# sergiventosa/ts-PWS

Hardware: AMD Instinct MI355X
Metric: stacked samples/s (Morlet ts-PWS, 10k×131072) + % HBM roofline, 1/2/4/8 GPU (higher is better)
Workload: dtype f64; 1 GPU; 10000 traces/GPU x 131072 samples, Morlet w0=pi*sqrt(2/ln2) V=4 J=14, two-stage K=10 + unbiased phase coherence (BASELINE configs[2]); HBM-resident float32 traces; traces_total=10000, traces_per_gpu=10000, parallelism=one GPU: no collective, world_size=1

## Files before the change

include/tspws_hip.h:

```cpp
#ifndef TSPWS_HIP_H
#define TSPWS_HIP_H

#include <stddef.h>
#include <stdint.h>
#include "ts_pws1f_lib.h"

#ifdef __cplusplus
extern "C" {
#endif

enum {
	TSPWS_OK        = 0,
	TSPWS_E_ARG     = -1,
	TSPWS_E_NOMEM   = 4,
	TSPWS_E_NODEV   = 5,
	TSPWS_E_HIP     = 6,
	TSPWS_E_FRAME   = 7
};

typedef struct tspws_hip_plan tspws_hip_plan;

typedef struct {
	int      type;
	unsigned S, V, J, N;
	double   s0, b0, w0;
	double   Cpsi;
	size_t   ncoef;
	size_t   ntaps;
	int      device;
} tspws_hip_frame_info;

int         tspws_hip_device_count(void);
const char *tspws_hip_last_error(void);
int  tspws_hip_alloc(void **d_ptr, size_t bytes, int device);
int  tspws_hip_free(void *d_ptr);
int  tspws_hip_upload(void *d_dst, const void *h_src, size_t bytes, void *stream);
int  tspws_hip_download(void *h_dst, const void *d_src, size_t bytes, void *stream);
int  tspws_hip_zero(void *d_ptr, size_t bytes, void *stream);
int  tspws_hip_sync(void *stream);


void tspws_resolve_params(t_tsPWS *p, unsigned nsamp, float dt);

int  tspws_hip_plan_create(tspws_hip_plan **plan, int type, unsigned J, unsigned V, unsigned N,
                           double s0, double b0, double w0, int uni, int device);
void tspws_hip_plan_destroy(tspws_hip_plan *plan);
int  tspws_hip_plan_info(const tspws_hip_plan *plan, tspws_hip_frame_info *info);
int  tspws_hip_plan_tables(const tspws_hip_plan *plan, double *scale, unsigned *L, int *c, int *cd,
                           unsigned *D, unsigned *Ns);
int  tspws_hip_plan_taps(const tspws_hip_plan *plan, double *h_w, double *h_wd);

int  tspws_hip_fold(float *d_sigall, size_t mtr, size_t max, size_t ld, void *stream);
int  tspws_hip_remove_mean(float *d_sigall, size_t mtr, size_t max, size_t ld, void *stream);

int  tspws_hip_partial_stacks(tspws_hip_plan *plan, const float *d_sigall, size_t ld,
                              size_t mtr_local, size_t first, size_t mtr_global, unsigned Kmax,
                              double *d_P, size_t ldP, void *stream);

int  tspws_hip_partial_stacks_range(tspws_hip_plan *plan, const float *d_sigall, size_t ld,
                                    size_t mtr_local, size_t first, size_t mtr_global, unsigned Kmax,
                                    unsigned g_begin, unsigned g_end, double *d_P, size_t ldP, void *stream);

int  tspws_hip_forward_f64(tspws_hip_plan *plan, const double *d_x, size_t ntr, size_t ld, double *d_Y, void *stream);
int  tspws_hip_forward_f32(tspws_hip_plan *plan, const float  *d_x, size_t ntr, size_t ld, double *d_Y, void *stream);
unsigned tspws_hip_spectral_first_scale(const tspws_hip_plan *plan, unsigned nsmax);
unsigned tspws_hip_spectral_end_scale(const tspws_hip_plan *plan);
unsigned tspws_hip_spectral_transform_length(const tspws_hip_plan *plan);
unsigned tspws_hip_spectral_choice(const tspws_hip_plan *plan, size_t ntr);
int  tspws_hip_forward_spectral_f64(tspws_hip_plan *plan, const double *d_x, size_t ntr, size_t ld, double *d_Y, unsigned nsmax, void *stream);
int  tspws_hip_forward_spectral_f32(tspws_hip_plan *plan, const float  *d_x, size_t ntr, size_t ld, double *d_Y, unsigned nsmax, void *stream);
int  tspws_hip_inverse(tspws_hip_plan *plan, const double *d_Y, size_t nrec, double *d_x, void *stream);
typedef struct {
	unsigned items;
	unsigned per_scale;
	unsigned waves;
	unsigned waves_lds;
	unsigned waves_fast;
	unsigned generic;
} tspws_hip_inverse_info_t;
int  tspws_hip_inverse_info(const tspws_hip_plan *plan, tspws_hip_inverse_info_t *info);

typedef struct { unsigned s_begin, s_end; } tspws_band;
#define TSPWS_MAX_BANDS 1024u
int  tspws_hip_inverse_bands(tspws_hip_plan *plan, const double *d_Y, size_t nset, const tspws_band *h_bands, unsigned R,
                             double *d_re, double *d_im, void *stream);
int  tspws_bands_from_frequencies(const double *scale, unsigned S, double w0, double dt, const double *f_lo, const double *f_hi, unsigned R,
                                  tspws_band *bands, double *fc);

int  tspws_hip_accumulate(tspws_hip_plan *plan, const double *d_Y, size_t ntr, double *d_ST, double *d_PS,
                          int zero_first, void *stream);
int  tspws_hip_stacks_double(tspws_hip_plan *plan, const double *d_P, unsigned K, size_t ldP,
                             double *d_ST, double *d_PS, void *stream);
int  tspws_hip_stacks_float(tspws_hip_plan *plan, const float *d_sigall, size_t mtr, size_t ld,
                            double *d_ST, double *d_PS, void *stream);
int  tspws_hip_weight(tspws_hip_plan *plan, double *d_OUT, const double *d_ST, const double *d_PS,
                      unsigned K, unsigned M, double wu, int unbiased, void *stream);
int  tspws_hip_epilogue(float *d_ls, float *d_tsPWS, const double *d_x_st, const double *d_x_out,
                        size_t N, unsigned mtr, void *stream);

int  tspws_hip_stack_local(tspws_hip_plan *plan, const t_tsPWS *p, const float *d_sigall, size_t ld,
                           size_t mtr_local, size_t first, size_t mtr_global, void *stream);
int  tspws_hip_reduce_buffer(tspws_hip_plan *plan, const t_tsPWS *p, size_t mtr_global,
                             double **d_buf, size_t *ndoubles);
int  tspws_hip_stack_finish(tspws_hip_plan *plan, const t_tsPWS *p, size_t mtr_global,
                            float *d_ls, float *d_tsPWS, void *stream);

int  tspws_hip_stack_finish_range(tspws_hip_plan *plan, const t_tsPWS *p, size_t mtr_global,
                                  unsigned g_begin, unsigned g_end, void *stream);
int  tspws_hip_stack_finish_tail(tspws_hip_plan *plan, const t_tsPWS *p, size_t mtr_global,
                                 float *d_ls, float *d_tsPWS, void *stream);

int  tspws_hip_stack(tspws_hip_plan *plan, const t_tsPWS *p, const float *d_sigall, size_t ld, size_t mtr,
                     float *d_ls, float *d_tsPWS, void *stream);
int  tspws_hip_stack_batch(tspws_hip_plan *plan, const t_tsPWS *p, const float *d_sigall, size_t ld, const size_t *h_first, unsigned B,
                           float *d_ls, float *d_tsPWS, void *stream);
typedef struct {
	unsigned single_pass;
	unsigned two_stage_pass;
	unsigned looped;
	unsigned empty;
	unsigned rounds;
	unsigned pass_batches;
} tspws_hip_batch_stats;
int  tspws_hip_stack_batch_stats(const tspws_hip_plan *plan, tspws_hip_batch_stats *stats);
int  tspws_hip_stack_batch_bands(tspws_hip_plan *plan, const t_tsPWS *p, const float *d_sigall, size_t ld, const size_t *h_first, unsigned B,
                                 const tspws_band *h_bands, unsigned R, float *d_ls, float *d_tsPWS, float *d_ls_env, float *d_tsPWS_env,
                                 void *stream);
typedef struct {
	tspws_hip_batch_stats batch;
	unsigned finish_batches;
	unsigned scales;
	unsigned quadrature;
} tspws_hip_stack_bands_stats;
int  tspws_hip_stack_batch_bands_stats(const tspws_hip_plan *plan, tspws_hip_stack_bands_stats *stats);
int  tspws_hip_profile_begin(tspws_hip_plan *plan, size_t max_calls);
int  tspws_hip_profile_read(tspws_hip_plan *plan, double *stage_ms, double *call_ms, size_t cap, size_t *ncalls);
int  tspws_hip_profile_end(tspws_hip_plan *plan, double *mean_ms, size_t *ncalls);
int  tspws_hip_stream_launches(const tspws_hip_plan *plan);

int  tspws_hip_finish_shard(const tspws_hip_plan *plan, const t_tsPWS *p, size_t mtr_global, unsigned rank, unsigned world,
                            unsigned *s_begin, unsigned *s_end);
int  tspws_hip_stack_finish_scales(tspws_hip_plan *plan, const t_tsPWS *p, size_t mtr_global, unsigned s_begin, unsigned s_end,
                                   double *d_x2, void *stream);

int  tspws_jackknife_plan(char *sel, const time_t *time, size_t mtr, unsigned d, unsigned n, unsigned C);
int  tspws_hip_jackknife(tspws_hip_plan *plan, const t_tsPWS *p, const float *d_sigall, size_t ld,
                         size_t mtr, const char *h_sel, unsigned C,
                         float *d_ls_out, float *d_ts_out, unsigned *h_mtr_out, void *stream);

int  tspws_hip_stack_jackknife(tspws_hip_plan *plan, const t_tsPWS *p, const float *d_sigall, size_t ld, size_t mtr,
                               float *d_ls, float *d_tsPWS, const char *h_sel, unsigned C,
                               float *d_ls_out, float *d_ts_out, unsigned *h_mtr_out, void *stream);

int  tspws_hip_jackknife_buffer(tspws_hip_plan *plan, const t_tsPWS *p, unsigned C, double **d_buf, size_t *nd);
int  tspws_hip_jackknife_local(tspws_hip_plan *plan, const t_tsPWS *p, const float *d_sigall, size_t ld, size_t mtr_local,
                               size_t first, size_t mtr_global, const char *h_sel, unsigned C, void *stream);
int  tspws_hip_jackknife_finish(tspws_hip_plan *plan, const t_tsPWS *p, size_t mtr_global, const char *h_sel, unsigned C,
                                unsigned c_begin, unsigned c_end, float *d_ls_out, float *d_ts_out, unsigned *h_mtr_out,
                                void *stream);

int  tspws_selection_classes(const char *sel, unsigned C, size_t mtr, unsigned *class_of_trace, char *kept, unsigned *ncls);
int  tspws_hip_jackknife_single(tspws_hip_plan *plan, const t_tsPWS *p, const float *d_sigall, size_t ld, size_t mtr,
                                const char *h_sel, unsigned C, float *d_ls_out, float *d_ts_out, unsigned *h_mtr_out, void *stream);

int  tspws_hip_jackknife_batch(tspws_hip_plan *plan, const t_tsPWS *p, const float *d_sigall, size_t ld, const size_t *h_first, unsigned B,
                               const char *h_sel, unsigned C, float *d_ls, float *d_tsPWS, float *d_ls_out, float *d_ts_out,
                               unsigned *h_mtr_out, void *stream);
typedef struct {
	unsigned shared;
	unsigned looped;
	unsigned empty;
	unsigned rounds;
	unsigned pass_batches;
	unsigned classes;
} tspws_hip_jk_batch_stats;
int  tspws_hip_jackknife_batch_stats(const tspws_hip_plan *plan, tspws_hip_jk_batch_stats *stats);

int  tspws_hip_jackknife_batch_two_stage(tspws_hip_plan *plan, const t_tsPWS *p, const float *d_sigall, size_t ld, const size_t *h_first,
                                         unsigned B, const char *h_sel, unsigned C, float *d_ls, float *d_tsPWS, float *d_ls_out,
                                         float *d_ts_out, unsigned *h_mtr_out, void *stream);
typedef struct {
	unsigned shared;
	unsigned looped;
	unsigned empty;
	unsigned rounds;
	unsigned tiles;
	unsigned rows;
} tspws_hip_jk_batch2_stats;
int  tspws_hip_jackknife_batch_two_stage_stats(const tspws_hip_plan *plan, tspws_hip_jk_batch2_stats *stats);

int  tspws_subsampling_plan(char *sel, size_t J, size_t K);
int  tspws_hip_subsample(tspws_hip_plan *plan, const t_tsPWS *p, const float *d_sigall, size_t ld, size_t mtr, unsigned M,
                         float *d_ls_out, float *d_ts_out, void *stream);
int  tspws_hip_subsample_sel(tspws_hip_plan *plan, const t_tsPWS *p, const float *d_sigall, size_t ld, size_t mtr, unsigned M,
                             const char *h_sel, float *d_ls_out, float *d_ts_out, void *stream);

int  tspws_subsampling_plan_batch(char *sel, const size_t *first, unsigned B, unsigned M, double prob);
int  tspws_hip_subsample_batch_sel(tspws_hip_plan *plan, const t_tsPWS *p, const float *d_sigall, size_t ld, const size_t *h_first, unsigned B,
                                   unsigned M, const char *h_sel, float *d_ls_out, float *d_ts_out, unsigned *h_mtr_out, void *stream);
int  tspws_hip_subsample_batch(tspws_hip_plan *plan, const t_tsPWS *p, const float *d_sigall, size_t ld, const size_t *h_first, unsigned B,
                               unsigned M, float *d_ls_out, float *d_ts_out, unsigned *h_mtr_out, void *stream);
typedef struct {
	unsigned single_shared;
	unsigned two_stage_shared;
	unsigned looped;
	unsigned empty;
	unsigned rounds;
	unsigned rows;
} tspws_hip_sub_batch_stats;
int  tspws_hip_subsample_batch_stats(const tspws_hip_plan *plan, tspws_hip_sub_batch_stats *stats);

int  tspws_bootstrap_plan(unsigned char *cnt, size_t J);
int  tspws_bootstrap_plan_batch(unsigned char *cnt, const size_t *first, unsigned B, unsigned M);
int  tspws_hip_bootstrap_batch_cnt(tspws_hip_plan *plan, const t_tsPWS *p, const float *d_sigall, size_t ld, const size_t *h_first, unsigned B,
                                   unsigned M, const unsigned char *h_cnt, float *d_ls_out, float *d_ts_out, unsigned *h_mtr_out, float *d_stats,
                                   void *stream);
int  tspws_hip_bootstrap_batch(tspws_hip_plan *plan, const t_tsPWS *p, const float *d_sigall, size_t ld, const size_t *h_first, unsigned B,
                               unsigned M, float *d_ls_out, float *d_ts_out, unsigned *h_mtr_out, float *d_stats, void *stream);
typedef struct {
	unsigned shared;
	unsigned empty;
	unsigned rounds;
	unsigned rows;
	unsigned max_count;
} tspws_hip_boot_batch_stats;
int  tspws_hip_bootstrap_batch_stats(const tspws_hip_plan *plan, tspws_hip_boot_batch_stats *stats);

int  tspws_hip_weighted_stack_batch(tspws_hip_plan *plan, const t_tsPWS *p, const float *d_sigall, size_t ld, const size_t *h_first, unsigned B,
                                    unsigned M, const double *h_w, float *d_ls_out, float *d_ts_out, unsigned *h_mtr_out, double *h_keff,
                                    void *stream);
typedef struct {
	unsigned shared;
	unsigned empty;
	unsigned rounds;
	unsigned rows;
} tspws_hip_weighted_batch_stats;
int  tspws_hip_weighted_stack_batch_stats(const tspws_hip_plan *plan, tspws_hip_weighted_batch_stats *stats);
int  tspws_weights_from_scores(double *w, const double *score, const size_t *first, unsigned B, int rule, double a);

int  tspws_hip_replica_bands(tspws_hip_plan *plan, const float *d_rows, size_t ld, unsigned B, unsigned M, const unsigned *h_mtr,
                             const double *h_q, unsigned Q, float *d_bands, void *stream);
typedef struct {
	unsigned lds;
	unsigned global;
	unsigned empty;
	unsigned rounds;
	unsigned lds_max_rows;
} tspws_hip_bands_stats;
int  tspws_hip_replica_bands_stats(const tspws_hip_plan *plan, tspws_hip_bands_stats *stats);

int  tspws_hip_trace_scores(tspws_hip_plan *plan, const float *d_sigall, size_t ld, const size_t *h_first, unsigned B, const float *d_ref,
                            size_t ldr, unsigned R, size_t n0, size_t n1, double *d_scores, double *d_energy, void *stream);
typedef struct {
	unsigned vec;
	unsigned segments;
	unsigned rounds;
	unsigned empty;
} tspws_hip_trace_scores_stats_t;
int  tspws_hip_trace_scores_stats(const tspws_hip_plan *plan, tspws_hip_trace_scores_stats_t *stats);
int  tspws_selection_from_scores(char *sel, unsigned *kept, const double *score, const size_t *first, unsigned B, int rule, double a);
int  tspws_hip_selective_stack_batch(tspws_hip_plan *plan, const t_tsPWS *p, const float *d_sigall, size_t ld, const size_t *h_first, unsigned B,
                                     int against, int rule, double a, unsigned iters, size_t n0, size_t n1, float *d_ls, float *d_tsPWS,
                                     char *h_sel, unsigned *h_kept, unsigned *iters_done, void *stream);

int  tspws_hip_stretch_rows(tspws_hip_plan *plan, const float *d_rows, size_t ld, unsigned B, unsigned M, const unsigned *h_mtr,
                            const float *d_ref, size_t ldr, double z, const double *h_eps, unsigned E, const size_t *h_win, unsigned W,
                            double *d_cc, double *d_fit, void *stream);
typedef struct {
	unsigned rounds;
	unsigned segments;
	unsigned rows;
	unsigned left_out;
	unsigned chunks;
} tspws_hip_stretch_stats;
int  tspws_hip_stretch_rows_stats(const tspws_hip_plan *plan, tspws_hip_stretch_stats *stats);
int  tspws_stretch_grid(double *eps, double eps_max, unsigned E);

int  tspws_hip_wxs_coef(tspws_hip_plan *plan, const double *d_Yc, const double *d_Yr, const unsigned *h_ens, size_t nrow, unsigned B, double z,
                        const tspws_band *h_bands, unsigned R, const size_t *h_win, unsigned W, int skip_wrapped, double *d_sums, double *d_fit,
                        void *stream);
int  tspws_hip_wxs_rows(tspws_hip_plan *plan, const float *d_rows, size_t ld, unsigned B, unsigned M, const unsigned *h_mtr, const float *d_ref,
                        size_t ldr, double z, const tspws_band *h_bands, unsigned R, const size_t *h_win, unsigned W, int skip_wrapped,
                        double *d_sums, double *d_fit, void *stream);
typedef struct {
	unsigned rounds;
	unsigned rows;
	unsigned left_out;
	unsigned items;
	unsigned scales;
} tspws_hip_wxs_stats;
int  tspws_hip_wxs_rows_stats(const tspws_hip_plan *plan, tspws_hip_wxs_stats *stats);

typedef struct {
	unsigned L, hop, P, q0, q1, h;
	double taper, min_coh, max_err, max_delta, err_floor;
} tspws_mwcs_par;
int    tspws_mwcs_bins(unsigned P, double dt, double f_lo, double f_hi, unsigned *q0, unsigned *q1);
size_t tspws_mwcs_basis_size(const tspws_mwcs_par *par);
int    tspws_mwcs_basis(const tspws_mwcs_par *par, double *tab);
int  tspws_hip_mwcs_rows(tspws_hip_plan *plan, const float *d_rows, size_t ld, unsigned B, unsigned M, const unsigned *h_mtr, const float *d_ref,
                         size_t ldr, double z, const tspws_mwcs_par *par, const size_t *h_win, unsigned W, double *d_win, double *d_fit,
                         double *d_spec, double *d_spec_ref, void *stream);
typedef struct {
	unsigned rounds;
	unsigned rows;
	unsigned left_out;
	unsigned windows;
	unsigned bins;
} tspws_hip_mwcs_stats;
int  tspws_hip_mwcs_rows_stats(const tspws_hip_plan *plan, tspws_hip_mwcs_stats *stats);

typedef struct { unsigned Lmax, b; } tspws_dtw_par;
int  tspws_hip_dtw_rows(tspws_hip_plan *plan, const float *d_rows, size_t ld, unsigned B, unsigned M, const unsigned *h_mtr, const float *d_ref,
                        size_t ldr, double z, const tspws_dtw_par *par, const size_t *h_win, unsigned W, int *d_lag, double *d_fit, void *stream);
typedef struct {
	unsigned rounds;
	unsigned rows;
	unsigned left_out;
	unsigned lags;
	unsigned samples;
} tspws_hip_dtw_stats;
int  tspws_hip_dtw_rows_stats(const tspws_hip_plan *plan, tspws_hip_dtw_stats *stats);

int  tspws_hip_ftan_coef(tspws_hip_plan *plan, const double *d_Y, const unsigned *h_ens, size_t nrow, unsigned B, double z, unsigned s_begin,
                         unsigned s_end, const size_t *h_win, unsigned W, const size_t *h_noise, unsigned P, int skip_wrapped, double *d_peaks,
                         double *d_noise, void *stream);
int  tspws_hip_ftan_rows(tspws_hip_plan *plan, const float *d_rows, size_t ld, unsigned B, unsigned M, const unsigned *h_mtr, double z,
                         unsigned s_begin, unsigned s_end, const size_t *h_win, unsigned W, const size_t *h_noise, unsigned P, int skip_wrapped,
                         double *d_peaks, double *d_noise, void *stream);
typedef struct {
	unsigned rounds;
	unsigned rows;
	unsigned left_out;
	unsigned items;
	unsigned classes;
} tspws_hip_ftan_stats;
int  tspws_hip_ftan_rows_stats(const tspws_hip_plan *plan, tspws_hip_ftan_stats *stats);
int  tspws_ftan_windows(double dist, double vmin, double vmax, double dt, double z, size_t N, int sides, size_t *win);
int  tspws_ftan_periods(const double *scale, unsigned S, double w0, double dt, double *T);

int  tspws_hip_convergence(tspws_hip_plan *plan, const t_tsPWS *p, const float *d_sigall, size_t ld, size_t mtr,
                           const float *d_ref_ts, const float *d_ref_ls, double *h_ts_sim, double *h_ts_misfit,
                           double *h_ls_sim, double *h_ls_misfit, float *d_ts_steps, float *d_ls_steps, void *stream);

int  tspws_hip_convergence_batch(tspws_hip_plan *plan, const t_tsPWS *p, const float *d_sigall, size_t ld, const size_t *h_first, unsigned B,
                                 const float *d_ref_ts, const float *d_ref_ls, double *h_ts_sim, double *h_ts_misfit, double *h_ls_sim,
                                 double *h_ls_misfit, float *d_ts_steps, float *d_ls_steps, void *stream);
typedef struct {
	unsigned single_steps;
	unsigned two_stage_steps;
	unsigned rows;
	unsigned rounds;
	unsigned looped;
	unsigned empty;
} tspws_hip_conv_batch_stats;
int  tspws_hip_convergence_batch_stats(const tspws_hip_plan *plan, tspws_hip_conv_batch_stats *stats);

typedef struct tspws_hip_comm tspws_hip_comm;
int   tspws_hip_comm_create(tspws_hip_comm **comm, int ndev, const int *devices);
void  tspws_hip_comm_destroy(tspws_hip_comm *comm);
int   tspws_hip_comm_size(const tspws_hip_comm *comm);
int   tspws_hip_comm_device(const tspws_hip_comm *comm, int i);
void *tspws_hip_comm_stream(const tspws_hip_comm *comm, int i);
const char *tspws_hip_comm_backend(const tspws_hip_comm *comm);
int   tspws_hip_allreduce_f64(tspws_hip_comm *comm, double *const *d_bufs, size_t count, void *const *streams);
int   tspws_hip_reduce_f64(tspws_hip_comm *comm, double *const *d_bufs, size_t count, int root, void *const *streams);
void  tspws_shard_range(size_t mtr, unsigned r, unsigned n, size_t *first, size_t *count);

typedef struct tspws_hip_multi tspws_hip_multi;
int   tspws_hip_multi_create(tspws_hip_multi **m, int ndev, const int *devices, int type, unsigned J, unsigned V, unsigned N,
                             double s0, double b0, double w0, int uni);
void  tspws_hip_multi_destroy(tspws_hip_multi *m);
tspws_hip_comm *tspws_hip_multi_comm(tspws_hip_multi *m);
// ... 21 lines not shown
```

ts-pws_amd/__init__.py:

```python
import ctypes as C
import os
import subprocess

_HERE = os.path.dirname(os.path.abspath(__file__))
ROOT = os.path.dirname(_HERE)
LIB_PATH = os.environ.get("TSPWS_LIB_PATH") or os.path.join(_HERE, "lib", "libtspws_hip.so")

time_t = C.c_long


class t_tsPWS(C.Structure):
    _fields_ = [
        ("type", C.c_int), ("uni", C.c_uint), ("J", C.c_uint), ("V", C.c_uint),
        ("s0", C.c_double), ("b0", C.c_double), ("w0", C.c_double), ("wu", C.c_double),
        ("fmin", C.c_double), ("Q", C.c_double), ("cycle", C.c_double),
        ("w0set", C.c_int), ("lrm", C.c_int), ("bin", C.c_int), ("lkinst", C.c_int),
        ("lVfix", C.c_int), ("ls0fix", C.c_int), ("lb0fix", C.c_int), ("verbose", C.c_int),
        ("fold", C.c_int), ("unbiased", C.c_int), ("convergence", C.c_int),
        ("subsmpl_N", C.c_uint), ("subsmpl_p", C.c_double),
        ("jackknife_n", C.c_uint), ("jackknife_d", C.c_uint), ("obin", C.c_uint),
        ("AllSteps", C.c_int), ("Nmax", C.c_uint), ("Kmax", C.c_uint),
        ("kinst", C.c_char_p), ("filein", C.c_char_p), ("fileout", C.c_char_p), ("fileconv", C.c_char_p),
    ]


class FrameInfo(C.Structure):
    _fields_ = [
        ("type", C.c_int), ("S", C.c_uint), ("V", C.c_uint), ("J", C.c_uint), ("N", C.c_uint),
        ("s0", C.c_double), ("b0", C.c_double), ("w0", C.c_double), ("Cpsi", C.c_double),
        ("ncoef", C.c_size_t), ("ntaps", C.c_size_t), ("device", C.c_int),
    ]


class InverseInfo(C.Structure):
    _fields_ = [("items", C.c_uint), ("per_scale", C.c_uint), ("waves", C.c_uint), ("waves_lds", C.c_uint), ("waves_fast", C.c_uint),
                ("generic", C.c_uint)]


class TspwsError(RuntimeError):
    pass


def build(verbose=False):
    out = subprocess.run(["make", "-C", _HERE, "all"], capture_output=True, text=True)
    if verbose or out.returncode:
        print(out.stdout + out.stderr)
    if out.returncode:
        raise TspwsError("building libtspws_hip.so failed")
    return LIB_PATH


_lib = None

_vp, _u, _d, _sz, _i, _f = C.c_void_p, C.c_uint, C.c_double, C.c_size_t, C.c_int, C.c_float
SYMBOLS = {
    "tspws_main": (_i, [_vp, _vp, _vp]),
    "tspws_hip_device_count": (_i, []),
    "tspws_hip_last_error": (C.c_char_p, []),
    "tspws_hip_alloc": (_i, [C.POINTER(_vp), _sz, _i]),
    "tspws_hip_free": (_i, [_vp]),
    "tspws_hip_upload": (_i, [_vp, _vp, _sz, _vp]),
    "tspws_hip_download": (_i, [_vp, _vp, _sz, _vp]),
    "tspws_hip_zero": (_i, [_vp, _sz, _vp]),
    "tspws_hip_sync": (_i, [_vp]),
    "tspws_resolve_params": (None, [_vp, _u, _f]),
    "tspws_hip_plan_create": (_i, [C.POINTER(_vp), _i, _u, _u, _u, _d, _d, _d, _i, _i]),
    "tspws_hip_plan_destroy": (None, [_vp]),
    "tspws_hip_plan_info": (_i, [_vp, _vp]),
    "tspws_hip_plan_tables": (_i, [_vp] + [_vp] * 6),
    "tspws_hip_plan_taps": (_i, [_vp, _vp, _vp]),
    "tspws_hip_fold": (_i, [_vp, _sz, _sz, _sz, _vp]),
    "tspws_hip_remove_mean": (_i, [_vp, _sz, _sz, _sz, _vp]),
    "tspws_hip_partial_stacks": (_i, [_vp, _vp, _sz, _sz, _sz, _sz, _u, _vp, _sz, _vp]),
    "tspws_hip_partial_stacks_range": (_i, [_vp, _vp, _sz, _sz, _sz, _sz, _u, _u, _u, _vp, _sz, _vp]),
    "tspws_hip_forward_f64": (_i, [_vp, _vp, _sz, _sz, _vp, _vp]),
    "tspws_hip_forward_f32": (_i, [_vp, _vp, _sz, _sz, _vp, _vp]),
    "tspws_hip_spectral_first_scale": (_u, [_vp, _u]),
    "tspws_hip_spectral_end_scale": (_u, [_vp]),
    "tspws_hip_spectral_transform_length": (_u, [_vp]),
    "tspws_hip_spectral_choice": (_u, [_vp, _sz]),
    "tspws_hip_forward_spectral_f64": (_i, [_vp, _vp, _sz, _sz, _vp, _u, _vp]),
    "tspws_hip_forward_spectral_f32": (_i, [_vp, _vp, _sz, _sz, _vp, _u, _vp]),
    "tspws_hip_inverse": (_i, [_vp, _vp, _sz, _vp, _vp]),
    "tspws_hip_inverse_info": (_i, [_vp, _vp]),
    "tspws_hip_inverse_bands": (_i, [_vp, _vp, _sz, _vp, _u, _vp, _vp, _vp]),
    "tspws_bands_from_frequencies": (_i, [_vp, _u, _d, _d, _vp, _vp, _u, _vp, _vp]),
    "tspws_hip_accumulate": (_i, [_vp, _vp, _sz, _vp, _vp, _i, _vp]),
    "tspws_hip_stacks_double": (_i, [_vp, _vp, _u, _sz, _vp, _vp, _vp]),
    "tspws_hip_stacks_float": (_i, [_vp, _vp, _sz, _sz, _vp, _vp, _vp]),
    "tspws_hip_weight": (_i, [_vp, _vp, _vp, _vp, _u, _u, _d, _i, _vp]),
    "tspws_hip_epilogue": (_i, [_vp, _vp, _vp, _vp, _sz, _u, _vp]),
    "tspws_hip_stack_local": (_i, [_vp, _vp, _vp, _sz, _sz, _sz, _sz, _vp]),
    "tspws_hip_reduce_buffer": (_i, [_vp, _vp, _sz, C.POINTER(_vp), C.POINTER(_sz)]),
    "tspws_hip_stack_finish": (_i, [_vp, _vp, _sz, _vp, _vp, _vp]),
    "tspws_hip_stack_finish_range": (_i, [_vp, _vp, _sz, _u, _u, _vp]),
    "tspws_hip_stack_finish_tail": (_i, [_vp, _vp, _sz, _vp, _vp, _vp]),
    "tspws_hip_stack": (_i, [_vp, _vp, _vp, _sz, _sz, _vp, _vp, _vp]),
    "tspws_hip_stack_batch": (_i, [_vp, _vp, _vp, _sz, _vp, _u, _vp, _vp, _vp]),
    "tspws_hip_stack_batch_stats": (_i, [_vp, _vp]),
    "tspws_hip_stack_batch_bands": (_i, [_vp, _vp, _vp, _sz, _vp, _u, _vp, _u, _vp, _vp, _vp, _vp, _vp]),
    "tspws_hip_stack_batch_bands_stats": (_i, [_vp, _vp]),
    "tspws_hip_profile_begin": (_i, [_vp, _sz]),
    "tspws_hip_profile_read": (_i, [_vp, _vp, _vp, _sz, C.POINTER(_sz)]),
    "tspws_hip_profile_end": (_i, [_vp, C.POINTER(_d), C.POINTER(_sz)]),
    "tspws_hip_stream_launches": (_i, [_vp]),
    "tspws_jackknife_plan": (_i, [_vp, _vp, _sz, _u, _u, _u]),
    "tspws_hip_jackknife": (_i, [_vp, _vp, _vp, _sz, _sz, _vp, _u, _vp, _vp, _vp, _vp]),
    "tspws_hip_stack_jackknife": (_i, [_vp, _vp, _vp, _sz, _sz, _vp, _vp, _vp, _u, _vp, _vp, _vp, _vp]),
    "tspws_main_release": (None, []),
    "tspws_main_on": (_i, [_i, _vp, _vp, _vp]),
    "tspws_main_cached_devices": (C.c_ulonglong, []),
    "tspws_hip_finish_shard": (_i, [_vp, _vp, _sz, _u, _u, C.POINTER(_u), C.POINTER(_u)]),
    "tspws_hip_stack_finish_scales": (_i, [_vp, _vp, _sz, _u, _u, _vp, _vp]),
    "tspws_hip_jackknife_buffer": (_i, [_vp, _vp, _u, C.POINTER(_vp), C.POINTER(_sz)]),
    "tspws_hip_jackknife_local": (_i, [_vp, _vp, _vp, _sz, _sz, _sz, _sz, _vp, _u, _vp]),
    "tspws_hip_jackknife_finish": (_i, [_vp, _vp, _sz, _vp, _u, _u, _u, _vp, _vp, _vp, _vp]),
    "tspws_selection_classes": (_i, [_vp, _u, _sz, _vp, _vp, C.POINTER(_u)]),
    "tspws_hip_jackknife_single": (_i, [_vp, _vp, _vp, _sz, _sz, _vp, _u, _vp, _vp, _vp, _vp]),
    "tspws_hip_jackknife_batch": (_i, [_vp, _vp, _vp, _sz, _vp, _u, _vp, _u, _vp, _vp, _vp, _vp, _vp, _vp]),
    "tspws_hip_jackknife_batch_stats": (_i, [_vp, _vp]),
    "tspws_hip_jackknife_batch_two_stage": (_i, [_vp, _vp, _vp, _sz, _vp, _u, _vp, _u, _vp, _vp, _vp, _vp, _vp, _vp]),
    "tspws_hip_jackknife_batch_two_stage_stats": (_i, [_vp, _vp]),
    "tspws_subsampling_plan": (_i, [_vp, _sz, _sz]),
    "tspws_hip_subsample": (_i, [_vp, _vp, _vp, _sz, _sz, _u, _vp, _vp, _vp]),
    "tspws_hip_subsample_sel": (_i, [_vp, _vp, _vp, _sz, _sz, _u, _vp, _vp, _vp, _vp]),
    "tspws_subsampling_plan_batch": (_i, [_vp, _vp, _u, _u, _d]),
    "tspws_hip_subsample_batch_sel": (_i, [_vp, _vp, _vp, _sz, _vp, _u, _u, _vp, _vp, _vp, _vp, _vp]),
    "tspws_hip_subsample_batch": (_i, [_vp, _vp, _vp, _sz, _vp, _u, _u, _vp, _vp, _vp, _vp]),
    "tspws_hip_subsample_batch_stats": (_i, [_vp, _vp]),
    "tspws_bootstrap_plan": (_i, [_vp, _sz]),
    "tspws_bootstrap_plan_batch": (_i, [_vp, _vp, _u, _u]),
    "tspws_hip_bootstrap_batch_cnt": (_i, [_vp, _vp, _vp, _sz, _vp, _u, _u, _vp, _vp, _vp, _vp, _vp, _vp]),
    "tspws_hip_bootstrap_batch": (_i, [_vp, _vp, _vp, _sz, _vp, _u, _u, _vp, _vp, _vp, _vp, _vp]),
    "tspws_hip_bootstrap_batch_stats": (_i, [_vp, _vp]),
    "tspws_hip_weighted_stack_batch": (_i, [_vp, _vp, _vp, _sz, _vp, _u, _u, _vp, _vp, _vp, _vp, _vp, _vp]),
    "tspws_hip_weighted_stack_batch_stats": (_i, [_vp, _vp]),
    "tspws_weights_from_scores": (_i, [_vp, _vp, _vp, _u, _i, _d]),
    "tspws_hip_replica_bands": (_i, [_vp, _vp, _sz, _u, _u, _vp, _vp, _u, _vp, _vp]),
    "tspws_hip_replica_bands_stats": (_i, [_vp, _vp]),
    "tspws_hip_trace_scores": (_i, [_vp, _vp, _sz, _vp, _u, _vp, _sz, _u, _sz, _sz, _vp, _vp, _vp]),
    "tspws_hip_trace_scores_stats": (_i, [_vp, _vp]),
    "tspws_selection_from_scores": (_i, [_vp, _vp, _vp, _vp, _u, _i, _d]),
    "tspws_hip_stretch_rows": (_i, [_vp, _vp, _sz, _u, _u, _vp, _vp, _sz, _d, _vp, _u, _vp, _u, _vp, _vp, _vp]),
    "tspws_hip_stretch_rows_stats": (_i, [_vp, _vp]),
    "tspws_stretch_grid": (_i, [_vp, _d, _u]),
    "tspws_hip_wxs_coef": (_i, [_vp, _vp, _vp, _vp, _sz, _u, _d, _vp, _u, _vp, _u, _i, _vp, _vp, _vp]),
    "tspws_hip_wxs_rows": (_i, [_vp, _vp, _sz, _u, _u, _vp, _vp, _sz, _d, _vp, _u, _vp, _u, _i, _vp, _vp, _vp]),
    "tspws_hip_wxs_rows_stats": (_i, [_vp, _vp]),
    "tspws_hip_mwcs_rows": (_i, [_vp, _vp, _sz, _u, _u, _vp, _vp, _sz, _d, _vp, _vp, _u, _vp, _vp, _vp, _vp, _vp]),
    "tspws_hip_mwcs_rows_stats": (_i, [_vp, _vp]),
    "tspws_mwcs_bins": (_i, [_u, _d, _d, _d, _vp, _vp]),
    "tspws_hip_dtw_rows": (_i, [_vp, _vp, _sz, _u, _u, _vp, _vp, _sz, _d, _vp, _vp, _u, _vp, _vp, _vp]),
    "tspws_hip_dtw_rows_stats": (_i, [_vp, _vp]),
    "tspws_hip_ftan_coef": (_i, [_vp, _vp, _vp, _sz, _u, _d, _u, _u, _vp, _u, _vp, _u, _i, _vp, _vp, _vp]),
    "tspws_hip_ftan_rows": (_i, [_vp, _vp, _sz, _u, _u, _vp, _d, _u, _u, _vp, _u, _vp, _u, _i, _vp, _vp, _vp]),
    "tspws_hip_ftan_rows_stats": (_i, [_vp, _vp]),
    "tspws_ftan_windows": (_i, [_d, _d, _d, _d, _d, _sz, _i, _vp]),
    "tspws_ftan_periods": (_i, [_vp, _u, _d, _d, _vp]),
    "tspws_mwcs_basis_size": (_sz, [_vp]),
    "tspws_mwcs_basis": (_i, [_vp, _vp]),
    "tspws_hip_selective_stack_batch": (_i, [_vp, _vp, _vp, _sz, _vp, _u, _i, _i, _d, _u, _sz, _sz, _vp, _vp, _vp, _vp, _vp, _vp]),
    "tspws_hip_convergence": (_i, [_vp, _vp, _vp, _sz, _sz, _vp, _vp, _vp, _vp, _vp, _vp, _vp, _vp, _vp]),
    "tspws_hip_convergence_batch": (_i, [_vp, _vp, _vp, _sz, _vp, _u, _vp, _vp, _vp, _vp, _vp, _vp, _vp, _vp, _vp]),
    "tspws_hip_convergence_batch_stats": (_i, [_vp, _vp]),
    "tspws_hip_synth": (_i, [_vp, _sz, _sz, _sz, C.c_uint64, _sz, _vp]),
    "tspws_hip_comm_create": (_i, [C.POINTER(_vp), _i, _vp]),
    "tspws_hip_comm_destroy": (None, [_vp]),
    "tspws_hip_comm_size": (_i, [_vp]),
    "tspws_hip_comm_device": (_i, [_vp, _i]),
    "tspws_hip_comm_stream": (_vp, [_vp, _i]),
    "tspws_hip_comm_backend": (C.c_char_p, [_vp]),
    "tspws_hip_allreduce_f64": (_i, [_vp, _vp, _sz, _vp]),
    "tspws_hip_reduce_f64": (_i, [_vp, _vp, _sz, _i, _vp]),
    "tspws_shard_range": (None, [_sz, _u, _u, C.POINTER(_sz), C.POINTER(_sz)]),
    "tspws_hip_multi_create": (_i, [C.POINTER(_vp), _i, _vp, _i, _u, _u, _u, _d, _d, _d, _i]),
    "tspws_hip_multi_destroy": (None, [_vp]),
    "tspws_hip_multi_comm": (_vp, [_vp]),
    "tspws_hip_multi_plan": (_vp, [_vp, _i]),
    "tspws_hip_multi_upload": (_i, [_vp, _vp, _sz, _sz, C.POINTER(_vp), C.POINTER(_vp), C.POINTER(_vp)]),
    "tspws_hip_multi_prologue": (_i, [_vp, _vp, _sz, _sz, _sz, _i, _i]),
    "tspws_hip_multi_stack": (_i, [_vp, _vp, _vp, _sz, _sz, _vp, _vp]),
    "tspws_hip_multi_stack_jackknife": (_i, [_vp, _vp, _vp, _sz, _sz, _vp, _vp, _vp, _u, _vp, _vp, _vp]),
}


def load():
    global _lib
    if _lib is None:
        if not os.path.exists(LIB_PATH):
            raise TspwsError(f"{LIB_PATH} is missing: run __graft_entry__.build() / make -C ts-pws_amd")
        try:
            import torch
        except ImportError:
            pass
        lib = C.CDLL(LIB_PATH)
        for name, (res, args) in SYMBOLS.items():
            fn = getattr(lib, name)
            fn.restype, fn.argtypes = res, args
        _lib = lib
    return _lib


def check(rc, what=""):
    if rc:
        raise TspwsError(f"{what} failed with code {rc}: {load().tspws_hip_last_error().decode()}")


def _offsets(first, limit=None, rows="trace rows"):
    import numpy as np
    f = np.asarray(first)
    if f.ndim != 1 or f.size < 1 or f.dtype.kind not in "iu":
        raise TspwsError("first must be a 1-D integer array of B + 1 ensemble offsets")
    if (f < 0).any() or (np.diff(f) < 0).any() or (limit is not None and int(f[-1]) > limit):
        raise TspwsError("first must be non-decreasing offsets" + (f" into the {limit} {rows}" if limit is not None else " >= 0"))
    f = np.ascontiguousarray(f, dtype=np.uint64)
    return f, f.size - 1, int(f[-1] - f[0])


def _host_array(a, name, dtype, shape, optional=False):
    import numpy as np
    if a is None and optional:
        return None
    if not isinstance(a, np.ndarray) or a.dtype != dtype or a.shape != shape or not (optional or a.flags.c_contiguous):
        dims = f"of {shape[0]} entries" if len(shape) == 1 else "".join(f"[{n}]" for n in shape)
        raise TspwsError(f"{name} must be {'None or a' if optional else 'a contiguous'} {np.dtype(dtype).name} numpy array {dims}")
    return a if a.flags.c_contiguous else np.ascontiguousarray(a)


def _score_plane(score, T):
    import numpy as np
    if hasattr(score, "detach"):
        score = score.detach().cpu().numpy()
    sc = np.ascontiguousarray(score, dtype=np.float64)
    if sc.shape != (T,):
        raise TspwsError(f"score must be one plane of {T} scores, got {sc.shape}")
    return sc


def resolve(params, nsamp, dt=1.0):
    p = t_tsPWS.from_buffer_copy(params)
    load().tspws_resolve_params(C.byref(p), nsamp, dt)
    return p


def shard_range(mtr_global, rank, world):
    first = rank * mtr_global // world
    last = (rank + 1) * mtr_global // world
    return first, last - first


class Plan:

    def __init__(self, params, N, device=0):
        self.lib = load()
        self.params = t_tsPWS.from_buffer_copy(params)
        h = C.c_void_p()
        p = self.params
        check(self.lib.tspws_hip_plan_create(C.byref(h), p.type, p.J, p.V, N, p.s0, p.b0, p.w0, int(p.uni), device), "plan_create")
        self.h = h
        info = FrameInfo()
        check(self.lib.tspws_hip_plan_info(self.h, C.byref(info)), "plan_info")
        self.info = info
        self.N, self.S, self.ncoef, self.ntaps, self.Cpsi = N, info.S, info.ncoef, info.ntaps, info.Cpsi
        self.device = device

    def tables(self):
        import numpy as np
        S = self.S
        t = dict(scale=np.zeros(S), L=np.zeros(S, np.uint32), c=np.zeros(S, np.int32), cd=np.zeros(S, np.int32),
                 D=np.zeros(S, np.uint32), Ns=np.zeros(S, np.uint32))
        check(self.lib.tspws_hip_plan_tables(self.h, *[t[k].ctypes.data for k in ("scale", "L", "c", "cd", "D", "Ns")]), "plan_tables")
        return t

    def taps(self):
        import numpy as np
        w = np.zeros(self.ntaps, np.complex128)
        wd = np.zeros(self.ntaps, np.complex128)
        check(self.lib.tspws_hip_plan_taps(self.h, w.ctypes.data, wd.ctypes.data), "plan_taps")
        return w, wd

    @staticmethod
    def _stream():
        import torch
        return C.c_void_p(torch.cuda.current_stream().cuda_stream)

    def reduce_buffer(self, mtr_global):
        import torch
        ptr, n = C.c_void_p(), C.c_size_t()
        check(self.lib.tspws_hip_reduce_buffer(self.h, C.byref(self.params), mtr_global, C.byref(ptr), C.byref(n)), "reduce_buffer")
        return _as_tensor(ptr.value, n.value, torch.float64, self.device)

    def _traces(self, traces, dtype=None):
        import torch
        dtype = dtype or torch.float32
        if traces.dtype != dtype or traces.dim() != 2 or traces.shape[1] != self.N:
            raise TspwsError(f"traces must be {dtype} [mtr][{self.N}], got {traces.dtype} {tuple(traces.shape)}")
        if traces.shape[0] and traces.stride(1) != 1:
            raise TspwsError("traces must be contiguous along the samples (stride(1) == 1)")
        if not traces.is_cuda or (traces.device.index or 0) != self.device:
            raise TspwsError(f"traces live on {traces.device}, the plan on cuda:{self.device}")
        mtr = traces.shape[0]
        ld = traces.stride(0) if mtr > 1 else traces.shape[1]
        if ld < self.N:
            raise TspwsError("overlapping trace rows (stride(0) < N)")
        return mtr, ld

    def _need(self, t, name, dt, size, what="{} tensor", exact=False):
        import torch
        if not isinstance(t, torch.Tensor) or t.dtype != getattr(torch, dt) or not t.is_contiguous() or not t.is_cuda or (t.device.index or 0) != self.device or \
                (tuple(t.shape) != size if isinstance(size, tuple) else t.numel() < size or (exact and t.numel() != size)):
            dims = "".join(f"[{n}]" for n in size) if isinstance(size, tuple) else size
            raise TspwsError(f"{name} must be a contiguous {dt} {what.format(dims)} on cuda:{self.device}")

    def _out(self, t, name):
        self._need(t, name, "float32", self.N, "tensor of >= {} samples")
        return t.data_ptr()

    def _refs(self, t, name, rows):
        one = rows == 1 and getattr(t, "ndim", 2) == 1
        self._need(t, name, "float32", (self.N,) if one else (rows, self.N), f"[{rows}][{self.N}] tensor")
        return t.data_ptr()

    def _rows_out(self, lead, device, ls_out, ts_out, mtr_out=None, counts=True, new="empty", what="{} tensor"):
        import numpy as np
        import torch
        if new is not None:
            ls_out = getattr(torch, new)((*lead, self.N), dtype=torch.float32, device=device) if ls_out is None else ls_out
            ts_out = getattr(torch, new)((*lead, self.N), dtype=torch.float32, device=device) if ts_out is None else ts_out
            mtr_out = np.zeros(lead, np.uint32) if mtr_out is None and counts else mtr_out
        if counts:
            _host_array(mtr_out, "mtr_out", np.uint32, lead)
        self._need(ls_out, "ls_out", "float32", (*lead, self.N), what)
        self._need(ts_out, "ts_out", "float32", (*lead, self.N), what)
        return ls_out, ts_out, mtr_out

    def _coef_sets(self, Y, what):
        import numpy as np
        import torch
        if not isinstance(Y, (np.ndarray, torch.Tensor)):
            raise TspwsError("Y must be a complex128 numpy array or device tensor")
        host = isinstance(Y, np.ndarray)
        if Y.dtype != (np.complex128 if host else torch.complex128) or Y.ndim != 2 or Y.shape[1] != self.ncoef or not Y.shape[0]:
            raise TspwsError(f"Y must be complex128 [{what} >= 1][{self.ncoef}], got {Y.dtype} {tuple(Y.shape)}")
        if host:
            return torch.as_tensor(np.ascontiguousarray(Y), device=f"cuda:{self.device}"), True
        if not Y.is_cuda or (Y.device.index or 0) != self.device or not Y.is_contiguous():
            raise TspwsError(f"Y must be a contiguous tensor on cuda:{self.device}, got {Y.device}")
        return Y, False

    def _strided_rows(self, t, name="rows", kind="", mid="M"):
        import torch
        if not isinstance(t, torch.Tensor) or t.dtype != torch.float32 or t.dim() != 3 or t.shape[2] != self.N:
            raise TspwsError(f"{name} must be a float32 [B][{mid}][{self.N}] tensor, got {getattr(t, 'dtype', type(t))} {tuple(getattr(t, 'shape', ()))}")
        if not t.is_cuda or (t.device.index or 0) != self.device:
            raise TspwsError(f"{name} live on {t.device}, the plan on cuda:{self.device}")
        B, Mn = t.shape[0], t.shape[1]
        ld = t.stride(1) if Mn > 1 else (t.stride(0) if B > 1 else self.N)
        if B and Mn:
            if t.stride(2) != 1:
                raise TspwsError(f"{name} must be contiguous along the samples (stride(2) == 1)")
            if ld < self.N:
                raise TspwsError(f"overlapping {kind}rows (row stride < N)")
            if B > 1 and t.stride(0) != Mn * ld:
                raise TspwsError(f"{name} must be a [B][{mid}][N] view of one [B][{mid}][ld] base (stride(0) == {mid} * stride(1))")
        return B, Mn, ld

    def _strided_refs(self, ref, B):
        import torch
        if not isinstance(ref, torch.Tensor) or ref.dtype != torch.float32 or tuple(ref.shape) != (B, self.N):
            raise TspwsError(f"ref must be a float32 [{B}][{self.N}] tensor, got {getattr(ref, 'dtype', type(ref))} {tuple(getattr(ref, 'shape', ()))}")
        if not ref.is_cuda or (ref.device.index or 0) != self.device:
            raise TspwsError(f"ref lives on {ref.device}, the plan on cuda:{self.device}")
        ldr = ref.stride(0) if B > 1 else self.N
        if B and (ref.stride(1) != 1 or ldr < self.N):
            raise TspwsError("ref must be contiguous along the samples, its rows not overlapping")
        return ldr

    @staticmethod
    def _windows(windows):
        import numpy as np
        try:
            wa = np.ascontiguousarray(np.asarray(windows, dtype=np.int64))
        except (TypeError, ValueError):
            raise TspwsError("windows must be a sequence of (n0, n1) pairs of non-negative integers") from None
# ... 1002 lines not shown
```

ts-pws_amd/csrc/forward.hip:

```cpp
#include "tspws_internal.h"
#include <type_traits>

#ifndef FL_PASSES
#define FL_PASSES 2
#endif
#ifndef FL_WAVES
#define FL_WAVES 4
#endif
#ifndef FL_PASSES_FINE
#define FL_PASSES_FINE 1
#endif

template <typename TIn, bool BLOCK_PER_OUT>
__global__ void __launch_bounds__(256) k_fwd_generic(const TIn *__restrict__ x, size_t ld, unsigned N, const ScaleDesc *__restrict__ sc,
                                                     unsigned S, const double2 *__restrict__ w, double2 *__restrict__ Y, size_t ncoef,
                                                     unsigned long long first_coef, unsigned long long n_items)
{
	__shared__ double red[8];
	const unsigned lane = threadIdx.x & 63, wv = threadIdx.x >> 6;
	unsigned long long item = BLOCK_PER_OUT ? blockIdx.x : (unsigned long long)blockIdx.x * 4 + wv;
	if (item >= n_items) return;
	const unsigned long long ci = first_coef + item;
	const unsigned s = find_scale(sc, S, ci, false);
	const ScaleDesc d = sc[s];
// ... 376 lines not shown
template int tspws_forward_parts<float>(tspws_hip_plan *, const float *, size_t, size_t, double2 *, hipStream_t, FuseOut *, ScaleRange);
template int tspws_forward_parts<double>(tspws_hip_plan *, const double *, size_t, size_t, double2 *, hipStream_t, FuseOut *, ScaleRange);

#if FL_ABLATE
extern "C" int tspws_hip_fwd_ablate(void)
{
	if (const char *e = sweep_env("TSPWS_FWD_CLASSES")) {
		const unsigned m = (unsigned)strtoul(e, nullptr, 16);
		HIP_TRY(hipMemcpyToSymbol(HIP_SYMBOL(fl_class_mask), &m, sizeof m));
	}
	return 0;
}
#endif

#if FL_TIMING
extern "C" int tspws_hip_fwd_timing(unsigned long long *h_out, int reset)
{
	static unsigned long long *d_buf = nullptr;
	if (!d_buf) {
		HIP_TRY(hipMalloc(&d_buf, 56 * sizeof(unsigned long long)));
		HIP_TRY(hipMemset(d_buf, 0, 56 * sizeof(unsigned long long)));
		HIP_TRY(hipMemcpyToSymbol(HIP_SYMBOL(fl_timing_out), &d_buf, sizeof d_buf));
	}
	HIP_TRY(hipDeviceSynchronize());
	if (h_out) HIP_TRY(hipMemcpy(h_out, d_buf, 56 * sizeof(unsigned long long), hipMemcpyDeviceToHost));
	if (reset) HIP_TRY(hipMemset(d_buf, 0, 56 * sizeof(unsigned long long)));
	return 0;
}
#endif

size_t tspws_part_budget_bytes()
{
	static size_t v = 0;
	if (!v) { const char *e = getenv("TSPWS_PART_MB"); v = (size_t)(e ? std::max(16, atoi(e)) : 2048) << 20; }
	return v;
}

bool tspws_generic_forward()
{
	static int v = -1;
	if (v < 0) { const char *e = sweep_env("TSPWS_FWD_GENERIC"); v = (e && *e == '1') ? 1 : 0; }
	return v == 1;
}

bool tspws_fused_forward(const tspws_hip_plan *p) { return p->n_fusable != 0; }

static bool many_trace_size(const tspws_hip_plan *p, size_t ntr) { return ntr >= 128 && (double)ntr * (double)p->N >= 7.0 * 1048576.0; }
static bool spectral_size(const tspws_hip_plan *p, size_t ntr) { return ntr >= 64 && ((double)ntr * (double)p->N >= 1048576.0 || ntr >= 256); }
unsigned tspws_spectral_choice(const tspws_hip_plan *p, size_t ntr)
{
	const int eng = tspws_engine_pin();
	static unsigned nsmax_env = ~0u;
	if (nsmax_env == ~0u) { const char *m = sweep_env("TSPWS_SPEC_NSMAX"); nsmax_env = m ? (unsigned)std::max(2, atoi(m)) : 0u; }
	if (eng == 1 || tspws_generic_forward() || !ntr) return p->S;
	if (eng == 0 && !spectral_size(p, ntr)) return p->S;
	const unsigned dmin = p->V > 2 ? 32u : 16u;
	return tspws_spectral_first_scale(p, nsmax_env ? nsmax_env : std::max(512u, (p->N + dmin - 1) / dmin));
}

bool tspws_many_trace_path(const tspws_hip_plan *p, size_t ntr)
{
	if (tspws_generic_forward()) return false;
	if (tspws_spectral_choice(p, ntr) < p->S) return true;
	if (!(p->tl[0].n || p->tl[1].n)) return false;
	const long forced = tl_min_env();
	if (forced > 0) return ntr >= (size_t)forced;
	return p->V > 2 && many_trace_size(p, ntr);
}

template <typename TIn>
static int forward_impl(tspws_hip_plan *p, const TIn *d_x, size_t ntr, size_t ld, double *d_Y, hipStream_t st)
{
	if (!p || !d_x || !d_Y) return fail(TSPWS_E_ARG, "forward: NULL");
	if (!ntr) return 0;
	HIP_TRY(hipSetDevice(p->device));
	if (tspws_generic_forward()) return forward_generic<TIn>(p, d_x, ntr, ld, d_Y, st);
	const size_t batch = std::min<size_t>(ntr, std::max<size_t>(2, ((tspws_part_budget_bytes()) / (p->npart * sizeof(double2))) & ~(size_t)1));
	void *v;
	int rc = scratch(p, SCR_PART, batch * p->npart * sizeof(double2), &v);
	if (rc) return rc;
	for (size_t t0 = 0; t0 < ntr; t0 += batch) {
		const size_t nb = std::min(batch, ntr - t0);
		if ((rc = tspws_forward_parts<TIn>(p, d_x + t0 * ld, nb, ld, (double2 *)v, st, nullptr, ScaleRange()))) return rc;
		hipLaunchKernelGGL(k_gather_parts, dim3((unsigned)((p->ncoef + 255) / 256), (unsigned)nb), dim3(256), 0, st, (const double2 *)v,
		                   p->npart, p->d_sc, p->S, (double2 *)d_Y + t0 * p->ncoef, p->ncoef);
	}
	HIP_TRY(hipGetLastError());
	return 0;
}

extern "C" int tspws_hip_forward_f64(tspws_hip_plan *p, const double *d_x, size_t ntr, size_t ld, double *d_Y, void *s)
{
	return forward_impl<double>(p, d_x, ntr, ld, d_Y, S_(s));
}
extern "C" int tspws_hip_forward_f32(tspws_hip_plan *p, const float *d_x, size_t ntr, size_t ld, double *d_Y, void *s)
{
	return forward_impl<float>(p, d_x, ntr, ld, d_Y, S_(s));
}

template <typename TIn>
static int forward_spectral(tspws_hip_plan *p, const TIn *d_x, size_t ntr, size_t ld, double *d_Y, unsigned nsmax, hipStream_t st)
{
	if (!p || !d_x || !d_Y) return fail(TSPWS_E_ARG, "forward_spectral: NULL");
	if (!ntr) return 0;
	HIP_TRY(hipSetDevice(p->device));
	const unsigned sf = tspws_spectral_first_scale(p, nsmax);
	if (sf >= p->S) return fail(TSPWS_E_ARG, "forward_spectral: this frame has no spectral set");
	SpecDecomp *dc = nullptr;
	int rc;
	if ((rc = tspws_spectral_decomp(p, sf, (unsigned)std::min<size_t>((ntr + 63) / 64, 64), &dc))) return rc;
	const size_t batch = std::min<size_t>(4096, (ntr + 63) & ~(size_t)63);
	void *v;
	if ((rc = scratch(p, SCR_XT, (size_t)p->N * batch * sizeof(TIn), &v))) return rc;
	TIn *xT = (TIn *)v;
	for (size_t t0 = 0; t0 < ntr; t0 += batch) {
		const unsigned nb = (unsigned)std::min(batch, ntr - t0), nblk = (nb + 63) / 64, TP = nblk * 64;
		if ((rc = tspws_spectral_transpose<TIn>(p, d_x + t0 * ld, ld, nb, xT, TP, st))) return rc;
		if ((rc = tspws_spectral_run<TIn>(p, dc, (const TIn *)xT, TP, nb, nullptr, nullptr, 0, (double2 *)d_Y + t0 * p->ncoef, st))) return rc;
	}
	HIP_TRY(hipGetLastError());
	return 0;
}

extern "C" unsigned tspws_hip_spectral_first_scale(const tspws_hip_plan *p, unsigned nsmax) { return p ? tspws_spectral_first_scale(p, nsmax) : 0u; }
extern "C" unsigned tspws_hip_spectral_end_scale(const tspws_hip_plan *p) { return p ? tspws_spectral_end_scale(p) : 0u; }
extern "C" unsigned tspws_hip_spectral_transform_length(const tspws_hip_plan *p)
{
	unsigned NT = 0, e, c;
	if (p) tspws_spectral_geometry(p, &NT, &e, &c);
	return NT;
}
extern "C" unsigned tspws_hip_spectral_choice(const tspws_hip_plan *p, size_t ntr) { return p ? tspws_spectral_choice(p, ntr) : 0u; }
extern "C" int tspws_hip_forward_spectral_f64(tspws_hip_plan *p, const double *d_x, size_t ntr, size_t ld, double *d_Y, unsigned nsmax, void *s)
{
	return forward_spectral<double>(p, d_x, ntr, ld, d_Y, nsmax, S_(s));
}
extern "C" int tspws_hip_forward_spectral_f32(tspws_hip_plan *p, const float *d_x, size_t ntr, size_t ld, double *d_Y, unsigned nsmax, void *s)
{
	return forward_spectral<float>(p, d_x, ntr, ld, d_Y, nsmax, S_(s));
}

__global__ void __launch_bounds__(256) k_accumulate(const double2 *__restrict__ Y, size_t ncoef, unsigned ntr, double2 *__restrict__ ST,
                                                    double2 *__restrict__ PS, int zero_first)
{
	const size_t i = (size_t)blockIdx.x * 256 + threadIdx.x;
	if (i >= ncoef) return;
	double2 st = zero_first ? make_double2(0, 0) : ST[i];
	double2 ps = zero_first ? make_double2(0, 0) : PS[i];
	for (unsigned b = 0; b < ntr; b++) {
		const double2 v = Y[(size_t)b * ncoef + i];
		st.x += v.x; st.y += v.y;
		add_unit_phasor(ps, v);
	}
	ST[i] = st; PS[i] = ps;
}

extern "C" int tspws_hip_accumulate(tspws_hip_plan *p, const double *d_Y, size_t ntr, double *d_ST, double *d_PS, int zero_first, void *s)
{
	if (!p || !d_ST || !d_PS || (ntr && !d_Y)) return fail(TSPWS_E_ARG, "accumulate: NULL");
	HIP_TRY(hipSetDevice(p->device));
	hipLaunchKernelGGL(k_accumulate, dim3((unsigned)((p->ncoef + 255) / 256)), dim3(256), 0, S_(s), (const double2 *)d_Y, p->ncoef,
	                   (unsigned)ntr, (double2 *)d_ST, (double2 *)d_PS, zero_first);
	HIP_TRY(hipGetLastError());
	return 0;
}

void tspws_launch_accumulate(tspws_hip_plan *p, const double2 *part, unsigned nb, double2 *ST, double2 *PS, int zero_first, const FuseOut *fz,
                             unsigned nslices, hipStream_t st, unsigned nbatch, size_t y_part, size_t y_stack, const TlTable *tl, const WeightArgs *wa,
                             ScaleRange rg, const AccExtra *ex)
{
	const size_t trace_stride = ex ? ex->trace_stride : 0;
	const WeightArgs w0;
	const bool on = fz && fz->applied;
	const bool direct = on && fz->accST == ST;
	const LaunchRange lr = launch_range(p, rg);
	const unsigned a0 = tl ? 0u : lr.acc0, a1 = tl ? tl->acc2_blocks : lr.acc1;
	if (a1 <= a0) return;
	auto kern = (wa && wa->OUTP) ? k_accumulate_parts<true> : k_accumulate_parts<false>;
	hipLaunchKernelGGL(kern, dim3(a1 - a0, nbatch), dim3(256), 0, st, part, trace_stride ? trace_stride : (tl ? tl->npart : p->npart),
	                   (const ScaleDesc *)(tl ? tl->d_sc : p->d_sc), p->S, nb, ST, PS, zero_first,
	                   (ex && ex->fused_done) ? 3 : on ? (direct ? 1 : 2) : 0, on ? (const double2 *)fz->accST : nullptr, on ? (const double2 *)fz->accPS : nullptr,
	                   on ? fz->stride : (size_t)0, nslices, y_part, y_stack, tl ? 1 : 0, wa ? *wa : w0, a0, ex ? ex->y_fz : (size_t)0,
	                   ex ? ex->rowmap : (const unsigned *)nullptr);
}

unsigned tspws_first_unfused_scale(const tspws_hip_plan *p)
{
	unsigned s = 0;
	while (s < p->S && p->sc[s].fuse_ok) s++;
	return s;
}

static unsigned fuse_tps(const tspws_hip_plan *p, size_t nb)
{
	static int target = -1;
	if (target < 0) { const char *e = sweep_env("TSPWS_FUSE_WGS"); target = e ? std::max(1, atoi(e)) : 256; }
	unsigned tps = (unsigned)std::min<size_t>(nb, 32);
	static int mintps = -1;
	if (mintps < 0) { const char *e = sweep_env("TSPWS_FUSE_MINTPS"); mintps = e ? std::max(1, atoi(e)) : 3; }
	while (tps > 1 && (tps + 1) / 2 >= (unsigned)mintps && (size_t)std::max(1u, p->lds_blocks) * ((nb + tps - 1) / tps) < (size_t)target) tps = (tps + 1) / 2;
	return std::max(1u, tps);
}

template <typename TIn>
int tspws_tl_pass_setup(tspws_hip_plan *p, size_t ntr, size_t nslots, TlPass &P)
{
	int rc;
	void *v;
	unsigned pick = ((nslots + 63) / 64 >= 12 && p->V > 2) ? 0u : 1u;
	if (const char *e = sweep_env("TSPWS_TL_PICK")) pick = atoi(e) ? 1u : 0u;
	SpecDecomp *dc = nullptr;
	const unsigned spec_first = tspws_spectral_choice(p, ntr);
	if (spec_first < p->S && (rc = tspws_spectral_decomp(p, spec_first, (unsigned)std::min<size_t>((nslots + 63) / 64, 64), &dc))) return rc;
	const TlTable &T = dc ? dc->T : p->tl[p->tl[pick].n ? pick : 1u - pick];
	size_t batch = std::min<size_t>(4096, std::max<size_t>(64, (((size_t)1 << 30) / ((size_t)p->N * sizeof(TIn))) & ~(size_t)63));
	if (T.npart) batch = std::min(batch, std::max<size_t>(64, (tspws_part_budget_bytes() / (T.npart * sizeof(double2))) & ~(size_t)63));
	if (const char *e = sweep_env("TSPWS_TL_BATCH")) batch = std::max<size_t>(64, (size_t)atoi(e) & ~(size_t)63);
	batch = std::min(batch, (nslots + 63) & ~(size_t)63);
	const size_t nblk_max = batch / 64;
	if ((rc = scratch(p, SCR_XT, (size_t)p->N * batch * sizeof(TIn), &v))) return rc;
	P.xT = v;
	if ((rc = scratch(p, SCR_FZ, nblk_max * 2 * p->ncoef * sizeof(double2), &v))) return rc;
	P.planes = (double2 *)v;
	P.part = P.gsum = nullptr;
	if (T.npart) { if ((rc = scratch(p, SCR_PART, batch * T.npart * sizeof(double2), &v))) return rc; P.part = (double2 *)v; }
	if (T.gcoltiles) { if ((rc = scratch(p, SCR_GEMM, (size_t)T.gKS * batch * T.gcoltiles * 16 * sizeof(double2), &v))) return rc; P.gsum = (double2 *)v; }
	P.dc = dc; P.T = &T; P.batch = batch;
	return 0;
}

template <typename TIn>
int tspws_tl_pass_transform(tspws_hip_plan *p, const TlPass &P, const TIn *xb, size_t ld, unsigned nb, hipStream_t st)
{
	int rc;
	SpecDecomp *dc = P.dc;
	const TlTable &T = *P.T;
	const unsigned nblk = (nb + 63) / 64, TP = nblk * 64;
	TIn *xT = (TIn *)P.xT;
	double2 *planes = P.planes, *part = P.part, *gsum = P.gsum;
	hipStream_t sp = st;
	bool poly_join = false;
	static const int gemm_order = sweep_env("TSPWS_GEMM_ORDER") ? atoi(sweep_env("TSPWS_GEMM_ORDER")) : 1;
	auto launch_gemm = [&](hipStream_t gs) {
		hipLaunchKernelGGL((k_fwd_gemm<TIn>), dim3((T.gcoltiles + 3) / 4, T.gKS, nblk), dim3(256), 0, gs, (const TIn *)xT, TP, nb, p->N,
		                   (const GemmCol *)T.d_gcols, T.gcoltiles, T.gKC, (const double2 *)p->d_w, gsum);
		const size_t nred = (size_t)nb * T.gcoltiles * 16;
		hipLaunchKernelGGL(k_gemm_reduce, dim3((unsigned)((nred + 255) / 256)), dim3(256), 0, gs, (const double2 *)gsum, TP, nb, T.gcoltiles * 16, T.gKS,
		                   (const GemmCol *)T.d_gcols, part, T.npart);
	};
	if ((T.waves || (T.gcoltiles && gemm_order == 2)) && dc) {
		if ((rc = tspws_fork(p, st, p->xs, p->ev_xs0))) return rc;
		if (T.waves) launch_poly2<TIn>(p, xb, ld, nb, T.d_sc, part, T.npart, T.waves, 0u, p->xs);
		poly_join = true;
	} else if (T.waves) {
		if ((rc = tspws_fork(p, st, p->side, p->ev_fork))) return rc;
		sp = p->side;
		launch_poly2<TIn>(p, xb, ld, nb, T.d_sc, part, T.npart, T.waves, 0u, sp);
	}
	if (dc) { if ((rc = tspws_spectral_transpose<TIn>(p, xb, ld, nb, xT, TP, st))) return rc; }
	else hipLaunchKernelGGL((k_transpose_traces<TIn>), dim3((p->N + 63) / 64, nblk), dim3(256), 0, st, xb, ld, nb, p->N, TP, xT);
	static const bool spec_serial = sweep_env("TSPWS_SPEC_SERIAL") != nullptr;
	if (dc && ((T.n && !spec_serial) || (T.gcoltiles && gemm_order == 2))) {
		hipEvent_t forked = nullptr;
		if (T.n && !spec_serial) { if ((rc = tspws_fork(p, st, p->side, p->ev_fork))) return rc; sp = p->side; forked = p->ev_fork; }
		if (T.gcoltiles && gemm_order == 2) { if ((rc = tspws_fork(p, st, p->xs, p->ev_fork, forked))) return rc; launch_gemm(p->xs); }
	}
	if (T.gcoltiles && gemm_order == 0) launch_gemm(st);
	if (dc && (rc = tspws_spectral_run<TIn>(p, dc, (const TIn *)xT, TP, nb, planes, planes + p->ncoef, 2 * p->ncoef, nullptr, dc && T.n && !spec_serial ? sp : st))) return rc;
	if (T.n)
		hipLaunchKernelGGL((k_fwd_tl<TIn>), dim3(T.wgs, nblk), dim3(TL_NT), T.lds, st, (const TIn *)xT, TP, nb, p->N, T.d_items, T.n, p->d_w,
		                   planes, planes + p->ncoef, 2 * p->ncoef, part, T.npart);
	if (T.gcoltiles && gemm_order == 1) launch_gemm(st);
	if (sp != st && (rc = tspws_join(sp, st, p->ev_join))) return rc;
	if (poly_join && (rc = tspws_join(p->xs, st, p->ev_xs1))) return rc;
	return 0;
}
template int tspws_tl_pass_setup<float>(tspws_hip_plan *, size_t, size_t, TlPass &);
template int tspws_tl_pass_transform<float>(tspws_hip_plan *, const TlPass &, const float *, size_t, unsigned, hipStream_t);

template <typename TIn>
static int stacks_tl(tspws_hip_plan *p, const TIn *d_x, size_t ntr, size_t ld, double *d_ST, double *d_PS, hipStream_t st, bool keep,
                     const WeightArgs *wa, bool *weighted)
{
	int rc;
	TlPass P;
	if ((rc = tspws_tl_pass_setup<TIn>(p, ntr, ntr, P))) return rc;
	const size_t batch = P.batch;
	for (size_t t0 = 0; t0 < ntr; t0 += batch) {
		const unsigned nb = (unsigned)std::min(batch, ntr - t0), nblk = (nb + 63) / 64;
		if ((rc = tspws_tl_pass_transform<TIn>(p, P, d_x + t0 * ld, ld, nb, st))) return rc;
		FuseOut fz;
		fz.accST = P.planes; fz.accPS = P.planes + p->ncoef; fz.stride = 2 * p->ncoef; fz.tps = 64; fz.applied = true;
		const bool last = t0 + batch >= ntr;
		tspws_launch_accumulate(p, P.part, nb, (double2 *)d_ST, (double2 *)d_PS, (t0 == 0 && !keep) ? 1 : 0, &fz, nblk, st, 1, 0, 0, P.T, last && !keep ? wa : nullptr, ScaleRange());
		if (last && !keep && wa && wa->OUT && weighted) *weighted = true;
	}
	HIP_TRY(hipGetLastError());
	return 0;
}


template <typename TIn>
int tspws_stacks(tspws_hip_plan *p, const TIn *d_x, size_t ntr, size_t ld, double *d_ST, double *d_PS, hipStream_t st, bool keep,
                       const WeightArgs *wa, bool *weighted, ScaleRange rg)
{
	HIP_TRY(hipSetDevice(p->device));
	if (weighted) *weighted = false;
	if (!rg.on() && tspws_many_trace_path(p, ntr)) return stacks_tl<TIn>(p, d_x, ntr, ld, d_ST, d_PS, st, keep, wa, weighted);
	if (!ntr) { if (!keep) { HIP_TRY(hipMemsetAsync(d_ST, 0, p->ncoef * 16, st)); HIP_TRY(hipMemsetAsync(d_PS, 0, p->ncoef * 16, st)); } return 0; }
	int rc;
	if (tspws_generic_forward()) {
		size_t batch = std::max<size_t>(1, ((size_t)256 << 20) / (p->ncoef * sizeof(double2)));
		batch = std::min(batch, ntr);
		void *d_Y = nullptr;
		if ((rc = scratch(p, SCR_Y, batch * p->ncoef * sizeof(double2), &d_Y))) return rc;
		for (size_t t0 = 0; t0 < ntr; t0 += batch) {
			const size_t nb = std::min(batch, ntr - t0);
			if ((rc = forward_generic<TIn>(p, d_x + t0 * ld, nb, ld, (double *)d_Y, st))) return rc;
			if ((rc = tspws_hip_accumulate(p, (const double *)d_Y, nb, d_ST, d_PS, t0 == 0 && !keep, (void *)st))) return rc;
		}
		return 0;
	}
	const size_t batch = std::min<size_t>(ntr, std::max<size_t>(2, ((tspws_part_budget_bytes()) / (p->npart * sizeof(double2))) & ~(size_t)1));
	void *v;
	if ((rc = scratch(p, SCR_PART, batch * p->npart * sizeof(double2), &v))) return rc;
	const bool fuse = p->n_fusable != 0;
	void *vz = nullptr;
	if (fuse) {
		const unsigned tps = fuse_tps(p, batch);
		size_t nsl = (batch + tps - 1) / tps;
		if (const size_t last = ntr % batch) nsl = std::max(nsl, (last + fuse_tps(p, last) - 1) / fuse_tps(p, last));
		if (!(nsl == 1 && !keep && batch >= ntr) && (rc = scratch(p, SCR_FZ, nsl * 2 * p->ncoef * sizeof(double2), &vz))) return rc;
	}
	for (size_t t0 = 0; t0 < ntr; t0 += batch) {
		const size_t nb = std::min(batch, ntr - t0);
		const int zero_first = (t0 == 0 && !keep) ? 1 : 0;
		FuseOut fz;
		unsigned nsl = 0;
		if (fuse) {
			fz.tps = fuse_tps(p, nb);
			nsl = (unsigned)((nb + fz.tps - 1) / fz.tps);
			if (nsl == 1 && zero_first) { fz.accST = (double2 *)d_ST; fz.accPS = (double2 *)d_PS; fz.stride = 0; }
			else { fz.accST = (double2 *)vz; fz.accPS = (double2 *)vz + p->ncoef; fz.stride = 2 * p->ncoef; }
		}
		const bool all = nb == ntr && !keep;
		if ((rc = tspws_forward_parts<TIn>(p, d_x + t0 * ld, nb, ld, (double2 *)v, st, fuse ? &fz : nullptr, rg))) return rc;
		tspws_launch_accumulate(p, (const double2 *)v, (unsigned)nb, (double2 *)d_ST, (double2 *)d_PS, zero_first, &fz, nsl, st, 1, 0, 0, nullptr, all ? wa : nullptr, rg);
		if (all && wa && wa->OUT && weighted) *weighted = true;
	}
	HIP_TRY(hipGetLastError());
	return 0;
}

template int tspws_stacks<float>(tspws_hip_plan *, const float *, size_t, size_t, double *, double *, hipStream_t, bool, const WeightArgs *, bool *, ScaleRange);
template int tspws_stacks<double>(tspws_hip_plan *, const double *, size_t, size_t, double *, double *, hipStream_t, bool, const WeightArgs *, bool *, ScaleRange);

extern "C" int tspws_hip_stacks_double(tspws_hip_plan *p, const double *d_P, unsigned K, size_t ldP, double *d_ST, double *d_PS, void *s)
{
	if (!p || !d_P || !d_ST || !d_PS) return fail(TSPWS_E_ARG, "stacks_double: NULL");
	return tspws_stacks<double>(p, d_P, K, ldP, d_ST, d_PS, S_(s), false, nullptr, nullptr, ScaleRange());
}

extern "C" int tspws_hip_stacks_float(tspws_hip_plan *p, const float *d_x, size_t mtr, size_t ld, double *d_ST, double *d_PS, void *s)
{
	if (!p || !d_x || !d_ST || !d_PS) return fail(TSPWS_E_ARG, "stacks_float: NULL");
	return tspws_stacks<float>(p, d_x, mtr, ld, d_ST, d_PS, S_(s), false, nullptr, nullptr, ScaleRange());
}
```

ts-pws_amd/csrc/spectral.hip:

```cpp
#include "tspws_internal.h"
#include "lane_reduce.h"
#include "spectral.h"


namespace {
constexpr double quarter64(int k)
{
	return k == 0 ? 1.0 : k == 1 ? 0.9951847266721969 : k == 2 ? 0.9807852804032304 : k == 3 ? 0.9569403357322088 : k == 4 ? 0.9238795325112867
	     : k == 5 ? 0.881921264348355 : k == 6 ? 0.8314696123025452 : k == 7 ? 0.773010453362737 : k == 8 ? 0.7071067811865476
	     : k == 9 ? 0.6343932841636455 : k == 10 ? 0.5555702330196023 : k == 11 ? 0.4713967368259978 : k == 12 ? 0.38268343236508984
	     : k == 13 ? 0.29028467725446233 : k == 14 ? 0.19509032201612833 : k == 15 ? 0.09801714032956077 : 0.0;
}
constexpr double cos64(int k)
{
	k = ((k % 64) + 64) % 64;
	return k <= 16 ? quarter64(k) : k <= 32 ? -quarter64(32 - k) : k <= 48 ? -quarter64(k - 32) : quarter64(64 - k);
}
constexpr double sin64(int k) { return cos64(k - 16); }

__device__ __forceinline__ double2 cadd(const double2 a, const double2 b) { return make_double2(a.x + b.x, a.y + b.y); }
__device__ __forceinline__ double2 csub(const double2 a, const double2 b) { return make_double2(a.x - b.x, a.y - b.y); }
__device__ __forceinline__ double2 cmul(const double2 a, const double2 b) { return make_double2(fma(a.x, b.x, -a.y * b.y), fma(a.x, b.y, a.y * b.x)); }

template <int R, bool INV, int K> struct SpecBfly {
// ... 449 lines not shown
				for (unsigned k = 0; k < 4 && m; k++) {
					const unsigned sidx = (unsigned)__builtin_ctz(m);
					m &= m - 1u;
					const unsigned sld = (unsigned)__builtin_amdgcn_readlane((int)my.ld, (int)sidx), slb = (unsigned)__builtin_amdgcn_readlane((int)my.lb, (int)sidx);
					const unsigned long long sgo = ((unsigned long long)(unsigned)__builtin_amdgcn_readlane((int)(my.goff >> 32), (int)sidx) << 32) |
					                               (unsigned)__builtin_amdgcn_readlane((int)(unsigned)my.goff, (int)sidx);
					const unsigned ilo = slb ? (__brev(c >> sld) >> (32 - slb)) : 0u;
					G[((size_t)tb * grows + sgo + r + (size_t)R * ilo) * 64 + lane] = make_double2(tile[wv][k][0][lane ^ (k << 3)], tile[wv][k][1][lane ^ (k << 3)]);
				}
			}
			if (done) {
#pragma unroll
				for (int t = 0; t < 4; t++) { cre[t] = (spec_v4d){0, 0, 0, 0}; cim[t] = (spec_v4d){0, 0, 0, 0}; }
			}
		}
	};
	for (unsigned c0 = 0;;) {
		block(oa, oc, c0); if ((c0 += 4) >= nsteps) break;
		block(ob, oa, c0); if ((c0 += 4) >= nsteps) break;
		block(oc, ob, c0); if ((c0 += 4) >= nsteps) break;
	}
	if (my.ld == 31u && my.lb != 31u) {
		double2 *dst = gc + (my.goff + r) * 64;
#pragma unroll
		for (int t = 0; t < 4; t++)
#pragma unroll
			for (int q = 0; q < 4; q++) dst[16 * t + 4 * q] = make_double2(cre[t][q], cim[t][q]);
	}
}

#define SPEC_EXACT_G 1024.0

struct SpecEpi {
	double2 *ST, *PS;
	size_t stride;
	const double *amax;
	double2 *Y;
	size_t ncoef;
	unsigned ntr;
	unsigned long long *mask;
	unsigned long long nspec, coff0;
};

template <int R, bool COEF>
__device__ __forceinline__ void spec_inv_last_body(const double2 *__restrict__ src, const SpecSeg *__restrict__ sg, unsigned j, const double2 *__restrict__ tw,
                                                   const SpecEpi &ep, unsigned tb, unsigned lane)
{
	const unsigned L = sg->L, k = j & (L - 1);
	double2 v[R];
	spec_load_tw<R, true>(v, src, sg, j, k, tw);
	SpecDFT<R, true>::run(v);
	const size_t j0 = (size_t)(j - k) * R + k;
	const unsigned t = tb * 64 + lane;
	if constexpr (COEF) {
		if (t < ep.ntr) {
			double2 *y = ep.Y + (size_t)t * ep.ncoef + sg->coff;
#pragma unroll
			for (int n = 0; n < R; n++) if (j0 + (size_t)n * L < sg->nvalid) y[j0 + (size_t)n * L] = make_double2(v[n].x, -v[n].y);
		}
		return;
	}
	const double am = ep.amax[t];
	const double thr = SPEC_EXACT_G * sg->tau * am, thr2 = thr * thr;
	const bool exact_ok = am > 0.0 && am <= 1.7976931348623157e308;
	unsigned long long *mrow = ep.mask + (size_t)tb * ep.nspec + (sg->coff - ep.coff0);
	const unsigned o16 = ((lane >> 5) & 1) * 8 + ((lane >> 4) & 1) * 4 + ((lane >> 3) & 1) * 2 + ((lane >> 2) & 1);
	double2 *pS = ep.ST + (size_t)tb * ep.stride + sg->coff, *pP = ep.PS + (size_t)tb * ep.stride + sg->coff;
	constexpr int NCH = (R + 7) / 8;
#pragma unroll
	for (int ch = 0; ch < NCH; ch++) {
		if (j0 + (size_t)(ch * 8) * L >= sg->nvalid) break;
		double st16[16], ps16[16];
#pragma unroll
		for (int i = 0; i < 8; i++) {
			const int n = ch * 8 + i;
			double2 y = make_double2(0.0, 0.0), u = make_double2(0.0, 0.0);
			if (n < R) {
				y = make_double2(v[n < R ? n : 0].x, -v[n < R ? n : 0].y);
				const double r2 = fma(y.x, y.x, y.y * y.y);
				const bool counted = r2 > thr2;
				if (counted) add_unit_phasor(u, y);
				const unsigned long long word = __ballot(!counted && exact_ok);
				const size_t kk = j0 + (size_t)n * L;
				if (lane == 0 && kk < sg->nvalid) mrow[kk] = word;
			}
			st16[2 * i] = y.x; st16[2 * i + 1] = y.y;
			ps16[2 * i] = u.x; ps16[2 * i + 1] = u.y;
		}
		const double sm = valu_reduce16(st16, lane), q = valu_reduce16(ps16, lane);
		const int n = ch * 8 + (int)(o16 >> 1);
		if ((lane & 3) == 0 && n < R) {
			const size_t kk = j0 + (size_t)n * L;
			if (kk < sg->nvalid) {
				((double *)(pS + kk))[o16 & 1] = sm;
				((double *)(pP + kk))[o16 & 1] = q;
			}
		}
	}
}

template <bool COEF>
__global__ void __launch_bounds__(256) k_spec_inv(const SpecSeg *__restrict__ segs, unsigned nseg, unsigned nitems, const double2 *__restrict__ src, size_t src_rows,
                                                  double2 *__restrict__ dst, size_t dst_rows, const double2 *__restrict__ tw, const SpecEpi ep, const int rows_mode)
{
	const unsigned lane = threadIdx.x & 63, wv = __builtin_amdgcn_readfirstlane(threadIdx.x >> 6);
	const unsigned item = blockIdx.x * 4 + wv, tb = blockIdx.y;
	if (item >= nitems) return;
	const SpecSeg *sg = spec_find_seg(segs, nseg, item);
	const unsigned j = item - sg->item0;
	const double2 *s = src + ((size_t)tb * src_rows + sg->src) * 64 + lane;
	if (sg->last && !rows_mode) {
		switch (sg->radix) {
		case 16: spec_inv_last_body<16, COEF>(s, sg, j, tw, ep, tb, lane); break;
		case 8: spec_inv_last_body<8, COEF>(s, sg, j, tw, ep, tb, lane); break;
		case 4: spec_inv_last_body<4, COEF>(s, sg, j, tw, ep, tb, lane); break;
		default: spec_inv_last_body<2, COEF>(s, sg, j, tw, ep, tb, lane); break;
		}
		return;
	}
	double2 *d = dst + ((size_t)tb * dst_rows + sg->dst) * 64 + lane;
	switch (sg->radix) {
	case 32: spec_mid_body<32, true>(s, d, sg, j, tw); break;
	case 16: spec_mid_body<16, true>(s, d, sg, j, tw); break;
	case 8: spec_mid_body<8, true>(s, d, sg, j, tw); break;
	case 4: spec_mid_body<4, true>(s, d, sg, j, tw); break;
	default: spec_mid_body<2, true>(s, d, sg, j, tw); break;
	}
}

struct SpecRowScale {
	unsigned long long roff;
	unsigned long long goff;
	unsigned long long coff;
	double tau;
	unsigned Ns, buf;
	unsigned s, pad;
};

__device__ __forceinline__ unsigned spec_row_scale(const SpecRowScale *__restrict__ rs, unsigned nrs, unsigned lane, unsigned long long i)
{
	const unsigned long long ro0 = lane < nrs ? rs[lane].roff : ~0ull, ro1 = lane + 64 < nrs ? rs[lane + 64].roff : ~0ull;
	return (unsigned)__popcll(__ballot(ro0 <= i)) + (unsigned)__popcll(__ballot(ro1 <= i)) - 1u;
}

template <typename TIn>
__device__ __forceinline__ double2 spec_fir_exact(const TIn *__restrict__ col, unsigned TP, unsigned N, const ScaleDesc &d, const double2 *__restrict__ w, unsigned k)
{
	long long n0 = ((long long)k * d.D - d.c) % (long long)N;
	const unsigned n = (unsigned)(n0 < 0 ? n0 + N : n0), l0 = min(d.L, N - n);
	const double2 *__restrict__ ws = w + d.tap_off;
	const TIn *__restrict__ xp = col + (size_t)n * TP;
	double2 a = make_double2(0.0, 0.0);
#pragma unroll 8
	for (unsigned l = 0; l < l0; l++) {
		const double x = (double)xp[(size_t)l * TP];
		a.x = fma(x, ws[l].x, a.x);
		a.y = fma(x, ws[l].y, a.y);
	}
#pragma unroll 8
	for (unsigned l = l0; l < d.L; l++) {
		const double x = (double)col[(size_t)(l - l0) * TP];
		a.x = fma(x, ws[l].x, a.x);
		a.y = fma(x, ws[l].y, a.y);
	}
	return a;
}

template <typename TIn>
__global__ void __launch_bounds__(256) k_spec_fixup(const unsigned long long *__restrict__ mask, unsigned long long nspec, const SpecRowScale *__restrict__ rs,
                                                    unsigned nrs, const ScaleDesc *__restrict__ sc, const double2 *__restrict__ w, const TIn *__restrict__ xT,
                                                    unsigned TP, unsigned N, double2 *__restrict__ PS, size_t stride)
{
	const unsigned lane = threadIdx.x & 63, wv = threadIdx.x >> 6, tb = blockIdx.y;
	const unsigned long long i0 = ((unsigned long long)blockIdx.x * 4 + wv) * 64;
	if (i0 >= nspec) return;
	const unsigned long long mine = i0 + lane < nspec ? mask[(size_t)tb * nspec + i0 + lane] : 0ull;
	for (unsigned long long todo = __ballot(mine != 0ull); todo; todo &= todo - 1) {
		const unsigned j = (unsigned)__builtin_ctzll(todo);
		const unsigned long long word = ((unsigned long long)(unsigned)__builtin_amdgcn_readlane((int)(unsigned)(mine >> 32), (int)j) << 32) |
		                                (unsigned)__builtin_amdgcn_readlane((int)(unsigned)mine, (int)j);
		const unsigned long long i = i0 + j;
		const SpecRowScale d = rs[spec_row_scale(rs, nrs, lane, i)];
		const ScaleDesc sd = sc[d.s];
		const unsigned k = (unsigned)(i - d.roff);
		double2 u = make_double2(0.0, 0.0);
		if ((word >> lane) & 1ull) {
			const double2 r = spec_fir_exact<TIn>(xT + (size_t)tb * 64 + lane, TP, N, sd, w, k);
			add_unit_phasor(u, make_double2(r.x, -r.y));
		}
		double2 *pp = PS + (size_t)tb * stride + d.coff + k;
		double2 ps = *pp;
		for (unsigned long long b = word; b; b &= b - 1) {
			const int l = __builtin_ctzll(b);
			ps.x += __shfl(u.x, l, 64);
			ps.y += __shfl(u.y, l, 64);
		}
		if (lane == 0) *pp = ps;
	}
}

struct SpecRowsOut {
	double2 *OUT; size_t out_stride; const double *Mv; double M, K, wu; int mode, keep; double2 *keepST;
	double2 *accST, *accPS; size_t stride;
};

__global__ void __launch_bounds__(256) k_spec_stack_rows(const SpecRowScale *__restrict__ rs, unsigned nrs, unsigned long long ntot, const double2 *__restrict__ b0,
                                                         size_t rows0, const double2 *__restrict__ b1, size_t rows1, unsigned nblk, unsigned ntr, unsigned tps,
                                                         unsigned ncol, const double *__restrict__ amax, const ScaleDesc *__restrict__ sc, const double2 *__restrict__ taps,
                                                         const double *__restrict__ xT, unsigned N, const SpecRowsOut o)
{
	extern __shared__ double slab[];
	const unsigned lane = threadIdx.x & 63, wv = threadIdx.x >> 6;
	const unsigned long long i = (unsigned long long)blockIdx.x * 4 + wv;
	if (i >= ntot) return;
	const SpecRowScale d = rs[spec_row_scale(rs, nrs, lane, i)];
	const size_t k = (size_t)(i - d.roff);
	const double2 *__restrict__ src = d.buf ? b1 : b0;
	const size_t rows = d.buf ? rows1 : rows0;
	double *w = slab + (size_t)wv * nblk * 64 * 4;
	for (unsigned tb = 0; tb < nblk; tb++) {
		const unsigned t = tb * 64 + lane;
		const double2 r = src[((size_t)tb * rows + d.goff + k) * 64 + lane];
		const double2 y = t < ntr ? make_double2(r.x, -r.y) : make_double2(0.0, 0.0);
		double2 u = make_double2(0.0, 0.0);
		const double am = amax[t], thr = SPEC_EXACT_G * d.tau * am;
		if (fma(y.x, y.x, y.y * y.y) > thr * thr) add_unit_phasor(u, y);
		else if (t < ntr && am > 0.0 && am <= 1.7976931348623157e308) {
			const double2 ex = spec_fir_exact<double>(xT + t, nblk * 64, N, sc[d.s], taps, (unsigned)k);
			add_unit_phasor(u, make_double2(ex.x, -ex.y));
		}
		double *e = w + (size_t)t * 4;
		e[0] = y.x; e[1] = y.y; e[2] = u.x; e[3] = u.y;
	}
	for (unsigned c = lane; c < ncol; c += 64) {
		double2 st = make_double2(0.0, 0.0), ps = make_double2(0.0, 0.0);
		const unsigned t0 = c * tps, t1 = min(ntr, t0 + tps);
		for (unsigned t = t0; t < t1; t++) {
			const double *e = w + (size_t)t * 4;
			st.x += e[0]; st.y += e[1]; ps.x += e[2]; ps.y += e[3];
		}
		const size_t ci = (size_t)d.coff + k;
		if (o.OUT) {
			o.OUT[(size_t)c * o.out_stride + ci] = weight_value(st, ps, o.mode, o.K, o.Mv ? o.Mv[c] : o.M, o.wu);
			if ((int)c == o.keep && o.keepST) o.keepST[ci] = st;
		} else {
			o.accST[(size_t)c * o.stride + ci] = st;
			o.accPS[(size_t)c * o.stride + ci] = ps;
		}
	}
}

static unsigned ilog2u(unsigned v) { unsigned l = 0; while ((1u << l) < v) l++; return l; }

static std::vector<unsigned> radix_bits(unsigned m, unsigned last_max)
{
	std::vector<unsigned> b;
	if (!m) return b;
	for (unsigned np = (m + 4) / 5;; np++) {
		const unsigned base = m / np, extra = m % np;
		if (base > last_max || base + (extra ? 1u : 0u) > 5u) continue;
		for (unsigned i = 0; i < np; i++) b.push_back(base + (i < extra ? 1u : 0u));
		return b;
	}
}

struct SpecPlan {
	unsigned s_first = 0, s_end = 0;
	unsigned N = 0;
	unsigned Nx = 0, split = 0;
	unsigned M = 0, R = 0, logsteps = 0, NS = 0, ngroups = 0;
	size_t grows = 0;
	std::vector<unsigned> fwd_bits;
	double2 *d_tw = nullptr, *d_tab = nullptr;
	SpecSlot *d_slots = nullptr;
	SpecSeg *d_fseg = nullptr;
	std::vector<SpecSeg *> d_iseg;
	std::vector<unsigned> iseg_n, iseg_items;
	SpecRowScale *d_rows = nullptr;
	unsigned long long nrowcoef = 0;
};

static void spec_plan_free(SpecPlan *sp)
{
	if (!sp) return;
	if (sp->d_tw) (void)hipFree(sp->d_tw);
	if (sp->d_tab) (void)hipFree(sp->d_tab);
	if (sp->d_slots) (void)hipFree(sp->d_slots);
	if (sp->d_fseg) (void)hipFree(sp->d_fseg);
	for (SpecSeg *s : sp->d_iseg) if (s) (void)hipFree(s);
	if (sp->d_rows) (void)hipFree(sp->d_rows);
	delete sp;
}

static void spec_decomp_free(SpecDecomp *d)
{
	if (!d) return;
	spec_plan_free(d->sp);
	if (d->T.d_sc) (void)hipFree(d->T.d_sc);
	if (d->T.d_items) (void)hipFree(d->T.d_items);
	if (d->T.d_gcols) (void)hipFree(d->T.d_gcols);
	delete d;
}

void tspws_spectral_destroy(tspws_hip_plan *p)
{
	for (SpecDecomp *d : p->spec) spec_decomp_free(d);
	p->spec.clear();
}

void tspws_spectral_geometry(const tspws_hip_plan *p, unsigned *NT, unsigned *s_end, unsigned *cneg)
{
	const unsigned N = p->N, S = p->S;
	*NT = N; *s_end = S; *cneg = 0;
	if ((N & (N - 1)) == 0) return;
	unsigned nt = 1;
	while (nt < N) nt <<= 1;
	unsigned e = 0;
	while (e < S && (unsigned long long)N + p->sc[e].L - 1 <= nt) e++;
	double in = 0, out = 0;
	for (unsigned s = 0; s < S; s++) {
		const unsigned D = p->sc[s].D;
		if (D < 8 || (D & (D - 1))) continue;
		(s < e ? in : out) += (double)p->sc[s].L * (double)p->sc[s].Ns;
	}
	bool dbl = e < S && out > 0.25 * (in + out);
	if (const char *v = sweep_env("TSPWS_SPEC_NT")) { if (!strcmp(v, "min")) dbl = false; else if (!strcmp(v, "double")) dbl = true; }
	if (dbl && nt <= (1u << 30)) { nt <<= 1; e = S; }
	int cm = 0;
	for (unsigned s = 0; s < e; s++) cm = std::max(cm, p->sc[s].c);
	*NT = nt; *s_end = e; *cneg = (unsigned)cm;
}

unsigned tspws_spectral_end_scale(const tspws_hip_plan *p)
{
	unsigned NT, e, c;
	tspws_spectral_geometry(p, &NT, &e, &c);
	return e;
}

static bool spec_scale_ok(const tspws_hip_plan *p, unsigned s, unsigned NT, unsigned s_end)
{
	const unsigned N = p->N, D = p->sc[s].D;
	if (N < 1024 || s >= s_end || D < 8 || (D & (D - 1)) || NT / D < 2 || p->sc[s].L > N) return false;
	if (NT == N) return N % D == 0 && p->sc[s].Ns == N / D && p->sc[s].Ns >= 2;
	return (unsigned long long)N + p->sc[s].L - 1 <= NT && p->sc[s].Ns == (N + D - 1) / D;
}

unsigned tspws_spectral_first_scale(const tspws_hip_plan *p, unsigned nsmax)
{
	unsigned NT, s_end, cneg;
	tspws_spectral_geometry(p, &NT, &s_end, &cneg);
	unsigned first = s_end;
	for (unsigned e = s_end; e > 0;) {
		unsigned s = e - 1;
		while (s > 0 && p->sc[s - 1].D == p->sc[e - 1].D && p->sc[s - 1].Ns == p->sc[e - 1].Ns) s--;
		bool ok = p->sc[s].Ns <= nsmax && s_end - s <= 128;
		for (unsigned v = s; v < e && ok; v++) ok = spec_scale_ok(p, v, NT, s_end);
		if (ok && e < s_end && p->sc[e].D != 2 * p->sc[s].D) ok = false;
		if (!ok) break;
		first = s;
		e = s;
	}
	return first < s_end ? first : p->S;
}

static int spec_build(tspws_hip_plan *p, unsigned s_first, unsigned nblk_hint, SpecPlan *sp)
{
	struct Tmp {
		void *v[5] = {nullptr, nullptr, nullptr, nullptr, nullptr};
		~Tmp() { for (void *q : v) if (q) (void)hipFree(q); }
	} tmp;
	unsigned NT, s_end, cneg;
	tspws_spectral_geometry(p, &NT, &s_end, &cneg);
	const unsigned N = NT, M = N / 2, S = p->S;
	if (s_first >= s_end) return fail(TSPWS_E_ARG, "spectral: empty set");
	const unsigned nsc = s_end - s_first;
	sp->s_first = s_first; sp->s_end = s_end; sp->N = N; sp->M = M; sp->Nx = p->N; sp->split = N - cneg;
	if (nsc > 128) return fail(TSPWS_E_ARG, "spectral: more than 128 scales in the spectral set");
	unsigned nsw = 16;
	if (const char *e = sweep_env("TSPWS_SPEC_NSW")) nsw = atoi(e) <= 8 ? 8u : 16u;
	if (nsc > 8 * nsw) nsw = 16;
	const unsigned ngroups = (nsc + nsw - 1) / nsw;
	const unsigned per = (nsc + ngroups - 1) / ngroups, NS = per <= 8 ? 8u : 16u;
	sp->ngroups = ngroups; sp->NS = NS;
	unsigned R = 64;
	while ((size_t)R * ngroups * std::max(1u, nblk_hint) < 4096 && N / (2 * R) >= 32) R *= 2;
	sp->R = R; sp->logsteps = ilog2u(N / R);
	std::vector<SpecSlot> slots((size_t)ngroups * NS);
	std::vector<unsigned> slot_scale((size_t)ngroups * NS, ~0u);
	std::vector<size_t> goff(S, 0);
	size_t rows = 0;
	for (unsigned g = 0; g < ngroups; g++) {
		for (unsigned i = 0; i < NS; i++) {
			SpecSlot &sl = slots[(size_t)g * NS + i];
			const unsigned s = s_first + g * per + i;
			if (i < per && s < s_end) {
				const unsigned D = p->sc[s].D, Nb = N / D;
				slot_scale[(size_t)g * NS + i] = s;
				goff[s] = rows;
				sl.goff = rows;
				if (Nb >= R) { sl.ld = ilog2u(D); sl.lb = ilog2u(Nb / R); rows += Nb; }
				else { sl.ld = 31; sl.lb = 0; rows += R; }
			} else { sl.ld = 31; sl.lb = 31; sl.goff = 0; }
		}
	}
	if (rows >> 32) return fail(TSPWS_E_ARG, "spectral: folded spectra of a trace block exceed 2^32 rows");
	sp->grows = rows;
	HIP_TRY(hipMalloc(&sp->d_slots, slots.size() * sizeof(SpecSlot)));
	HIP_TRY(hipMemcpy(sp->d_slots, slots.data(), slots.size() * sizeof(SpecSlot), hipMemcpyHostToDevice));
	HIP_TRY(hipMalloc(&sp->d_tw, (size_t)N * sizeof(double2)));
	hipLaunchKernelGGL(k_spec_twiddle, dim3((N + 255) / 256), dim3(256), 0, 0, sp->d_tw, N);
	sp->fwd_bits = radix_bits(ilog2u(M), 4);
	{
		static const bool r64_off = sweep_env("TSPWS_SPEC_R64") && !strcmp(sweep_env("TSPWS_SPEC_R64"), "0");
		const unsigned m = ilog2u(M);
		if (!r64_off && nblk_hint >= 4 && m == 15) {
			if (3 < sp->fwd_bits.size()) sp->fwd_bits = std::vector<unsigned>{6u, 5u, 4u};
		}
	}
	{
		std::vector<SpecSeg> fs;
		unsigned L = 1;
		for (size_t i = 0; i < sp->fwd_bits.size(); i++) {
			const unsigned Rr = 1u << sp->fwd_bits[i];
			SpecSeg g;
			memset(&g, 0, sizeof g);
			g.len = M; g.L = L; g.radix = Rr; g.nfold = 1; g.tw_mul = N / (L * Rr);
			fs.push_back(g);
			L *= Rr;
		}
		HIP_TRY(hipMalloc(&sp->d_fseg, fs.size() * sizeof(SpecSeg)));
		HIP_TRY(hipMemcpy(sp->d_fseg, fs.data(), fs.size() * sizeof(SpecSeg), hipMemcpyHostToDevice));
	}
	std::vector<double> wn(S, 0.0);
	{
		HIP_TRY(hipMalloc(&tmp.v[0], S * sizeof(double)));
		hipLaunchKernelGGL(k_spec_wnorm, dim3(S), dim3(256), 0, 0, (const ScaleDesc *)p->d_sc, (const double2 *)p->d_w, (double *)tmp.v[0]);
		HIP_TRY(hipMemcpy(wn.data(), tmp.v[0], S * sizeof(double), hipMemcpyDeviceToHost));
	}
	auto tau_of = [&](unsigned s) { return 8.0 * 1.1102230246251565e-16 * (double)ilog2u(N) * sqrt((double)N) * wn[s]; };
	{
		std::vector<std::vector<SpecSeg>> lev;
		for (unsigned s = s_first; s < s_end; s++) {
			const unsigned Nb = N / p->sc[s].D;
			const std::vector<unsigned> bits = radix_bits(ilog2u(Nb), 4);
			unsigned L = 1;
			for (size_t i = 0; i < bits.size(); i++) {
				if (lev.size() <= i) lev.emplace_back();
				const unsigned Rr = 1u << bits[i];
				SpecSeg g;
				memset(&g, 0, sizeof g);
				g.len = Nb; g.L = L; g.radix = Rr; g.tw_mul = N / (L * Rr);
				g.nfold = (i == 0 && Nb < R) ? R / Nb : 1u;
				g.src = g.dst = goff[s];
				g.last = (i + 1 == bits.size()) ? 1u : 0u;
				g.nvalid = p->sc[s].Ns;
				g.coff = p->sc[s].coef_off;
				g.tau = tau_of(s);
				lev[i].push_back(g);
				L *= Rr;
			}
		}
		{
			std::vector<SpecRowScale> rv;
			unsigned long long ro = 0;
			for (unsigned s = s_first; s < s_end; s++) {
				const unsigned Ns = p->sc[s].Ns;
				SpecRowScale q;
				memset(&q, 0, sizeof q);
				q.roff = ro; q.goff = goff[s]; q.coff = p->sc[s].coef_off; q.Ns = Ns;
				q.buf = (unsigned)(radix_bits(ilog2u(N / p->sc[s].D), 4).size() & 1u);
				q.tau = tau_of(s);
				q.s = s;
				rv.push_back(q);
				ro += Ns;
			}
			sp->nrowcoef = ro;
			HIP_TRY(hipMalloc(&sp->d_rows, rv.size() * sizeof(SpecRowScale)));
			HIP_TRY(hipMemcpy(sp->d_rows, rv.data(), rv.size() * sizeof(SpecRowScale), hipMemcpyHostToDevice));
		}
		for (std::vector<SpecSeg> &v : lev) {
			unsigned items = 0;
			for (SpecSeg &g : v) { g.item0 = items; items += g.len / g.radix; }
			SpecSeg *d = nullptr;
			HIP_TRY(hipMalloc(&d, v.size() * sizeof(SpecSeg)));
			sp->d_iseg.push_back(d); sp->iseg_n.push_back((unsigned)v.size()); sp->iseg_items.push_back(items);
			HIP_TRY(hipMemcpy(d, v.data(), v.size() * sizeof(SpecSeg), hipMemcpyHostToDevice));
		}
	}
	{
		const unsigned nslots = ngroups * NS, nsb = (nslots + 63) / 64;
		const size_t bytes = (size_t)nsb * N * 64 * sizeof(double2);
		HIP_TRY(hipMalloc(&tmp.v[1], slot_scale.size() * sizeof(unsigned)));
		unsigned *d_ss = (unsigned *)tmp.v[1];
		HIP_TRY(hipMemcpy(d_ss, slot_scale.data(), slot_scale.size() * sizeof(unsigned), hipMemcpyHostToDevice));
		HIP_TRY(hipMalloc(&tmp.v[2], bytes));
		HIP_TRY(hipMalloc(&tmp.v[3], bytes));
		double2 *a = (double2 *)tmp.v[2], *b = (double2 *)tmp.v[3];
		HIP_TRY(hipMemset(a, 0, bytes));
		hipLaunchKernelGGL(k_spec_place, dim3((p->N + 255) / 256, nslots), dim3(256), 0, 0, (const ScaleDesc *)p->d_sc, (const double2 *)p->d_w, (const unsigned *)d_ss, N, a);
		const std::vector<unsigned> bits = radix_bits(ilog2u(N), 5);
		std::vector<SpecSeg> ts;
		unsigned L = 1;
		for (unsigned bt : bits) {
			SpecSeg g;
			memset(&g, 0, sizeof g);
			g.len = N; g.L = L; g.radix = 1u << bt; g.nfold = 1; g.tw_mul = N / (L * g.radix);
			ts.push_back(g);
			L *= g.radix;
		}
		HIP_TRY(hipMalloc(&tmp.v[4], ts.size() * sizeof(SpecSeg)));
		SpecSeg *d_ts = (SpecSeg *)tmp.v[4];
		HIP_TRY(hipMemcpy(d_ts, ts.data(), ts.size() * sizeof(SpecSeg), hipMemcpyHostToDevice));
		for (size_t i = 0; i < ts.size(); i++) {
			const unsigned items = N / ts[i].radix;
			hipLaunchKernelGGL((k_spec_mid<true>), dim3((items + 3) / 4, nsb), dim3(256), 0, 0, (const SpecSeg *)(d_ts + i), 1u, items, (const double2 *)a, (size_t)N, b,
			                   (size_t)N, (const double2 *)sp->d_tw);
			std::swap(a, b);
		}
		const size_t total = (size_t)ngroups * N * NS;
		HIP_TRY(hipMalloc(&sp->d_tab, (total + 8) * sizeof(double2)));
		HIP_TRY(hipMemset(sp->d_tab + total, 0, 8 * sizeof(double2)));
		hipLaunchKernelGGL(k_spec_permute, dim3((unsigned)((total + 255) / 256)), dim3(256), 0, 0, (const double2 *)a, N, R, sp->logsteps, NS, ngroups, sp->d_tab);
		HIP_TRY(hipDeviceSynchronize());
	}
	HIP_TRY(hipGetLastError());
	return 0;
}

int tspws_spectral_decomp(tspws_hip_plan *p, unsigned s_first, unsigned nblk_hint, SpecDecomp **out, bool few)
{
	const bool small = nblk_hint < 8;
	for (SpecDecomp *d : p->spec) if (d->s_first == s_first && d->few == few && d->small == small) { *out = d; return 0; }
	SpecDecomp *d = new SpecDecomp;
	d->s_first = s_first; d->few = few; d->small = small;
	d->sp = new SpecPlan;
	int rc = spec_build(p, s_first, nblk_hint, d->sp);
	d->s_end = d->sp->s_end;
	if (!rc && !few) rc = tspws_build_tl_spectral(p, s_first, d->s_end, nblk_hint, d->T);
	if (rc) { spec_decomp_free(d); return rc; }
	p->spec.push_back(d);
	*out = d;
	return 0;
}

template <typename TIn>
int tspws_spectral_run(tspws_hip_plan *p, SpecDecomp *dc, const TIn *xT, unsigned TP, unsigned ntr, double2 *ST, double2 *PS, size_t stride, double2 *Y, hipStream_t st,
                       const SpecRowsOut *ro, unsigned tps, unsigned ncol)
{
	SpecPlan *sp = dc->sp;
	const unsigned N = sp->N, M = sp->M, nblk = TP / 64;
	const size_t xrows = (size_t)M + 1;
	void *v;
	int rc;
	if ((rc = scratch(p, SCR_SPA, (size_t)nblk * xrows * 64 * sizeof(double2), &v))) return rc;
	double2 *A = (double2 *)v;
	if ((rc = scratch(p, SCR_SPB, (size_t)nblk * xrows * 64 * sizeof(double2), &v))) return rc;
	double2 *B = (double2 *)v;
	if ((rc = scratch(p, SCR_SPG, (size_t)nblk * sp->grows * 64 * sizeof(double2), &v))) return rc;
	double2 *G = (double2 *)v;
	if ((rc = scratch(p, SCR_SPM, (size_t)TP * sizeof(double), &v))) return rc;
	const double *amax = (const double *)v;
	unsigned long long *mask = nullptr;
	if (!Y && !ro) {
		if ((rc = scratch(p, SCR_SPK, (size_t)nblk * sp->nrowcoef * sizeof(unsigned long long), &v))) return rc;
		mask = (unsigned long long *)v;
	}
	const size_t np = sp->fwd_bits.size();
	{
		const unsigned R0 = 1u << sp->fwd_bits[0];
		if (R0 == 64) hipLaunchKernelGGL((k_spec_fwd_first<TIn, true>), dim3((M / R0 + 3) / 4, nblk), dim3(256), 0, st, xT, TP, A, xrows, M, R0, sp->Nx, sp->split);
		else hipLaunchKernelGGL((k_spec_fwd_first<TIn>), dim3((M / R0 + 3) / 4, nblk), dim3(256), 0, st, xT, TP, A, xrows, M, R0, sp->Nx, sp->split);
	}
	double2 *cur = A, *oth = B;
	for (size_t i = 1; i + 1 < np; i++) {
		const unsigned items = M >> sp->fwd_bits[i];
		if (sp->fwd_bits[i] == 6) hipLaunchKernelGGL((k_spec_mid<false, true>), dim3((items + 3) / 4, nblk), dim3(256), 0, st, (const SpecSeg *)(sp->d_fseg + i), 1u, items, (const double2 *)cur, xrows, oth,
		                                             xrows, (const double2 *)sp->d_tw);
		else hipLaunchKernelGGL((k_spec_mid<false>), dim3((items + 3) / 4, nblk), dim3(256), 0, st, (const SpecSeg *)(sp->d_fseg + i), 1u, items, (const double2 *)cur, xrows, oth,
		                        xrows, (const double2 *)sp->d_tw);
		std::swap(cur, oth);
	}
	{
		const unsigned Rl = 1u << sp->fwd_bits[np - 1], L = M / Rl;
		hipLaunchKernelGGL(k_spec_fwd_last, dim3((L / 2 + 1 + 3) / 4, nblk), dim3(256), 0, st, (const double2 *)cur, xrows, oth, xrows, M, Rl, (const double2 *)sp->d_tw);
		std::swap(cur, oth);
	}
	const double2 *Xh = cur;
	static const bool fold_lds = sweep_env("TSPWS_SPEC_FOLD") && !strcmp(sweep_env("TSPWS_SPEC_FOLD"), "lds");
	if (sp->NS == 16 && !fold_lds) {
		const unsigned gpw = nblk >= 3 ? 1u : 4u / nblk;
		hipLaunchKernelGGL(k_spec_fold_mfma, dim3(sp->R, (sp->ngroups + gpw - 1) / gpw, (nblk + 3) / 4), dim3(256), 0, st, Xh, xrows, (const double2 *)sp->d_tab,
		                   (const SpecSlot *)sp->d_slots, sp->R, sp->logsteps, N, nblk, sp->ngroups, G, sp->grows);
	} else {
		static int ntb = -1;
		if (ntb < 0) { const char *e = sweep_env("TSPWS_SPEC_NTB"); ntb = (e && atoi(e) == 1) ? 1 : 2; }
		const unsigned NTB = (unsigned)ntb;
		static const unsigned abl = sweep_env("TSPWS_SPEC_ABL") ? (unsigned)atoi(sweep_env("TSPWS_SPEC_ABL")) : 0u;
		const unsigned nsets = (nblk + NTB - 1) / NTB;
		const unsigned WG = sp->ngroups, WT = std::max(1u, std::min(8u / WG, nsets));
		const dim3 grid(sp->R, (nsets + WT - 1) / WT), block(64 * WG * WT);
		const size_t lds = (size_t)WG * SP_RB * 1024 + (size_t)WG * WT * 16 * sizeof(SpecSlot);
#define SPEC_FOLD(NSV, NT) hipLaunchKernelGGL((k_spec_fold<NSV, NT>), grid, block, lds, st, Xh, xrows, (const double2 *)sp->d_tab, (const SpecSlot *)sp->d_slots, sp->R, sp->logsteps, N, nblk, WG, G, sp->grows, abl)
		if (NTB == 2) { if (sp->NS == 8) SPEC_FOLD(8, 2); else SPEC_FOLD(16, 2); }
		else { if (sp->NS == 8) SPEC_FOLD(8, 1); else SPEC_FOLD(16, 1); }
#undef SPEC_FOLD
	}
	SpecEpi ep;
	ep.ST = ST; ep.PS = PS; ep.stride = stride; ep.amax = amax; ep.Y = Y; ep.ncoef = p->ncoef; ep.ntr = ntr;
	ep.mask = mask; ep.nspec = sp->nrowcoef; ep.coff0 = p->sc[sp->s_first].coef_off;
	double2 *g2 = oth;
	size_t g2rows = xrows;
	if ((ro || sp->d_iseg.size() > 1) && sp->grows > xrows) {
		if ((rc = scratch(p, SCR_SPH, (size_t)nblk * sp->grows * 64 * sizeof(double2), &v))) return rc;
		g2 = (double2 *)v; g2rows = sp->grows;
	}
	const double2 *src = G;
	size_t src_rows = sp->grows;
	double2 *dst = g2;
	size_t dst_rows = g2rows;
	for (size_t l = 0; l < sp->d_iseg.size(); l++) {
		const unsigned items = sp->iseg_items[l];
		if (Y) hipLaunchKernelGGL((k_spec_inv<true>), dim3((items + 3) / 4, nblk), dim3(256), 0, st, (const SpecSeg *)sp->d_iseg[l], sp->iseg_n[l], items, src, src_rows, dst, dst_rows,
		                          (const double2 *)sp->d_tw, ep, 0);
		else hipLaunchKernelGGL((k_spec_inv<false>), dim3((items + 3) / 4, nblk), dim3(256), 0, st, (const SpecSeg *)sp->d_iseg[l], sp->iseg_n[l], items, src, src_rows, dst, dst_rows,
		                        (const double2 *)sp->d_tw, ep, ro ? 1 : 0);
		const double2 *ns = dst;
		const size_t nr = dst_rows;
		dst = (double2 *)src; dst_rows = src_rows;
		src = ns; src_rows = nr;
	}
	if (ro) {
		if (nblk > 8) return fail(TSPWS_E_ARG, "spectral: at most 512 rows in columns");
		const size_t lds = (size_t)4 * nblk * 64 * 4 * sizeof(double);
		hipLaunchKernelGGL(k_spec_stack_rows, dim3((unsigned)((sp->nrowcoef + 3) / 4)), dim3(256), lds, st, (const SpecRowScale *)sp->d_rows, sp->s_end - sp->s_first, sp->nrowcoef,
		                   (const double2 *)G, sp->grows, (const double2 *)g2, g2rows, nblk, ntr, tps, ncol, amax, (const ScaleDesc *)p->d_sc, (const double2 *)p->d_w,
		                   (const double *)xT, sp->Nx, *ro);
	} else if (mask) {
		const unsigned nw = (unsigned)((sp->nrowcoef + 63) / 64);
		hipLaunchKernelGGL((k_spec_fixup<TIn>), dim3((nw + 3) / 4, nblk), dim3(256), 0, st, (const unsigned long long *)mask, (unsigned long long)sp->nrowcoef,
		                   (const SpecRowScale *)sp->d_rows, sp->s_end - sp->s_first, (const ScaleDesc *)p->d_sc, (const double2 *)p->d_w, xT, TP, sp->Nx, PS, stride);
	}
	HIP_TRY(hipGetLastError());
	return 0;
}

#define SPEC_TR_TILES 4
template <typename TIn> __global__ void __launch_bounds__(256) k_spec_transpose_rows(const TIn *__restrict__ x, size_t ld, unsigned ntr, unsigned N, unsigned TP,
                                                                                      TIn *__restrict__ xT, unsigned long long *__restrict__ pmax)
{
	__shared__ TIn tile[64][65];
	const unsigned t0 = blockIdx.y * 64;
	const unsigned tx = threadIdx.x & 63, ty = threadIdx.x >> 6;
	TIn m[16];
#pragma unroll
	for (int i = 0; i < 16; i++) m[i] = (TIn)0;
	for (unsigned it = 0; it < SPEC_TR_TILES; it++) {
		const unsigned n0 = (blockIdx.x * SPEC_TR_TILES + it) * 64;
		if (n0 >= N) break;
		TIn v[16];
#pragma unroll
		for (int i = 0; i < 16; i++) {
			const unsigned t = t0 + ty + 4u * (unsigned)i, n = n0 + tx;
			v[i] = (t < ntr && n < N) ? x[(size_t)t * ld + n] : (TIn)0;
		}
		if (it) __syncthreads();
#pragma unroll
		for (int i = 0; i < 16; i++) {
			tile[ty + 4 * i][tx] = v[i];
			const TIn a = v[i] < (TIn)0 ? -v[i] : v[i];
			m[i] = (a == a) ? (a > m[i] ? a : m[i]) : (TIn)INFINITY;
		}
		__syncthreads();
#pragma unroll
		for (int i = 0; i < 16; i++) { const unsigned r = ty + 4u * (unsigned)i, n = n0 + r; if (n < N) xT[(size_t)n * TP + t0 + tx] = tile[tx][r]; }
	}
#pragma unroll
	for (int i = 0; i < 16; i++) {
		double a = (double)m[i];
#pragma unroll
		for (int o = 32; o > 0; o >>= 1) a = fmax(a, __shfl_xor(a, o, 64));
		if (tx == 0) pmax[(size_t)blockIdx.x * TP + t0 + ty + 4u * (unsigned)i] = (unsigned long long)__double_as_longlong(a);
	}
}

__global__ void __launch_bounds__(1024) k_spec_rowmax(const unsigned long long *__restrict__ pmax, unsigned np, unsigned TP, unsigned long long *__restrict__ amax)
{
	__shared__ unsigned long long sm[16][64];
	const unsigned lane = threadIdx.x & 63, wv = threadIdx.x >> 6, t = blockIdx.x * 64 + lane;
	unsigned long long a = 0;
	for (unsigned g = wv; g < np; g += 16) a = max(a, pmax[(size_t)g * TP + t]);
	sm[wv][lane] = a;
	__syncthreads();
	if (wv == 0) {
#pragma unroll
		for (int w = 1; w < 16; w++) a = max(a, sm[w][lane]);
		amax[t] = a;
	}
}

template <typename TIn>
int tspws_spectral_transpose(tspws_hip_plan *p, const TIn *d_x, size_t ld, unsigned ntr, TIn *xT, unsigned TP, hipStream_t st)
{
	const unsigned nblk = TP / 64;
	void *v;
	const unsigned np = (p->N + 64 * SPEC_TR_TILES - 1) / (64 * SPEC_TR_TILES);
	if (int rc = scratch(p, SCR_SPM, (size_t)TP * (np + 1) * sizeof(double), &v)) return rc;
	unsigned long long *amax = (unsigned long long *)v, *pmax = amax + TP;
	hipLaunchKernelGGL((k_spec_transpose_rows<TIn>), dim3(np, nblk), dim3(256), 0, st, d_x, ld, ntr, p->N, TP, xT, pmax);
	hipLaunchKernelGGL(k_spec_rowmax, dim3(nblk), dim3(1024), 0, st, (const unsigned long long *)pmax, np, TP, amax);
	HIP_TRY(hipGetLastError());
	return 0;
}
template int tspws_spectral_transpose<float>(tspws_hip_plan *, const float *, size_t, unsigned, float *, unsigned, hipStream_t);
template int tspws_spectral_transpose<double>(tspws_hip_plan *, const double *, size_t, unsigned, double *, unsigned, hipStream_t);

template <typename TIn>
static int spectral_rows(tspws_hip_plan *p, SpecDecomp *dc, const TIn *d_x, size_t ld, unsigned ntr, unsigned tps, const SpecRowsOut &ro, hipStream_t st,
                         hipEvent_t after_transposition)
{
	const unsigned nblk = (ntr + 63) / 64, TP = nblk * 64, ncol = (ntr + tps - 1) / tps;
	void *v;
	int rc;
	if ((rc = scratch(p, SCR_XT, (size_t)p->N * TP * sizeof(TIn), &v))) return rc;
	TIn *xT = (TIn *)v;
	if ((rc = tspws_spectral_transpose<TIn>(p, d_x, ld, ntr, xT, TP, st))) return rc;
	if (after_transposition) HIP_TRY(hipEventRecord(after_transposition, st));
	return tspws_spectral_run<TIn>(p, dc, (const TIn *)xT, TP, ntr, nullptr, nullptr, 0, nullptr, st, &ro, tps, ncol);
}

int tspws_spectral_rows_f64(tspws_hip_plan *p, SpecDecomp *dc, const double *d_x, size_t ld, unsigned ntr, unsigned tps, const FuseOut &fz, hipStream_t st,
                            hipEvent_t after_transposition)
{
	SpecRowsOut ro;
	memset(&ro, 0, sizeof ro);
	const FuseFinal &f = fz.fin;
	if (f.OUT) { ro.OUT = f.OUT; ro.out_stride = f.out_stride; ro.Mv = f.Mv; ro.M = f.M; ro.K = f.K; ro.wu = f.wu; ro.mode = f.mode; ro.keep = f.keep_slice; ro.keepST = f.keepST; }
	else { ro.accST = fz.accST; ro.accPS = fz.accPS; ro.stride = fz.stride; ro.keep = -1; }
	return spectral_rows<double>(p, dc, d_x, ld, ntr, tps, ro, st, after_transposition);
}

template int tspws_spectral_run<float>(tspws_hip_plan *, SpecDecomp *, const float *, unsigned, unsigned, double2 *, double2 *, size_t, double2 *, hipStream_t, const SpecRowsOut *, unsigned, unsigned);
template int tspws_spectral_run<double>(tspws_hip_plan *, SpecDecomp *, const double *, unsigned, unsigned, double2 *, double2 *, size_t, double2 *, hipStream_t, const SpecRowsOut *, unsigned, unsigned);
```

ts-pws_amd/csrc/stack.hip:

```cpp
#include "tspws_internal.h"

bool tspws_is_two_stage(const t_tsPWS *p, size_t mtr_global) { return !(!p->Kmax || p->Kmax > mtr_global); }
#define is_two_stage tspws_is_two_stage

extern "C" int tspws_hip_reduce_buffer(tspws_hip_plan *pl, const t_tsPWS *p, size_t mtr_global, double **d_buf, size_t *nd)
{
	if (!pl || !p || !d_buf || !nd) return fail(TSPWS_E_ARG, "reduce_buffer: NULL");
	HIP_TRY(hipSetDevice(pl->device));
	void *b = nullptr;
	int rc;
	if (is_two_stage(p, mtr_global)) {
		*nd = (size_t)p->Kmax * pl->N;
		if ((rc = scratch(pl, SCR_P, *nd * sizeof(double), &b))) return rc;
	} else {
		*nd = 4 * pl->ncoef;
		if ((rc = scratch(pl, SCR_STPS, *nd * sizeof(double), &b))) return rc;
	}
	*d_buf = (double *)b;
	return 0;
}

extern "C" int tspws_hip_stack_local(tspws_hip_plan *pl, const t_tsPWS *p, const float *d_x, size_t ld, size_t mtr_local, size_t first,
                                     size_t mtr_global, void *s)
{
	if (!pl || !p || (!d_x && mtr_local)) return fail(TSPWS_E_ARG, "stack_local: NULL");
	double *buf; size_t nd; int rc;
	if ((rc = tspws_hip_reduce_buffer(pl, p, mtr_global, &buf, &nd))) return rc;
	if (!mtr_local) { HIP_TRY(hipMemsetAsync(buf, 0, nd * sizeof(double), S_(s))); return 0; }
	if (is_two_stage(p, mtr_global)) return tspws_hip_partial_stacks(pl, d_x, ld, mtr_local, first, mtr_global, p->Kmax, buf, pl->N, s);
	return tspws_hip_stacks_float(pl, d_x, mtr_local, ld, buf, buf + 2 * pl->ncoef, s);
}

static int finish_block(tspws_hip_plan *pl, double **OUT, double **ST, double **PS)
{
	void *v;
	const size_t nc = pl->ncoef;
	int rc = scratch(pl, SCR_OUT, 6 * nc * sizeof(double), &v);
	if (rc) return rc;
	*OUT = (double *)v; *ST = *OUT + 2 * nc; *PS = *ST + 2 * nc;
	return 0;
}

static WeightArgs weight_args(const t_tsPWS *p, double *OUT, unsigned K, size_t mtr_global)
{
	WeightArgs wa;
	wa.OUT = (double2 *)OUT; wa.mode = tspws_weight_mode(p->wu, p->unbiased, K); wa.K = (double)K; wa.M = (double)(unsigned)mtr_global; wa.wu = p->wu;
	return wa;
}

extern "C" int tspws_hip_stack_finish_range(tspws_hip_plan *pl, const t_tsPWS *p, size_t mtr_global, unsigned g_begin, unsigned g_end, void *s)
{
	if (!pl || !p) return fail(TSPWS_E_ARG, "stack_finish_range: NULL");
	if (!is_two_stage(p, mtr_global) || g_begin > g_end || g_end > p->Kmax) return fail(TSPWS_E_ARG, "stack_finish_range: two-stage calls, 0 <= g_begin <= g_end <= Kmax");
	HIP_TRY(hipSetDevice(pl->device));
	double *OUT, *ST, *PS, *P;
	size_t nd;
	int rc;
	if ((rc = finish_block(pl, &OUT, &ST, &PS))) return rc;
	if ((rc = tspws_hip_reduce_buffer(pl, p, mtr_global, &P, &nd))) return rc;
	return tspws_stacks<double>(pl, P + (size_t)g_begin * pl->N, g_end - g_begin, pl->N, ST, PS, S_(s), g_begin != 0, nullptr, nullptr, ScaleRange());
}

static int finish_tail(tspws_hip_plan *pl, const t_tsPWS *p, size_t mtr_global, float *d_ls, float *d_ts, void *s, bool weighted)
{
	HIP_TRY(hipSetDevice(pl->device));
	double *OUT, *ST, *PS;
	int rc;
	if ((rc = finish_block(pl, &OUT, &ST, &PS))) return rc;
	const unsigned K = is_two_stage(p, mtr_global) ? p->Kmax : (unsigned)mtr_global;
	if (!weighted && (rc = tspws_hip_weight(pl, OUT, ST, PS, K, (unsigned)mtr_global, p->wu, p->unbiased, s))) return rc;
	return tspws_inverse_pair_out(pl, (const double2 *)OUT, d_ts, d_ls, (float)(unsigned)mtr_global, S_(s));
}

extern "C" int tspws_hip_stack_finish_tail(tspws_hip_plan *pl, const t_tsPWS *p, size_t mtr_global, float *d_ls, float *d_ts, void *s)
{
	if (!pl || !p) return fail(TSPWS_E_ARG, "stack_finish_tail: NULL");
	return finish_tail(pl, p, mtr_global, d_ls, d_ts, s, false);
}

extern "C" int tspws_hip_stack_finish(tspws_hip_plan *pl, const t_tsPWS *p, size_t mtr_global, float *d_ls, float *d_ts, void *s)
{
	if (!pl || !p) return fail(TSPWS_E_ARG, "stack_finish: NULL");
	HIP_TRY(hipSetDevice(pl->device));
	int rc;
	double *OUT, *ST, *PS, *B;
	size_t nd;
	if ((rc = finish_block(pl, &OUT, &ST, &PS))) return rc;
	if ((rc = tspws_hip_reduce_buffer(pl, p, mtr_global, &B, &nd))) return rc;
	if (is_two_stage(p, mtr_global)) {
		const WeightArgs wa = weight_args(p, OUT, p->Kmax, mtr_global);
		bool weighted = false;
		if ((rc = tspws_stacks<double>(pl, B, p->Kmax, pl->N, ST, PS, S_(s), false, &wa, &weighted, ScaleRange()))) return rc;
		return finish_tail(pl, p, mtr_global, d_ls, d_ts, s, weighted);
	}
	HIP_TRY(hipMemcpyAsync(ST, B, 4 * pl->ncoef * sizeof(double), hipMemcpyDeviceToDevice, S_(s)));
	return finish_tail(pl, p, mtr_global, d_ls, d_ts, s, false);
}

static bool finish_shardable(const tspws_hip_plan *pl, const t_tsPWS *p, size_t mtr_global)
{
	return is_two_stage(p, mtr_global) && !tspws_generic_forward() && !tspws_generic_inverse() && pl->inv_noct && !pl->inv_ngeneric &&
	       !tspws_many_trace_path(pl, p->Kmax);
}

extern "C" int tspws_hip_finish_shard(const tspws_hip_plan *pl, const t_tsPWS *p, size_t mtr_global, unsigned rank, unsigned world, unsigned *s_begin,
                                      unsigned *s_end)
{
	if (!pl || !p || !s_begin || !s_end || !world || rank >= world) return fail(TSPWS_E_ARG, "finish_shard: bad argument");
	if (!finish_shardable(pl, p, mtr_global)) return 1;
	const std::vector<unsigned> &og_s0 = pl->og_s0, &og_nv = pl->og_nv;
	std::vector<unsigned> items(og_s0.size());
	for (unsigned i = 0; i < items.size(); i++) items[i] = i;
	std::vector<double> cost(items.size());
	double total = 0;
	for (size_t k = 0; k < items.size(); k++) {
		double c = 0;
		const double far_w = world >= 4 ? 2.0 : 1.0;
		for (unsigned s = og_s0[items[k]]; s < og_s0[items[k]] + og_nv[items[k]]; s++)
			c += (double)pl->sc[s].L * (double)pl->sc[s].Ns * (pl->sc[s].D >= 256 ? far_w : 1.0);
		cost[k] = c; total += c;
	}
	unsigned lo = ~0u, hi = 0;
	double cum = 0;
	for (size_t k = 0; k < items.size(); k++) {
		unsigned owner = total > 0 ? (unsigned)((double)world * (cum + 0.5 * cost[k]) / total) : 0u;
		if (owner >= world) owner = world - 1;
		cum += cost[k];
		if (owner != rank) continue;
		if (lo == ~0u) lo = og_s0[items[k]];
		hi = og_s0[items[k]] + og_nv[items[k]];
	}
	*s_begin = lo == ~0u ? 0u : lo;
	*s_end = lo == ~0u ? 0u : hi;
	return 0;
}

extern "C" int tspws_hip_stack_finish_scales(tspws_hip_plan *pl, const t_tsPWS *p, size_t mtr_global, unsigned s_begin, unsigned s_end, double *d_x2,
                                             void *s)
{
	if (!pl || !p || !d_x2) return fail(TSPWS_E_ARG, "stack_finish_scales: NULL");
	if (!finish_shardable(pl, p, mtr_global)) return fail(TSPWS_E_ARG, "stack_finish_scales: no sharded finish for this plan / parameter set (tspws_hip_finish_shard tells)");
	if (s_begin > s_end || s_end > pl->S) return fail(TSPWS_E_ARG, "stack_finish_scales: 0 <= s_begin <= s_end <= S");
	HIP_TRY(hipSetDevice(pl->device));
	hipStream_t st = S_(s);
	if (s_begin == s_end) { HIP_TRY(hipMemsetAsync(d_x2, 0, 2 * (size_t)pl->N * sizeof(double), st)); return 0; }
	bool lo_ok = false, hi_ok = false;
	for (size_t i = 0; i < pl->og_s0.size(); i++) { lo_ok |= pl->og_s0[i] == s_begin; hi_ok |= pl->og_s0[i] + pl->og_nv[i] == s_end; }
	if (!lo_ok || !hi_ok) return fail(TSPWS_E_ARG, "stack_finish_scales: the range must consist of whole decimation octaves");
	double *OUT, *ST, *PS, *P;
	size_t nd;
	int rc;
	if ((rc = finish_block(pl, &OUT, &ST, &PS))) return rc;
	if ((rc = tspws_hip_reduce_buffer(pl, p, mtr_global, &P, &nd))) return rc;
	const WeightArgs wa = weight_args(p, OUT, p->Kmax, mtr_global);
	bool weighted = false;
	ScaleRange rg; rg.s0 = s_begin; rg.s1 = s_end;
	if ((rc = tspws_stacks<double>(pl, P, p->Kmax, pl->N, ST, PS, st, false, &wa, &weighted, rg))) return rc;
	if (!weighted && (rc = tspws_hip_weight(pl, OUT, ST, PS, p->Kmax, (unsigned)mtr_global, p->wu, p->unbiased, s))) return rc;
	return tspws_inverse_scales(pl, (const double2 *)OUT, d_x2, st, rg);
}

extern "C" int tspws_hip_profile_begin(tspws_hip_plan *pl, size_t max_calls)
{
	if (!pl) return fail(TSPWS_E_ARG, "profile_begin: NULL");
	HIP_TRY(hipSetDevice(pl->device));
	const size_t need = max_calls * 3;
	while (pl->prof_ev.size() < need) {
		hipEvent_t e;
		HIP_TRY(hipEventCreateWithFlags(&e, hipEventDisableSystemFence));
		pl->prof_ev.push_back(e);
	}
	pl->prof_used = 0;
	return 0;
}

extern "C" int tspws_hip_stream_launches(const tspws_hip_plan *pl) { return pl ? (int)pl->last_stream_launches : 0; }

extern "C" int tspws_hip_profile_read(tspws_hip_plan *pl, double *stage_ms, double *call_ms, size_t cap, size_t *ncalls)
{
	if (!pl || !ncalls) return fail(TSPWS_E_ARG, "profile_read: NULL");
	HIP_TRY(hipSetDevice(pl->device));
	HIP_TRY(hipDeviceSynchronize());
	const size_t n = pl->prof_used / 3;
	for (size_t i = 0; i < n && i < cap; i++) {
		float a = 0, b = 0;
		HIP_TRY(hipEventElapsedTime(&a, pl->prof_ev[3 * i], pl->prof_ev[3 * i + 1]));
		HIP_TRY(hipEventElapsedTime(&b, pl->prof_ev[3 * i], pl->prof_ev[3 * i + 2]));
		if (stage_ms) stage_ms[i] = a;
		if (call_ms) call_ms[i] = b;
	}
	*ncalls = n;
	return 0;
}

extern "C" int tspws_hip_profile_end(tspws_hip_plan *pl, double *mean_ms, size_t *ncalls)
{
	if (!pl || !mean_ms || !ncalls) return fail(TSPWS_E_ARG, "profile_end: NULL");
	size_t n = 0;
	int rc = tspws_hip_profile_read(pl, nullptr, nullptr, 0, &n);
	if (rc) return rc;
	std::vector<double> st(n);
	if ((rc = tspws_hip_profile_read(pl, st.data(), nullptr, n, &n))) return rc;
	double tot = 0;
	for (double v : st) tot += v;
	*mean_ms = n ? tot / (double)n : 0.0;
	*ncalls = n;
	pl->prof_used = 0;
	return 0;
}

static int hip_rc(hipError_t e, const char *what) { return e == hipSuccess ? 0 : tspws_fail(e == hipErrorOutOfMemory ? TSPWS_E_NOMEM : TSPWS_E_HIP, what, e); }

extern "C" int tspws_hip_stack(tspws_hip_plan *pl, const t_tsPWS *p, const float *d_x, size_t ld, size_t mtr, float *d_ls, float *d_ts,
                               void *s)
{
	if (!pl || !p || !d_x || !mtr) return fail(TSPWS_E_ARG, "stack: bad argument");
	HIP_TRY(hipSetDevice(pl->device));
	int rc;
	const bool prof = pl->prof_used + 3 <= pl->prof_ev.size();
	hipEvent_t *pe = prof ? &pl->prof_ev[pl->prof_used] : nullptr;
	if ((rc = tspws_plan_event(pl->ev_fork))) return rc;
	pl->le = tspws_hip_plan::LaunchEvents();
	const bool ride = is_two_stage(p, mtr);
	if (ride) { pl->le.first_start = prof ? pe[0] : nullptr; pl->le.last_stop = prof ? pe[1] : pl->ev_fork; }
	else if (prof) HIP_TRY(hipEventRecord(pe[0], S_(s)));
	bool weighted = false;
	if (ride) rc = tspws_hip_stack_local(pl, p, d_x, ld, mtr, 0, mtr, s);
	else {
		double *OUT, *ST, *PS;
		if (!(rc = finish_block(pl, &OUT, &ST, &PS))) {
			const WeightArgs wa = weight_args(p, OUT, (unsigned)mtr, mtr);
			rc = tspws_stacks<float>(pl, d_x, mtr, ld, ST, PS, S_(s), false, &wa, &weighted, ScaleRange());
		}
	}
	if (!rc && prof && (!ride || pl->le.last_stop)) rc = hip_rc(hipEventRecord(pe[1], S_(s)), "stack: event");
	if (!rc && prof && pl->le.first_start) rc = hip_rc(hipEventRecord(pe[0], S_(s)), "stack: event");
	pl->le.first_start = pl->le.last_stop = nullptr;
	pl->le.call_end = (!rc && prof) ? pe[2] : nullptr;
	if (!rc) rc = ride ? tspws_hip_stack_finish(pl, p, mtr, d_ls, d_ts, s) : finish_tail(pl, p, mtr, d_ls, d_ts, s, weighted);
	if (!rc && prof) {
		if (pl->le.call_end) rc = hip_rc(hipEventRecord(pe[2], S_(s)), "stack: event");
		pl->prof_used += 3;
	}
	pl->le = tspws_hip_plan::LaunchEvents();
	return rc;
}
```

ts-pws_amd/csrc/tspws_internal.h:

```cpp
#pragma once

#include <hip/hip_runtime.h>

#include <algorithm>
#include <cmath>
#include <cstdio>
#include <cstdlib>
#include <cstring>
#include <string>
#include <vector>

#include "tspws_hip.h"
#include "column_runs.h"

#ifndef TSPWS_PI
#define TSPWS_PI 3.14159265358979328
#endif

int tspws_fail(int code, const char *what, hipError_t e = hipSuccess);
#define fail tspws_fail

#define HIP_TRY(expr)                                                              \
	do {                                                                           \
		hipError_t e_ = (expr);                                                    \
		if (e_ != hipSuccess) return tspws_fail(e_ == hipErrorOutOfMemory ? TSPWS_E_NOMEM : TSPWS_E_HIP, #expr, e_); \
	} while (0)

static inline hipStream_t S_(void *s) { return (hipStream_t)s; }

#ifdef TSPWS_SWEEPS
static inline const char *sweep_env(const char *name) { return getenv(name); }
#else
static inline const char *sweep_env(const char *) { return nullptr; }
#endif

struct ScaleDesc {
	unsigned L, D, Ns;
	int c, cd;
	unsigned Q;
	unsigned long long tap_off, coef_off;
	double scale, gain;
	unsigned DL, logDL;
	unsigned MC, cps, nsplit;
	unsigned ngw;
	unsigned wave_off;
	unsigned inv_fast;
	unsigned acc_off;
	unsigned use_lds;
	unsigned lds_off, lds_bps;
	unsigned acc2_off;
	unsigned fuse_ok;
	unsigned r16;
	unsigned long long part_off;
};

struct ScaleRange {
	unsigned s0 = 0, s1 = 0;
	bool on() const { return s1 != 0; }
};

struct FuseFinal {
	const double2 *pST = nullptr, *pPS = nullptr;
	size_t pair_stride = 0, slice_stride = 0;
	unsigned nprev = 0;
	double2 *OUT = nullptr;
	size_t out_stride = 0;
	const double *Mv = nullptr;
	double M = 0;
	int mode = 0, keep_slice = -1;
	double2 *keepST = nullptr;
	double K = 0, wu = 0;
};

struct FuseOut {
	double2 *accST = nullptr, *accPS = nullptr;
	size_t stride = 0;
	unsigned tps = 1;
	bool applied = false;
	FuseFinal fin;
	bool allow_spec = false;
	unsigned spec_first = ~0u;
	hipEvent_t ev_mid = nullptr;
	bool mid_recorded = false;
	bool defer_fir_join = false;
	hipStream_t fir_stream = nullptr;
};

struct WeightArgs {
	double2 *OUT = nullptr;
	int mode = 0;
	double K = 0, M = 0, wu = 0;
	double2 *OUTP = nullptr;
	size_t outp_stride = 0;
	unsigned k0 = 0;
	int mode1 = 0;
	const double *Mv = nullptr;
	size_t out_stride = 0;
	int planes_batch = -1;
};

struct AccExtra {
	size_t trace_stride = 0;
	size_t y_fz = 0;
	const unsigned *rowmap = nullptr;
	bool fused_done = false;
};

enum { SCR_Y = 0, SCR_PART, SCR_XT, SCR_OBUF, SCR_SEL, SCR_SUBST, SCR_CONV, SCR_CHUNK, SCR_P, SCR_STPS, SCR_OUT, SCR_X2, SCR_CLS, SCR_JKP, SCR_JKOUT, SCR_TAB, SCR_FZ, SCR_JKTAB, SCR_SPA, SCR_SPB, SCR_SPG, SCR_SPH, SCR_SPM, SCR_SPK, SCR_GEMM, SCR_J1TAB, SCR_J1PL, SCR_J1T, SCR_BTAB, SCR_BXG, SCR_BY, SCR_BX, SCR_BP, SCR_ROWY, SCR_ROWX, SCR_JBPL, SCR_JBT, SCR_J2P, SCR_J2ST, SCR_CBX, SCR_CBST, SCR_CBP, SCR_CBM, SCR_SBPL, SCR_RBTAB, SCR_TSTAB, SCR_TSP, SCR_TSOUT, SCR_SRTAB, SCR_SRS, SCR_SRP, SCR_WXTAB, SCR_WXY, SCR_WXP, SCR_MWTAB, SCR_MWF, SCR_MWW, SCR_DTTAB, SCR_DTP, SCR_FTTAB, SCR_FTY, SCR_FTP, SCR_N };

struct OctDesc;
struct TLItem;

struct GemmCol;
struct TlTable {
	unsigned minns = 0;
	std::vector<ScaleDesc> sc;
	ScaleDesc *d_sc = nullptr;
	TLItem *d_items = nullptr;
	unsigned n = 0, wgs = 0, waves = 0, acc2_blocks = 0;
	size_t npart = 0, lds = 0;
	GemmCol *d_gcols = nullptr;
	unsigned gcoltiles = 0, gKS = 0, gKC = 0;
};

struct SpecDecomp;

struct TlPass {
	SpecDecomp *dc = nullptr;
	const TlTable *T = nullptr;
	size_t batch = 0;
	void *xT = nullptr;
	double2 *planes = nullptr, *part = nullptr, *gsum = nullptr;
};

struct tspws_hip_plan {
	int device = 0, type = -1;
	unsigned S = 0, V = 0, J = 0, N = 0;
	double s0 = 0, b0 = 0, w0 = 0, Cpsi = 0;
	size_t ncoef = 0, ntaps = 0;
	size_t npart = 0;
	unsigned fwd_waves = 0;
	unsigned acc_blocks = 0;
	unsigned acc2_blocks = 0;
	unsigned lds_blocks = 0;
	unsigned lds_qt = 24;
	unsigned n_fusable = 0;
	TlTable tl[2];
	std::vector<SpecDecomp *> spec;
	std::vector<unsigned> oc_s0, oc_nv, oc_wave_off, oc_nwaves, oc_gen;
	std::vector<unsigned> og_s0, og_nv;
	unsigned inv_waves_lds = 0;
	unsigned inv_waves = 0, inv_waves_fast = 0, inv_noct = 0, inv_ngeneric = 0;
	OctDesc *d_oc = nullptr;
	struct BandTables *bands = nullptr;
	std::vector<ScaleDesc> sc;
	ScaleDesc *d_sc = nullptr;
	double2 *d_w = nullptr, *d_wd = nullptr;
	void *scr[SCR_N] = {nullptr};
	size_t scr_bytes[SCR_N] = {0};
	hipStream_t side = nullptr;
	hipEvent_t ev_fork = nullptr, ev_join = nullptr;
	hipStream_t xs = nullptr;
	hipEvent_t ev_xs0 = nullptr, ev_xs1 = nullptr, ev_xs2 = nullptr;
	hipEvent_t ev_mid = nullptr;
	hipEvent_t ev_lin = nullptr;
	struct LaunchEvents { hipEvent_t first_start = nullptr, last_stop = nullptr, ready = nullptr, call_end = nullptr; } le;
	std::vector<hipEvent_t> prof_ev;
	size_t prof_used = 0;
	std::vector<Chunk> chunks;
	std::vector<unsigned> row_first;
	size_t ck_mtr = 0, ck_first = 0, ck_glob = 0;
	unsigned ck_K = 0;
	bool ck_valid = false, ck_dev = false;
	hipEvent_t ck_ev = nullptr;
	hipStream_t ck_stream = nullptr;
	unsigned last_stream_launches = 0;
	unsigned long long jk_gen = 0;
	hipStream_t xf = nullptr;
	std::vector<hipEvent_t> stage_ev;
	std::vector<void *> retired;
	tspws_hip_batch_stats batch_stats{};
	tspws_hip_jk_batch_stats jk_batch_stats{};
	tspws_hip_jk_batch2_stats jk_batch2_stats{};
	tspws_hip_conv_batch_stats conv_batch_stats{};
	tspws_hip_sub_batch_stats sub_batch_stats{};
	tspws_hip_boot_batch_stats boot_batch_stats{};
	tspws_hip_weighted_batch_stats weighted_batch_stats{};
	tspws_hip_bands_stats bands_stats{};
	tspws_hip_stack_bands_stats stack_bands_stats{};
	tspws_hip_trace_scores_stats_t trace_scores_stats{};
	tspws_hip_stretch_stats stretch_stats{};
	tspws_hip_wxs_stats wxs_stats{};
	tspws_hip_mwcs_stats mwcs_stats{};
	tspws_hip_dtw_stats dtw_stats{};
	tspws_hip_ftan_stats ftan_stats{};
};

int tspws_scratch(tspws_hip_plan *p, int slot, size_t bytes, void **out);
#define scratch tspws_scratch
int tspws_plan_stream(tspws_hip_plan *p, hipStream_t &s);
int tspws_plan_event(hipEvent_t &e, bool system_scope = false);
int tspws_fork(tspws_hip_plan *p, hipStream_t from, hipStream_t &side, hipEvent_t &ev, hipEvent_t carried = nullptr);
int tspws_join(hipStream_t side, hipStream_t into, hipEvent_t &ev);

#ifdef __HIPCC__
__device__ __forceinline__ unsigned find_scale(const ScaleDesc *sc, unsigned S, unsigned long long idx, bool taps)
{
	unsigned lo = 0, hi = S;
	while (hi - lo > 1) {
		unsigned mid = (lo + hi) >> 1;
		unsigned long long off = taps ? sc[mid].tap_off : sc[mid].coef_off;
		if (off <= idx) lo = mid; else hi = mid;
	}
	return lo;
}

__device__ __forceinline__ unsigned find_block_scale(const ScaleDesc *sc, unsigned S, unsigned block, bool acc2)
{
	unsigned lo = 0, hi = S;
	while (hi - lo > 1) {
		const unsigned mid = (lo + hi) >> 1;
		if ((acc2 ? sc[mid].acc2_off : sc[mid].acc_off) <= block) lo = mid; else hi = mid;
	}
	return lo;
}

__device__ __forceinline__ double wave_sum(double v)
{
#pragma unroll
	for (int o = 32; o > 0; o >>= 1) v += __shfl_xor(v, o, 64);
	return v;
}

__device__ __forceinline__ double readlane_f64(const double x, const int src)
{
	const int lo = __builtin_amdgcn_readlane(__double2loint(x), src), hi = __builtin_amdgcn_readlane(__double2hiint(x), src);
	return __hiloint2double(hi, lo);
}

__device__ __forceinline__ void add_unit_phasor(double2 &ps, const double2 v)
{
	const double r2 = fma(v.x, v.x, v.y * v.y);
	if (r2 > 1e-280 && r2 < 1e280) {
		const double inv = rsqrt(r2);
		ps.x = fma(v.x, inv, ps.x);
		ps.y = fma(v.y, inv, ps.y);
	} else {
		const double r = hypot(v.x, v.y);
		const double ux = v.x / r, uy = v.y / r;
		if (ux * ux + uy * uy <= 1.001) { ps.x += ux; ps.y += uy; }
	}
}

__device__ __forceinline__ double2 weight_value_eff(const double2 st, const double2 ps, const int mode, const double K, const double Kb, const double M, const double wu)
{
	double a;
	if (mode == 0) {
		const double g = 1. / (K * K * M);
		a = (ps.x * ps.x + ps.y * ps.y) * g;
		return make_double2(a * st.x, a * st.y);
	} else if (mode == 1) {
		const double g = 1. / (K * M);
		const double r = hypot(ps.x, ps.y);
		return make_double2(st.x * r * g, st.y * r * g);
	} else if (mode == 2) {
		a = hypot(ps.x, ps.y) / K;
		a = pow(a, wu);
		return make_double2(st.x * a / M, st.y * a / M);
	}
	const double iK = 1. / K, iK1 = 1. / (Kb - 1), iM = 1. / M;
	const double px = ps.x * iK, py = ps.y * iK;
	a = px * px + py * py;
	a = (Kb * a - 1) * iK1;
	return make_double2(st.x * a * iM, st.y * a * iM);
}

__device__ __forceinline__ double2 weight_value(const double2 st, const double2 ps, const int mode, const double K, const double M, const double wu)
{
	return weight_value_eff(st, ps, mode, K, K, M, wu);
}
#endif

int  tspws_build_forward(tspws_hip_plan *p);
template <typename TIn>
int  tspws_forward_parts(tspws_hip_plan *p, const TIn *d_x, size_t ntr, size_t ld, double2 *d_part, hipStream_t st, FuseOut *fz, ScaleRange rg);
template <typename TIn>
int  tspws_tl_pass_setup(tspws_hip_plan *p, size_t ntr, size_t nslots, TlPass &P);
template <typename TIn>
int  tspws_tl_pass_transform(tspws_hip_plan *p, const TlPass &P, const TIn *xb, size_t ld, unsigned nb, hipStream_t st);
template <typename TIn>
int  tspws_stacks(tspws_hip_plan *p, const TIn *d_x, size_t ntr, size_t ld, double *d_ST, double *d_PS, hipStream_t st, bool keep,
                  const WeightArgs *wa, bool *weighted, ScaleRange rg);
unsigned tspws_first_unfused_scale(const tspws_hip_plan *p);
void tspws_launch_accumulate(tspws_hip_plan *p, const double2 *part, unsigned nb, double2 *ST, double2 *PS, int zero_first, const FuseOut *fz,
                             unsigned nslices, hipStream_t st, unsigned nbatch, size_t y_part, size_t y_stack, const TlTable *tl, const WeightArgs *wa,
                             ScaleRange rg, const AccExtra *ex = nullptr);
bool tspws_fused_forward(const tspws_hip_plan *p);
bool tspws_many_trace_path(const tspws_hip_plan *p, size_t ntr);
unsigned tspws_spectral_choice(const tspws_hip_plan *p, size_t ntr);
size_t tspws_part_budget_bytes();
int  tspws_engine_pin();
bool tspws_generic_forward();
unsigned tspws_spectral_first_scale(const tspws_hip_plan *p, unsigned nsmax);
int  tspws_spectral_decomp(tspws_hip_plan *p, unsigned s_first, unsigned nblk_hint, SpecDecomp **out, bool few = false);
int  tspws_spectral_rows_f64(tspws_hip_plan *p, SpecDecomp *dc, const double *d_x, size_t ld, unsigned ntr, unsigned tps, const FuseOut &fz, hipStream_t st,
                             hipEvent_t after_transposition = nullptr);
int  tspws_build_tl_spectral(tspws_hip_plan *p, unsigned s_first, unsigned s_end, unsigned nblk_hint, TlTable &T);
void tspws_spectral_geometry(const tspws_hip_plan *p, unsigned *NT, unsigned *s_end, unsigned *cneg);
unsigned tspws_spectral_end_scale(const tspws_hip_plan *p);
struct SpecRowsOut;
template <typename TIn>
int  tspws_spectral_run(tspws_hip_plan *p, SpecDecomp *dc, const TIn *xT, unsigned TP, unsigned ntr, double2 *ST, double2 *PS, size_t stride, double2 *Y, hipStream_t st,
                        const SpecRowsOut *ro = nullptr, unsigned tps = 0, unsigned ncol = 0);
template <typename TIn>
int  tspws_spectral_transpose(tspws_hip_plan *p, const TIn *d_x, size_t ld, unsigned ntr, TIn *xT, unsigned TP, hipStream_t st);
void tspws_spectral_destroy(tspws_hip_plan *p);
int  tspws_build_inverse(tspws_hip_plan *p);
size_t tspws_inverse_row_bytes(const tspws_hip_plan *p);
int  tspws_weight_mode(double wu, int unbiased, unsigned K);
void tspws_weight_batched(tspws_hip_plan *p, double2 *OUT, const double2 *ST, const double2 *PS, int mode, double K, double wu, const double *d_Mv,
                          unsigned nb, size_t y_out, size_t y_stack, hipStream_t st, double M = 0.0);
int  tspws_inverse_pair_out(tspws_hip_plan *p, const double2 *Y, float *d_ts, float *d_ls, float mtr, hipStream_t st);
int  tspws_inverse_scales(tspws_hip_plan *p, const double2 *Y, double *x2, hipStream_t st, ScaleRange rg);
int  tspws_inverse_pairs_early(tspws_hip_plan *p, const double2 *Y, unsigned nb, unsigned s_split, hipStream_t early, bool *done);
int  tspws_inverse_pairs_late(tspws_hip_plan *p, const double2 *Y, double *x, unsigned nb, unsigned s_split, hipStream_t st);
bool tspws_generic_inverse();
struct BandOut {
	double *re = nullptr, *im = nullptr;
	float *ts = nullptr, *ls = nullptr, *ts_env = nullptr, *ls_env = nullptr;
	const unsigned *d_row = nullptr, *d_cnt = nullptr;
	unsigned row0 = 0, cnt0 = 1;
};
int  tspws_bands_check(const tspws_hip_plan *p, const tspws_band *bands, unsigned R, const char *who);
int  tspws_inverse_bands_run(tspws_hip_plan *p, const double2 *Y, size_t nset, const tspws_band *bands, unsigned R, const BandOut &out, hipStream_t st,
                             unsigned *finish_batches, unsigned *scales);
void tspws_bands_destroy(tspws_hip_plan *p);
void tspws_epilogue_rows(float *d_ts, const double *d_x, size_t N, unsigned nb, hipStream_t st);
int  tspws_run_chunks(tspws_hip_plan *p, const float *d_x, size_t ld, size_t N, const std::vector<Chunk> &chunks,
                      const std::vector<unsigned> &row_first, unsigned rows, double *d_P, size_t ldP, hipStream_t st, bool cached,
                      unsigned row_begin = 0, unsigned row_end = ~0u);
int  tspws_chunks_upload(tspws_hip_plan *p, const std::vector<Chunk> &chunks, const std::vector<unsigned> &row_first, unsigned rows, hipStream_t st,
                         bool cached);
int  tspws_chunks_launch(tspws_hip_plan *p, const float *d_x, size_t ld, size_t N, const std::vector<Chunk> &chunks,
                         const std::vector<unsigned> &row_first, unsigned rows, double *d_P, size_t ldP, hipStream_t st,
                         unsigned row_begin = 0, unsigned row_end = ~0u);
int  tspws_prefix_launch(tspws_hip_plan *p, const float *d_x, size_t ld, size_t N, const Chunk *d_runs, const unsigned *d_seg_first, unsigned nseg,
                         size_t nruns_total, const unsigned *d_carry, unsigned ncarry, double **d_snap, size_t *ldpc, hipStream_t st);
void tspws_combine_terms_launch(const double *d_snap, size_t ldpc, const unsigned *d_row_ptr, const unsigned *d_idx, const float *d_coef, unsigned nrows,
                                double *d_P, size_t N, hipStream_t st);
int  tspws_rows_walk_launch(const float *d_x, size_t ld, size_t N, const RunDesc *d_runs, unsigned q0, unsigned qm, unsigned q1, unsigned W,
                            const unsigned *d_flush_rows, const unsigned *d_fix_row, double *d_rows, double *d_blk, int carry_in, int carry_out, hipStream_t st);
unsigned tspws_rows_walk_wmax();
unsigned tspws_chunk_len_for(size_t N, size_t mtr);
class BatchCall;
int  tspws_jb2_shared(tspws_hip_plan *p, const t_tsPWS *par, const float *d_x, size_t ld, const size_t *h_first, const unsigned *list, size_t n,
                      const char *h_sel, size_t Tn, unsigned C, bool main, float *d_ls, float *d_ts, float *d_ls_out, float *d_ts_out, unsigned *h_mtr_out,
                      BatchCall &call, tspws_hip_jk_batch2_stats *stats);
bool tspws_is_two_stage(const t_tsPWS *p, size_t mtr_global);
```

Before: 1348 billion samples/s.

## Add FFT-based row-spectral path for coarse scales in few-row second-stage stacking

```diff
diff --git a/include/tspws_hip.h b/include/tspws_hip.h
--- a/include/tspws_hip.h
+++ b/include/tspws_hip.h
@@ -69,6 +69,8 @@
 unsigned tspws_hip_spectral_choice(const tspws_hip_plan *plan, size_t ntr);
 int  tspws_hip_forward_spectral_f64(tspws_hip_plan *plan, const double *d_x, size_t ntr, size_t ld, double *d_Y, unsigned nsmax, void *stream);
 int  tspws_hip_forward_spectral_f32(tspws_hip_plan *plan, const float  *d_x, size_t ntr, size_t ld, double *d_Y, unsigned nsmax, void *stream);
+unsigned tspws_hip_few_rows_spectral_choice(const tspws_hip_plan *plan, size_t rows, unsigned elem_bytes);
+int  tspws_hip_forward_rows_spectral_f64(tspws_hip_plan *plan, const double *d_rows, size_t nrows, size_t ld, double *d_Y, unsigned s_first, void *stream);
 int  tspws_hip_inverse(tspws_hip_plan *plan, const double *d_Y, size_t nrec, double *d_x, void *stream);
 typedef struct {
 	unsigned items;
diff --git a/ts-pws_amd/__init__.py b/ts-pws_amd/__init__.py
--- a/ts-pws_amd/__init__.py
+++ b/ts-pws_amd/__init__.py
@@ -80,6 +80,8 @@
     "tspws_hip_spectral_transform_length": (_u, [_vp]),
     "tspws_hip_spectral_choice": (_u, [_vp, _sz]),
     "tspws_hip_forward_spectral_f64": (_i, [_vp, _vp, _sz, _sz, _vp, _u, _vp]),
+    "tspws_hip_few_rows_spectral_choice": (_u, [_vp, _sz, _u]),
+    "tspws_hip_forward_rows_spectral_f64": (_i, [_vp, _vp, _sz, _sz, _vp, _u, _vp]),
     "tspws_hip_forward_spectral_f32": (_i, [_vp, _vp, _sz, _sz, _vp, _u, _vp]),
     "tspws_hip_inverse": (_i, [_vp, _vp, _sz, _vp, _vp]),
     "tspws_hip_inverse_info": (_i, [_vp, _vp]),
diff --git a/ts-pws_amd/csrc/forward.hip b/ts-pws_amd/csrc/forward.hip
--- a/ts-pws_amd/csrc/forward.hip
+++ b/ts-pws_amd/csrc/forward.hip
@@ -702,7 +702,7 @@
 
 template <typename TIn>
 int tspws_stacks(tspws_hip_plan *p, const TIn *d_x, size_t ntr, size_t ld, double *d_ST, double *d_PS, hipStream_t st, bool keep,
-                       const WeightArgs *wa, bool *weighted, ScaleRange rg)
+                       const WeightArgs *wa, bool *weighted, ScaleRange rg, bool row_spec)
 {
 	HIP_TRY(hipSetDevice(p->device));
 	if (weighted) *weighted = false;
@@ -724,6 +724,19 @@
 	const size_t batch = std::min<size_t>(ntr, std::max<size_t>(2, ((tspws_part_budget_bytes()) / (p->npart * sizeof(double2))) & ~(size_t)1));
 	void *v;
 	if ((rc = scratch(p, SCR_PART, batch * p->npart * sizeof(double2), &v))) return rc;
+	unsigned sf = p->S;
+	hipStream_t fir = st;
+	if constexpr (std::is_same<TIn, double>::value) {
+		if (row_spec && !rg.on() && batch >= ntr && (sf = tspws_few_rows_spectral_choice(p, ntr, 8)) < p->S) {
+			static const bool serial = sweep_env("TSPWS_ROWSPEC_PARALLEL") && !strcmp(sweep_env("TSPWS_ROWSPEC_PARALLEL"), "0");
+			const bool all = !keep;
+			if (!serial && ((rc = tspws_plan_stream(p, p->xs)) || (rc = tspws_plan_event(p->ev_xs2)))) return rc;
+			if ((rc = tspws_row_spectral_stacks(p, sf, (const double *)d_x, ld, (unsigned)ntr, (double2 *)d_ST, (double2 *)d_PS, keep, (all && wa && wa->OUT) ? wa : nullptr, st,
+			                                    serial ? nullptr : p->ev_xs2))) return rc;
+			if (!serial) { if ((rc = tspws_fork(p, st, p->xs, p->ev_xs2, p->ev_xs2))) return rc; fir = p->xs; }
+			rg.s0 = 0; rg.s1 = sf;
+		}
+	}
 	const bool fuse = p->n_fusable != 0;
 	void *vz = nullptr;
 	if (fuse) {
@@ -744,16 +757,17 @@
 			else { fz.accST = (double2 *)vz; fz.accPS = (double2 *)vz + p->ncoef; fz.stride = 2 * p->ncoef; }
 		}
 		const bool all = nb == ntr && !keep;
-		if ((rc = tspws_forward_parts<TIn>(p, d_x + t0 * ld, nb, ld, (double2 *)v, st, fuse ? &fz : nullptr, rg))) return rc;
-		tspws_launch_accumulate(p, (const double2 *)v, (unsigned)nb, (double2 *)d_ST, (double2 *)d_PS, zero_first, &fz, nsl, st, 1, 0, 0, nullptr, all ? wa : nullptr, rg);
+		if ((rc = tspws_forward_parts<TIn>(p, d_x + t0 * ld, nb, ld, (double2 *)v, fir, fuse ? &fz : nullptr, rg))) return rc;
+		tspws_launch_accumulate(p, (const double2 *)v, (unsigned)nb, (double2 *)d_ST, (double2 *)d_PS, zero_first, &fz, nsl, fir, 1, 0, 0, nullptr, all ? wa : nullptr, rg);
 		if (all && wa && wa->OUT && weighted) *weighted = true;
 	}
+	if (fir != st && (rc = tspws_join(fir, st, p->ev_xs1))) return rc;
 	HIP_TRY(hipGetLastError());
 	return 0;
 }
 
-template int tspws_stacks<float>(tspws_hip_plan *, const float *, size_t, size_t, double *, double *, hipStream_t, bool, const WeightArgs *, bool *, ScaleRange);
-template int tspws_stacks<double>(tspws_hip_plan *, const double *, size_t, size_t, double *, double *, hipStream_t, bool, const WeightArgs *, bool *, ScaleRange);
+template int tspws_stacks<float>(tspws_hip_plan *, const float *, size_t, size_t, double *, double *, hipStream_t, bool, const WeightArgs *, bool *, ScaleRange, bool);
+template int tspws_stacks<double>(tspws_hip_plan *, const double *, size_t, size_t, double *, double *, hipStream_t, bool, const WeightArgs *, bool *, ScaleRange, bool);
 
 extern "C" int tspws_hip_stacks_double(tspws_hip_plan *p, const double *d_P, unsigned K, size_t ldP, double *d_ST, double *d_PS, void *s)
 {
diff --git a/ts-pws_amd/csrc/row_spectral.h b/ts-pws_amd/csrc/row_spectral.h
--- /dev/null
+++ b/ts-pws_amd/csrc/row_spectral.h
@@ -0,0 +1,460 @@
+
+#define RSP_TILE 2048u
+#define RSP_NRB 10
+#define RSP_NV 4
+#ifndef RSP_LGP_MIN
+#define RSP_LGP_MIN 11u
+#endif
+
+struct RspScale {
+	unsigned s, lgNs;
+	unsigned long long coff;
+	double tau;
+};
+
+struct RowSpec {
+	unsigned s_first = 0, ns = 0, lgP = 0, ngroups = 0, lgA = 0, lgB = 0;
+	size_t nspec = 0;
+	double2 *d_tw = nullptr, *d_tab = nullptr;
+	RspScale *d_rs = nullptr;
+	uint2 *d_groups = nullptr;
+};
+
+namespace {
+template <int R, bool INV>
+__device__ __forceinline__ void rsp_stage(double2 *__restrict__ buf, const unsigned len, const unsigned lgTC, const unsigned L, const double2 *__restrict__ tw,
+                                          const unsigned N)
+{
+	constexpr int MAXB = RSP_TILE / R / 256;
+	const unsigned TC = 1u << lgTC, nb = (len / R) << lgTC, q = len / R, twm = N / (L * R);
+	double2 v[MAXB][R];
+#pragma unroll
+	for (int b = 0; b < MAXB; b++) {
+		const unsigned e = threadIdx.x + 256u * b;
+		if (e < nb) {
+			const unsigned c = e & (TC - 1), j = e >> lgTC, k = j & (L - 1);
+#pragma unroll
+			for (int n = 0; n < R; n++) {
+				const double2 x = buf[((size_t)(j + n * q) << lgTC) + c];
+				if (n == 0 || k == 0) v[b][n] = x;
+				else v[b][n] = cmul(x, spec_tw<INV>(tw, n * k * twm));
+			}
+		}
+	}
+	__syncthreads();
+#pragma unroll
+	for (int b = 0; b < MAXB; b++) {
+		const unsigned e = threadIdx.x + 256u * b;
+		if (e < nb) {
+			const unsigned c = e & (TC - 1), j = e >> lgTC, k = j & (L - 1), j0 = (j - k) * R + k;
+			SpecDFT<R, INV>::run(v[b]);
+#pragma unroll
+			for (int n = 0; n < R; n++) buf[((size_t)(j0 + n * L) << lgTC) + c] = v[b][n];
+		}
+	}
+	__syncthreads();
+}
+
+template <bool INV>
+__device__ __forceinline__ void rsp_lds_fft(double2 *__restrict__ buf, const unsigned len, const unsigned lgTC, const double2 *__restrict__ tw, const unsigned N)
+{
+	unsigned L = 1;
+	while (L < len) {
+		if (len / L >= 4) { rsp_stage<4, INV>(buf, len, lgTC, L, tw, N); L *= 4; }
+		else { rsp_stage<2, INV>(buf, len, lgTC, L, tw, N); L *= 2; }
+	}
+}
+}
+
+template <bool FIRST>
+__global__ void __launch_bounds__(256) k_rsp_fft(const double *__restrict__ in, const size_t in_ld, double2 *__restrict__ out, const size_t out_ld, const unsigned lglen,
+                                                 const unsigned lgTC, const unsigned IS, const unsigned OC, const unsigned OK, const double2 *__restrict__ tw,
+                                                 const unsigned N, double *__restrict__ pmax)
+{
+	__shared__ double2 buf[RSP_TILE];
+	__shared__ double red[4];
+	const unsigned len = 1u << lglen, TC = 1u << lgTC, c0 = blockIdx.x << lgTC, row = blockIdx.y, npts = len << lgTC;
+	const double *xr = in + (size_t)row * in_ld;
+	double am = 0.0;
+	for (unsigned e = threadIdx.x; e < npts; e += 256) {
+		const unsigned c = e & (TC - 1), i = e >> lgTC;
+		const size_t idx = (size_t)(c0 + c) + (size_t)i * IS;
+		const double2 z = make_double2(xr[2 * idx], xr[2 * idx + 1]);
+		if (FIRST) am = fmax(am, fmax(fabs(z.x), fabs(z.y)));
+		buf[e] = z;
+	}
+	if (FIRST) {
+#pragma unroll
+		for (int o = 32; o > 0; o >>= 1) am = fmax(am, __shfl_xor(am, o, 64));
+		if ((threadIdx.x & 63) == 0) red[threadIdx.x >> 6] = am;
+	}
+	__syncthreads();
+	if (FIRST && threadIdx.x == 0) pmax[(size_t)row * gridDim.x + blockIdx.x] = fmax(fmax(red[0], red[1]), fmax(red[2], red[3]));
+	rsp_lds_fft<false>(buf, len, lgTC, tw, N);
+	double2 *o = out + (size_t)row * out_ld;
+	for (unsigned e = threadIdx.x; e < npts; e += 256) {
+		unsigned c, k;
+		if (OK == 1) { k = e & (len - 1); c = e >> lglen; }
+		else { c = e & (TC - 1); k = e >> lgTC; }
+		double2 v = buf[((size_t)k << lgTC) + c];
+		if (FIRST) v = cmul(v, tw[2u * (c0 + c) * k]);
+		o[(size_t)(c0 + c) * OC + (size_t)k * OK] = v;
+	}
+}
+
+__global__ void __launch_bounds__(256) k_rsp_place(const ScaleDesc *__restrict__ sc, const double2 *__restrict__ w, const unsigned s_first, const unsigned N,
+                                                   double *__restrict__ U)
+{
+	const ScaleDesc d = sc[s_first + blockIdx.y];
+	const unsigned l = blockIdx.x * 256 + threadIdx.x;
+	if (l >= d.L) return;
+	long long n = ((long long)l - d.c) % (long long)N;
+	if (n < 0) n += N;
+	const double2 t = w[d.tap_off + l];
+	double *row = U + ((size_t)2 * blockIdx.y + (size_t)(n & 1)) * N + 2 * (size_t)(n >> 1);
+	row[0] = t.x; row[1] = -t.y;
+}
+
+__global__ void __launch_bounds__(256) k_rsp_table(const double2 *__restrict__ Z, const double2 *__restrict__ tw, const unsigned N, double2 *__restrict__ tab)
+{
+	const unsigned f = blockIdx.x * 256 + threadIdx.x, M = N >> 1, g = f & (M - 1);
+	if (f >= N) return;
+	const double2 ze = Z[(size_t)2 * blockIdx.y * M + g], zo = Z[((size_t)2 * blockIdx.y + 1) * M + g];
+	const double2 a = cadd(ze, cmul(tw[f], zo));
+	const double inv = 1.0 / (double)N;
+	tab[(size_t)blockIdx.y * N + f] = make_double2(a.x * inv, -a.y * inv);
+}
+
+__global__ void __launch_bounds__(256) k_rsp_fold(const double2 *__restrict__ Z, const double2 *__restrict__ tab, const double2 *__restrict__ tw,
+                                                  const uint2 *__restrict__ groups, const unsigned N, const unsigned lgP, const unsigned nwin,
+                                                  const unsigned nrows, double2 *__restrict__ part)
+{
+	__shared__ double2 red[3][RSP_NRB][64];
+	const unsigned lane = threadIdx.x & 63, wv = __builtin_amdgcn_readfirstlane(threadIdx.x >> 6);
+	const unsigned w = blockIdx.x % nwin, g = blockIdx.x / nwin;
+	const uint2 grp = groups[g];
+	const unsigned P = 1u << lgP, M = N >> 1, J = N >> lgP, JL = (J + 3) / 4;
+	const unsigned p = w * 64 + lane;
+	const bool act = p < P;
+	const unsigned pp = act ? p : 0u;
+	const unsigned j0 = wv * JL, j1 = min(J, j0 + JL);
+	for (unsigned rb = 0; rb < nrows; rb += RSP_NRB) {
+		double2 acc[RSP_NV][RSP_NRB];
+#pragma unroll
+		for (int v = 0; v < RSP_NV; v++)
+#pragma unroll
+			for (int i = 0; i < RSP_NRB; i++) acc[v][i] = make_double2(0.0, 0.0);
+#pragma unroll 2
+		for (unsigned j = j0; j < j1; j++) {
+			const unsigned f = pp + (j << lgP), gq = f & (M - 1), gm = (M - gq) & (M - 1);
+			const double2 t = tw[f];
+			double2 h[RSP_NV];
+#pragma unroll
+			for (int v = 0; v < RSP_NV; v++) {
+				h[v] = make_double2(0.0, 0.0);
+				if ((unsigned)v < grp.y) {
+					const double *hp = (const double *)(tab + (size_t)(grp.x + v) * N + f);
+					h[v] = make_double2(__builtin_nontemporal_load(hp), __builtin_nontemporal_load(hp + 1));
+				}
+			}
+#pragma unroll
+			for (int i = 0; i < RSP_NRB; i++) {
+				if (rb + i < nrows) {
+					const double2 *zr = Z + (size_t)(rb + i) * M;
+					const double2 z = zr[gq], zm = zr[gm];
+					const double2 E = make_double2(0.5 * (z.x + zm.x), 0.5 * (z.y - zm.y));
+					const double2 O = make_double2(0.5 * (z.y + zm.y), -0.5 * (z.x - zm.x));
+					const double2 X = cadd(E, cmul(t, O));
+#pragma unroll
+					for (int v = 0; v < RSP_NV; v++) {
+						acc[v][i].x = fma(X.x, h[v].x, fma(-X.y, h[v].y, acc[v][i].x));
+						acc[v][i].y = fma(X.x, h[v].y, fma(X.y, h[v].x, acc[v][i].y));
+					}
+				}
+			}
+		}
+#pragma unroll
+		for (int v = 0; v < RSP_NV; v++) {
+			if ((unsigned)v >= grp.y) break;
+			if (wv > 0) {
+#pragma unroll
+				for (int i = 0; i < RSP_NRB; i++) red[wv - 1][i][lane] = acc[v][i];
+			}
+			__syncthreads();
+			if (wv == 0 && act) {
+#pragma unroll
+				for (int i = 0; i < RSP_NRB; i++) {
+					if (rb + i < nrows) {
+						double2 a = acc[v][i];
+						a = cadd(a, red[0][i][lane]); a = cadd(a, red[1][i][lane]); a = cadd(a, red[2][i][lane]);
+						part[(((size_t)(grp.x + v) * nrows + rb + i) << lgP) + p] = a;
+					}
+				}
+			}
+			__syncthreads();
+		}
+	}
+}
+
+__global__ void __launch_bounds__(256) k_rsp_inv(const double2 *__restrict__ part, const RspScale *__restrict__ rs, const unsigned lgP, const unsigned nrows,
+                                                 const double2 *__restrict__ tw, const unsigned N, double2 *__restrict__ out, const size_t out_ld)
+{
+	__shared__ double2 buf[RSP_TILE];
+	__shared__ double2 tmp[256];
+	const RspScale d = rs[blockIdx.x];
+	const unsigned row = blockIdx.y, Ns = 1u << d.lgNs, nm = 1u << (lgP - d.lgNs);
+	const double2 *src = part + (((size_t)blockIdx.x * nrows + row) << lgP);
+	if (Ns >= 256) {
+		for (unsigned q = threadIdx.x; q < Ns; q += 256) {
+			double2 a = src[q];
+			for (unsigned m = 1; m < nm; m++) a = cadd(a, src[q + ((size_t)m << d.lgNs)]);
+			buf[q] = a;
+		}
+	} else {
+		const unsigned q = threadIdx.x & (Ns - 1), sub = threadIdx.x >> d.lgNs, nsub = 256u >> d.lgNs;
+		double2 a = make_double2(0.0, 0.0);
+		for (unsigned m = sub; m < nm; m += nsub) a = cadd(a, src[q + ((size_t)m << d.lgNs)]);
+		tmp[threadIdx.x] = a;
+		__syncthreads();
+		if (threadIdx.x < Ns) {
+			double2 b = tmp[threadIdx.x];
+			for (unsigned u = 1; u < nsub; u++) b = cadd(b, tmp[threadIdx.x + (u << d.lgNs)]);
+			buf[threadIdx.x] = b;
+		}
+	}
+	__syncthreads();
+	rsp_lds_fft<true>(buf, Ns, 0u, tw, N);
+	double2 *o = out + (size_t)row * out_ld + d.coff;
+	for (unsigned k = threadIdx.x; k < Ns; k += 256) o[k] = make_double2(buf[k].x, -buf[k].y);
+}
+
+struct RspStackOut {
+	double2 *ST, *PS, *OUT;
+	int keep, mode;
+	double K, M, wu;
+};
+
+__global__ void __launch_bounds__(256) k_rsp_stack(const double2 *__restrict__ W, const size_t nspec, const RspScale *__restrict__ rs, const unsigned nrs,
+                                                   const unsigned nrows, const double *__restrict__ pmax, const unsigned ntiles, const ScaleDesc *__restrict__ sc,
+                                                   const double2 *__restrict__ taps, const double *__restrict__ x, const size_t ld, const unsigned N,
+                                                   const unsigned long long coff0, const RspStackOut o)
+{
+	__shared__ double amax[64];
+	if (threadIdx.x < nrows) {
+		double a = 0.0;
+		for (unsigned t = 0; t < ntiles; t++) a = fmax(a, pmax[(size_t)threadIdx.x * ntiles + t]);
+		amax[threadIdx.x] = a;
+	}
+	__syncthreads();
+	const size_t i = (size_t)blockIdx.x * 256 + threadIdx.x;
+	if (i >= nspec) return;
+	unsigned lo = 0, hi = nrs;
+	while (hi - lo > 1) { const unsigned mid = (lo + hi) >> 1; if (rs[mid].coff <= i) lo = mid; else hi = mid; }
+	const RspScale d = rs[lo];
+	const unsigned k = (unsigned)(i - d.coff);
+	const size_t ci = (size_t)coff0 + i;
+	double2 st = o.keep ? o.ST[ci] : make_double2(0.0, 0.0), ps = o.keep ? o.PS[ci] : make_double2(0.0, 0.0);
+	for (unsigned r = 0; r < nrows; r++) {
+		const double2 y = W[(size_t)r * nspec + i];
+		const double am = amax[r], thr = SPEC_EXACT_G * d.tau * am;
+		st.x += y.x; st.y += y.y;
+		if (fma(y.x, y.x, y.y * y.y) > thr * thr) add_unit_phasor(ps, y);
+		else if (am > 0.0 && am <= 1.7976931348623157e308) {
+			const double2 ex = spec_fir_exact<double>(x + (size_t)r * ld, 1u, N, sc[d.s], taps, k);
+			add_unit_phasor(ps, make_double2(ex.x, -ex.y));
+		}
+	}
+	o.ST[ci] = st; o.PS[ci] = ps;
+	if (o.OUT) o.OUT[ci] = weight_value(st, ps, o.mode, o.K, o.M, o.wu);
+}
+
+static void rsp_free(RowSpec *r);
+
+void tspws_row_spectral_destroy(tspws_hip_plan *p)
+{
+	for (RowSpec *r : p->rowspec) rsp_free(r);
+	p->rowspec.clear();
+}
+
+bool tspws_row_spectral_ok(const tspws_hip_plan *p, unsigned s_first)
+{
+	const unsigned N = p->N;
+	if (N < 1024 || (N & (N - 1)) || N > (1u << 22) || s_first >= p->S) return false;
+	for (unsigned s = s_first; s < p->S; s++) {
+		const ScaleDesc &d = p->sc[s];
+		if (!d.D || (d.D & (d.D - 1)) || N % d.D || d.Ns != N / d.D || d.Ns > RSP_TILE || d.L > N) return false;
+		if (s > s_first && d.D < p->sc[s - 1].D) return false;
+	}
+	return true;
+}
+
+static int rsp_transform(const RowSpec *r, const double *rows, size_t ld, unsigned nrows, double2 *T, double2 *Z, double *pmax, unsigned N, hipStream_t st,
+                         hipEvent_t after_first = nullptr)
+{
+	const unsigned M = N >> 1, A = 1u << r->lgA, B = 1u << r->lgB;
+	const unsigned lgTC1 = std::min(r->lgA, ilog2u(RSP_TILE) - r->lgB), lgTC2 = std::min(r->lgB, ilog2u(RSP_TILE) - r->lgA);
+	hipLaunchKernelGGL((k_rsp_fft<true>), dim3(A >> lgTC1, nrows), dim3(256), 0, st, rows, ld, T, (size_t)M, r->lgB, lgTC1, A, B, 1u, (const double2 *)r->d_tw, N, pmax);
+	if (after_first) HIP_TRY(hipEventRecord(after_first, st));
+	hipLaunchKernelGGL((k_rsp_fft<false>), dim3(B >> lgTC2, nrows), dim3(256), 0, st, (const double *)T, (size_t)N, Z, (size_t)M, r->lgA, lgTC2, B, 1u, B,
+	                   (const double2 *)r->d_tw, N, (double *)nullptr);
+	return 0;
+}
+static unsigned rsp_ntiles(const RowSpec *r) { return (1u << r->lgA) >> std::min(r->lgA, ilog2u(RSP_TILE) - r->lgB); }
+
+static void rsp_free(RowSpec *r)
+{
+	if (r->d_tw) (void)hipFree(r->d_tw);
+	if (r->d_tab) (void)hipFree(r->d_tab);
+	if (r->d_rs) (void)hipFree(r->d_rs);
+	if (r->d_groups) (void)hipFree(r->d_groups);
+	delete r;
+}
+
+static int rsp_fill(tspws_hip_plan *p, unsigned s_first, RowSpec *r)
+{
+	const unsigned N = p->N, M = N >> 1, S = p->S, ns = S - s_first;
+	r->s_first = s_first; r->ns = ns;
+	unsigned lgpmin = RSP_LGP_MIN;
+	if (const char *e = sweep_env("TSPWS_ROWSPEC_LGP")) lgpmin = (unsigned)std::max(6, atoi(e));
+	r->lgP = std::max(ilog2u(p->sc[s_first].Ns), std::min(lgpmin, ilog2u(N)));
+	const unsigned m = ilog2u(M);
+	r->lgA = m / 2; r->lgB = m - r->lgA;
+	HIP_TRY(hipMalloc(&r->d_tw, (size_t)N * sizeof(double2)));
+	hipLaunchKernelGGL(k_spec_twiddle, dim3((N + 255) / 256), dim3(256), 0, 0, r->d_tw, N);
+	std::vector<double> wn(S);
+	{
+		double *d_wn = nullptr;
+		HIP_TRY(hipMalloc(&d_wn, S * sizeof(double)));
+		hipLaunchKernelGGL(k_spec_wnorm, dim3(S), dim3(256), 0, 0, (const ScaleDesc *)p->d_sc, (const double2 *)p->d_w, d_wn);
+		const hipError_t e = hipMemcpy(wn.data(), d_wn, S * sizeof(double), hipMemcpyDeviceToHost);
+		(void)hipFree(d_wn);
+		HIP_TRY(e);
+	}
+	std::vector<RspScale> rs(ns);
+	std::vector<uint2> groups;
+	size_t co = 0;
+	for (unsigned i = 0; i < ns; i++) {
+		const ScaleDesc &d = p->sc[s_first + i];
+		rs[i].s = s_first + i; rs[i].lgNs = ilog2u(d.Ns); rs[i].coff = co;
+		rs[i].tau = 8.0 * 1.1102230246251565e-16 * (double)ilog2u(N) * sqrt((double)N) * wn[s_first + i];
+		co += d.Ns;
+		if (!groups.empty() && groups.back().y < RSP_NV) groups.back().y++;
+		else groups.push_back(make_uint2(i, 1u));
+	}
+	if (p->sc[s_first].coef_off + co != p->ncoef) return fail(TSPWS_E_ARG, "row spectral: the scales from s_first on are not the tail of the coefficient set");
+	r->nspec = co; r->ngroups = (unsigned)groups.size();
+	HIP_TRY(hipMalloc(&r->d_rs, ns * sizeof(RspScale)));
+	HIP_TRY(hipMemcpy(r->d_rs, rs.data(), ns * sizeof(RspScale), hipMemcpyHostToDevice));
+	HIP_TRY(hipMalloc(&r->d_groups, groups.size() * sizeof(uint2)));
+	HIP_TRY(hipMemcpy(r->d_groups, groups.data(), groups.size() * sizeof(uint2), hipMemcpyHostToDevice));
+	HIP_TRY(hipMalloc(&r->d_tab, (size_t)ns * N * sizeof(double2)));
+	const unsigned nb = std::min(ns, 16u);
+	double *U = nullptr, *pm = nullptr;
+	double2 *T = nullptr, *Z = nullptr;
+	hipError_t e = hipMalloc(&U, (size_t)2 * nb * N * sizeof(double));
+	if (e == hipSuccess) e = hipMalloc(&T, (size_t)2 * nb * M * sizeof(double2));
+	if (e == hipSuccess) e = hipMalloc(&Z, (size_t)2 * nb * M * sizeof(double2));
+	if (e == hipSuccess) e = hipMalloc(&pm, (size_t)2 * nb * rsp_ntiles(r) * sizeof(double));
+	for (unsigned b0 = 0; b0 < ns && e == hipSuccess; b0 += nb) {
+		const unsigned n = std::min(nb, ns - b0);
+		unsigned Lmax = 0;
+		for (unsigned i = 0; i < n; i++) Lmax = std::max(Lmax, p->sc[s_first + b0 + i].L);
+		e = hipMemsetAsync(U, 0, (size_t)2 * n * N * sizeof(double), 0);
+		if (e != hipSuccess) break;
+		hipLaunchKernelGGL(k_rsp_place, dim3((Lmax + 255) / 256, n), dim3(256), 0, 0, (const ScaleDesc *)p->d_sc, (const double2 *)p->d_w, s_first + b0, N, U);
+		(void)rsp_transform(r, U, (size_t)N, 2 * n, T, Z, pm, N, 0);
+		hipLaunchKernelGGL(k_rsp_table, dim3((N + 255) / 256, n), dim3(256), 0, 0, (const double2 *)Z, (const double2 *)r->d_tw, N, r->d_tab + (size_t)b0 * N);
+		e = hipGetLastError();
+	}
+	if (e == hipSuccess) e = hipDeviceSynchronize();
+	if (U) (void)hipFree(U);
+	if (T) (void)hipFree(T);
+	if (Z) (void)hipFree(Z);
+	if (pm) (void)hipFree(pm);
+	HIP_TRY(e);
+	return 0;
+}
+
+static int rsp_build(tspws_hip_plan *p, unsigned s_first, RowSpec **out)
+{
+	for (RowSpec *r : p->rowspec) if (r->s_first == s_first) { *out = r; return 0; }
+	if (!tspws_row_spectral_ok(p, s_first)) return fail(TSPWS_E_ARG, "row spectral: N a power of two >= 1024 and scales with power-of-two D | N, N / D <= 2048 from s_first on");
+	RowSpec *r = new RowSpec;
+	if (int rc = rsp_fill(p, s_first, r)) { rsp_free(r); return rc; }
+	p->rowspec.push_back(r);
+	*out = r;
+	return 0;
+}
+
+int tspws_row_spectral(tspws_hip_plan *p, unsigned s_first, const double *d_x, size_t ld, unsigned nrows, double2 *Y, const RspStackOut *so, hipStream_t st,
+                       hipEvent_t fork_ev)
+{
+	static const int fork_at = sweep_env("TSPWS_ROWSPEC_FORK") ? atoi(sweep_env("TSPWS_ROWSPEC_FORK")) : 0;
+	RowSpec *r = nullptr;
+	int rc;
+	if ((rc = rsp_build(p, s_first, &r))) return rc;
+	const unsigned N = p->N, M = N >> 1, P = 1u << r->lgP, nwin = std::max(1u, P / 64u), ntiles = rsp_ntiles(r);
+	void *vT, *vZ, *vG, *vW = nullptr, *vM;
+	if ((rc = scratch(p, SCR_RSA, (size_t)nrows * M * sizeof(double2), &vT))) return rc;
+	if ((rc = scratch(p, SCR_RSB, (size_t)nrows * M * sizeof(double2), &vZ))) return rc;
+	if ((rc = scratch(p, SCR_RSG, ((size_t)r->ns * nrows << r->lgP) * sizeof(double2), &vG))) return rc;
+	if (so && (rc = scratch(p, SCR_RSW, (size_t)nrows * r->nspec * sizeof(double2), &vW))) return rc;
+	if ((rc = scratch(p, SCR_RSM, (size_t)nrows * ntiles * sizeof(double), &vM))) return rc;
+	if ((rc = rsp_transform(r, d_x, ld, nrows, (double2 *)vT, (double2 *)vZ, (double *)vM, N, st, fork_at == 0 ? fork_ev : nullptr))) return rc;
+	if (fork_ev && fork_at == 2) HIP_TRY(hipEventRecord(fork_ev, st));
+	hipLaunchKernelGGL(k_rsp_fold, dim3(nwin * r->ngroups), dim3(256), 0, st, (const double2 *)vZ, (const double2 *)r->d_tab, (const double2 *)r->d_tw,
+	                   (const uint2 *)r->d_groups, N, r->lgP, nwin, nrows, (double2 *)vG);
+	if (fork_ev && fork_at == 1) HIP_TRY(hipEventRecord(fork_ev, st));
+	const unsigned long long coff0 = p->sc[s_first].coef_off;
+	hipLaunchKernelGGL(k_rsp_inv, dim3(r->ns, nrows), dim3(256), 0, st, (const double2 *)vG, (const RspScale *)r->d_rs, r->lgP, nrows, (const double2 *)r->d_tw, N,
+	                   so ? (double2 *)vW : Y + coff0, so ? r->nspec : p->ncoef);
+	if (so)
+		hipLaunchKernelGGL(k_rsp_stack, dim3((unsigned)((r->nspec + 255) / 256)), dim3(256), 0, st, (const double2 *)vW, r->nspec, (const RspScale *)r->d_rs, r->ns, nrows,
+		                   (const double *)vM, ntiles, (const ScaleDesc *)p->d_sc, (const double2 *)p->d_w, d_x, ld, N, coff0, *so);
+	HIP_TRY(hipGetLastError());
+	return 0;
+}
+
+int tspws_row_spectral_stacks(tspws_hip_plan *p, unsigned s_first, const double *d_x, size_t ld, unsigned nrows, double2 *ST, double2 *PS, bool keep,
+                              const WeightArgs *wa, hipStream_t st, hipEvent_t fork_ev)
+{
+	RspStackOut so;
+	so.ST = ST; so.PS = PS; so.OUT = wa ? wa->OUT : nullptr; so.keep = keep ? 1 : 0;
+	so.mode = wa ? wa->mode : 0; so.K = wa ? wa->K : 0.0; so.M = wa ? wa->M : 0.0; so.wu = wa ? wa->wu : 0.0;
+	return tspws_row_spectral(p, s_first, d_x, ld, nrows, nullptr, &so, st, fork_ev);
+}
+
+#ifndef RSP_RULE_MIN_N
+#define RSP_RULE_MIN_N 131072u
+#endif
+#ifndef RSP_RULE_DMIN
+#define RSP_RULE_DMIN 64u
+#endif
+unsigned tspws_few_rows_spectral_choice(const tspws_hip_plan *p, size_t rows, unsigned elem_bytes)
+{
+	const unsigned N = p->N, S = p->S;
+	if (elem_bytes != 8 || !rows || rows >= 64 || (N & (N - 1)) || N < 1024 || tspws_engine_pin() == 1 || tspws_generic_forward()) return S;
+	unsigned dmin = (RSP_RULE_MIN_N && N >= RSP_RULE_MIN_N) ? RSP_RULE_DMIN : 0u;
+	if (const char *e = sweep_env("TSPWS_ROWSPEC_DMIN")) dmin = (unsigned)std::max(0, atoi(e));
+	if (!dmin) return S;
+	dmin = std::max(dmin, N / RSP_TILE);
+	unsigned s = 0;
+	while (s < S && p->sc[s].D < dmin) s++;
+	while (s < S && !tspws_row_spectral_ok(p, s)) s++;
+	return (s > 0 && s < S) ? s : S;
+}
+
+extern "C" unsigned tspws_hip_few_rows_spectral_choice(const tspws_hip_plan *p, size_t rows, unsigned elem_bytes)
+{
+	return p ? tspws_few_rows_spectral_choice(p, rows, elem_bytes) : 0u;
+}
+
+extern "C" int tspws_hip_forward_rows_spectral_f64(tspws_hip_plan *p, const double *d_rows, size_t nrows, size_t ld, double *d_Y, unsigned s_first, void *s)
+{
+	if (!p || !d_rows || !d_Y) return fail(TSPWS_E_ARG, "forward_rows_spectral: NULL");
+	if (!nrows) return 0;
+	if (nrows >= 64) return fail(TSPWS_E_ARG, "forward_rows_spectral: fewer than 64 rows (more go through tspws_hip_forward_spectral_f64)");
+	if (ld < p->N) return fail(TSPWS_E_ARG, "forward_rows_spectral: ld < N");
+	HIP_TRY(hipSetDevice(p->device));
+	return tspws_row_spectral(p, s_first, d_rows, ld, (unsigned)nrows, (double2 *)d_Y, nullptr, S_(s), nullptr);
+}
diff --git a/ts-pws_amd/csrc/spectral.hip b/ts-pws_amd/csrc/spectral.hip
--- a/ts-pws_amd/csrc/spectral.hip
+++ b/ts-pws_amd/csrc/spectral.hip
@@ -775,10 +775,13 @@
 	delete d;
 }
 
+void tspws_row_spectral_destroy(tspws_hip_plan *p);
+
 void tspws_spectral_destroy(tspws_hip_plan *p)
 {
 	for (SpecDecomp *d : p->spec) spec_decomp_free(d);
 	p->spec.clear();
+	tspws_row_spectral_destroy(p);
 }
 
 void tspws_spectral_geometry(const tspws_hip_plan *p, unsigned *NT, unsigned *s_end, unsigned *cneg)
@@ -1215,3 +1218,5 @@
 
 template int tspws_spectral_run<float>(tspws_hip_plan *, SpecDecomp *, const float *, unsigned, unsigned, double2 *, double2 *, size_t, double2 *, hipStream_t, const SpecRowsOut *, unsigned, unsigned);
 template int tspws_spectral_run<double>(tspws_hip_plan *, SpecDecomp *, const double *, unsigned, unsigned, double2 *, double2 *, size_t, double2 *, hipStream_t, const SpecRowsOut *, unsigned, unsigned);
+
+#include "row_spectral.h"
diff --git a/ts-pws_amd/csrc/stack.hip b/ts-pws_amd/csrc/stack.hip
--- a/ts-pws_amd/csrc/stack.hip
+++ b/ts-pws_amd/csrc/stack.hip
@@ -58,7 +58,7 @@
 	int rc;
 	if ((rc = finish_block(pl, &OUT, &ST, &PS))) return rc;
 	if ((rc = tspws_hip_reduce_buffer(pl, p, mtr_global, &P, &nd))) return rc;
-	return tspws_stacks<double>(pl, P + (size_t)g_begin * pl->N, g_end - g_begin, pl->N, ST, PS, S_(s), g_begin != 0, nullptr, nullptr, ScaleRange());
+	return tspws_stacks<double>(pl, P + (size_t)g_begin * pl->N, g_end - g_begin, pl->N, ST, PS, S_(s), g_begin != 0, nullptr, nullptr, ScaleRange(), true);
 }
 
 static int finish_tail(tspws_hip_plan *pl, const t_tsPWS *p, size_t mtr_global, float *d_ls, float *d_ts, void *s, bool weighted)
@@ -90,7 +90,7 @@
 	if (is_two_stage(p, mtr_global)) {
 		const WeightArgs wa = weight_args(p, OUT, p->Kmax, mtr_global);
 		bool weighted = false;
-		if ((rc = tspws_stacks<double>(pl, B, p->Kmax, pl->N, ST, PS, S_(s), false, &wa, &weighted, ScaleRange()))) return rc;
+		if ((rc = tspws_stacks<double>(pl, B, p->Kmax, pl->N, ST, PS, S_(s), false, &wa, &weighted, ScaleRange(), true))) return rc;
 		return finish_tail(pl, p, mtr_global, d_ls, d_ts, s, weighted);
 	}
 	HIP_TRY(hipMemcpyAsync(ST, B, 4 * pl->ncoef * sizeof(double), hipMemcpyDeviceToDevice, S_(s)));
diff --git a/ts-pws_amd/csrc/tspws_internal.h b/ts-pws_amd/csrc/tspws_internal.h
--- a/ts-pws_amd/csrc/tspws_internal.h
+++ b/ts-pws_amd/csrc/tspws_internal.h
@@ -106,7 +106,7 @@
 	bool fused_done = false;
 };
 
-enum { SCR_Y = 0, SCR_PART, SCR_XT, SCR_OBUF, SCR_SEL, SCR_SUBST, SCR_CONV, SCR_CHUNK, SCR_P, SCR_STPS, SCR_OUT, SCR_X2, SCR_CLS, SCR_JKP, SCR_JKOUT, SCR_TAB, SCR_FZ, SCR_JKTAB, SCR_SPA, SCR_SPB, SCR_SPG, SCR_SPH, SCR_SPM, SCR_SPK, SCR_GEMM, SCR_J1TAB, SCR_J1PL, SCR_J1T, SCR_BTAB, SCR_BXG, SCR_BY, SCR_BX, SCR_BP, SCR_ROWY, SCR_ROWX, SCR_JBPL, SCR_JBT, SCR_J2P, SCR_J2ST, SCR_CBX, SCR_CBST, SCR_CBP, SCR_CBM, SCR_SBPL, SCR_RBTAB, SCR_TSTAB, SCR_TSP, SCR_TSOUT, SCR_SRTAB, SCR_SRS, SCR_SRP, SCR_WXTAB, SCR_WXY, SCR_WXP, SCR_MWTAB, SCR_MWF, SCR_MWW, SCR_DTTAB, SCR_DTP, SCR_FTTAB, SCR_FTY, SCR_FTP, SCR_N };
+enum { SCR_Y = 0, SCR_PART, SCR_XT, SCR_OBUF, SCR_SEL, SCR_SUBST, SCR_CONV, SCR_CHUNK, SCR_P, SCR_STPS, SCR_OUT, SCR_X2, SCR_CLS, SCR_JKP, SCR_JKOUT, SCR_TAB, SCR_FZ, SCR_JKTAB, SCR_SPA, SCR_SPB, SCR_SPG, SCR_SPH, SCR_SPM, SCR_SPK, SCR_GEMM, SCR_J1TAB, SCR_J1PL, SCR_J1T, SCR_BTAB, SCR_BXG, SCR_BY, SCR_BX, SCR_BP, SCR_ROWY, SCR_ROWX, SCR_JBPL, SCR_JBT, SCR_J2P, SCR_J2ST, SCR_CBX, SCR_CBST, SCR_CBP, SCR_CBM, SCR_SBPL, SCR_RBTAB, SCR_TSTAB, SCR_TSP, SCR_TSOUT, SCR_SRTAB, SCR_SRS, SCR_SRP, SCR_WXTAB, SCR_WXY, SCR_WXP, SCR_MWTAB, SCR_MWF, SCR_MWW, SCR_DTTAB, SCR_DTP, SCR_FTTAB, SCR_FTY, SCR_FTP, SCR_RSA, SCR_RSB, SCR_RSG, SCR_RSW, SCR_RSM, SCR_N };
 
 struct OctDesc;
 struct TLItem;
@@ -124,6 +124,7 @@
 };
 
 struct SpecDecomp;
+struct RowSpec;
 
 struct TlPass {
 	SpecDecomp *dc = nullptr;
@@ -147,6 +148,7 @@
 	unsigned n_fusable = 0;
 	TlTable tl[2];
 	std::vector<SpecDecomp *> spec;
+	std::vector<RowSpec *> rowspec;
 	std::vector<unsigned> oc_s0, oc_nv, oc_wave_off, oc_nwaves, oc_gen;
 	std::vector<unsigned> og_s0, og_nv;
 	unsigned inv_waves_lds = 0;
@@ -290,7 +292,7 @@
 int  tspws_tl_pass_transform(tspws_hip_plan *p, const TlPass &P, const TIn *xb, size_t ld, unsigned nb, hipStream_t st);
 template <typename TIn>
 int  tspws_stacks(tspws_hip_plan *p, const TIn *d_x, size_t ntr, size_t ld, double *d_ST, double *d_PS, hipStream_t st, bool keep,
-                  const WeightArgs *wa, bool *weighted, ScaleRange rg);
+                  const WeightArgs *wa, bool *weighted, ScaleRange rg, bool row_spec = false);
 unsigned tspws_first_unfused_scale(const tspws_hip_plan *p);
 void tspws_launch_accumulate(tspws_hip_plan *p, const double2 *part, unsigned nb, double2 *ST, double2 *PS, int zero_first, const FuseOut *fz,
                              unsigned nslices, hipStream_t st, unsigned nbatch, size_t y_part, size_t y_stack, const TlTable *tl, const WeightArgs *wa,
@@ -315,6 +317,10 @@
 template <typename TIn>
 int  tspws_spectral_transpose(tspws_hip_plan *p, const TIn *d_x, size_t ld, unsigned ntr, TIn *xT, unsigned TP, hipStream_t st);
 void tspws_spectral_destroy(tspws_hip_plan *p);
+struct RspStackOut;
+unsigned tspws_few_rows_spectral_choice(const tspws_hip_plan *p, size_t rows, unsigned elem_bytes);
+int  tspws_row_spectral_stacks(tspws_hip_plan *p, unsigned s_first, const double *d_x, size_t ld, unsigned nrows, double2 *ST, double2 *PS, bool keep,
+                               const WeightArgs *wa, hipStream_t st, hipEvent_t fork_ev);
 int  tspws_build_inverse(tspws_hip_plan *p);
 size_t tspws_inverse_row_bytes(const tspws_hip_plan *p);
 int  tspws_weight_mode(double wu, int unbiased, unsigned K);
```

Measured after the change: 1352 billion samples/s, median of 2. Within noise of the previous version (+0.4%).
